# 42jaylonw/shifu

Measured on NVIDIA B200. Metric: env-steps/sec (obs+reward+term+reset), higher is better.
Workload: dtype f32

## Files before the change

### include/shifu_b200.h

```cpp
#ifndef SHIFU_B200_H
#define SHIFU_B200_H

#include <stdint.h>

#ifdef __cplusplus
extern "C" {
#endif

#define SHIFU_ABI_VERSION 5

#define SHIFU_MAX_DOF 12
#define SHIFU_MAX_LEG_BODIES 8
#define SHIFU_MAX_POINTS_X 17
#define SHIFU_MAX_POINTS_Y 11
#define SHIFU_MAX_REWARD_TERMS 8
#define SHIFU_NUM_STATS 16
#define SHIFU_OBS_HEAD 72

#define SHIFU_STREAM_OBS_NOISE 8

enum {
  SHIFU_OK = 0,
  SHIFU_E_NULL = -1,
  SHIFU_E_RANGE = -2,
  SHIFU_E_STATE = -3,
  SHIFU_E_NODEVICE = -4,
  SHIFU_E_ALIGN = -5
};

enum ShifuRewardTerm {
  SHIFU_REW_TRACKING_LIN_VEL = 0,
  SHIFU_REW_TRACKING_ANG_VEL = 1,
  SHIFU_REW_STABILIZING_BASE = 2,
  SHIFU_REW_SMOOTHING_ACTION = 3,
  SHIFU_REW_LEG_COLLISION = 4,
  SHIFU_REW_TORQUES = 5,
  SHIFU_REW_ABB_REACHING = 6,
  SHIFU_REW_ABB_SUCCESS = 7,
  SHIFU_REW_LIN_VEL_Z = 8,
  SHIFU_REW_ANG_VEL_XY = 9,
  SHIFU_REW_ORIENTATION = 10,
  SHIFU_REW_DOF_VEL = 11,
  SHIFU_REW_ACTION_RATE = 12,
  SHIFU_REW_BASE_HEIGHT = 13,
  SHIFU_REW_DOF_POS_LIMITS = 14,
  SHIFU_REW_FEET_AIR_TIME = 15,
  SHIFU_REW_COUNT = 16
};

enum ShifuObsVec {
  SHIFU_OBS_COMMAND = 0,
  SHIFU_OBS_BASE_LIN_VEL = 1,
  SHIFU_OBS_BASE_ANG_VEL = 2,
  SHIFU_OBS_GRAVITY_VEC = 3,
  SHIFU_OBS_PROJECTED_GRAVITY = 4,
  SHIFU_OBS_VEC_COUNT = 5
};

enum {
  SHIFU_STAT_TERM0 = 0,
  SHIFU_STAT_NRESET = 8,
  SHIFU_STAT_LEVEL_SUM = 9,
  SHIFU_STAT_SUCCESS = 10,
  SHIFU_STAT_NENVS = 11
};

typedef struct ShifuCtx ShifuCtx;

typedef struct ShifuA1Desc {
  int32_t abi_version;
  int32_t num_envs;
  int64_t env_offset;
  uint64_t rng_seed;
  int32_t num_dof;
  int32_t num_bodies;
  int32_t num_hist;
  int32_t num_obs;
  int32_t base_body;
  int32_t num_leg_bodies;
  int32_t leg_bodies[SHIFU_MAX_LEG_BODIES];
  int32_t force_body;
  int32_t root_stride;
  int32_t root_offset;
  float q0[SHIFU_MAX_DOF];
  float kp[SHIFU_MAX_DOF];
  float kd[SHIFU_MAX_DOF];
  float torque_limit[SHIFU_MAX_DOF];
  float action_scale;
  float clip_actions;
  float clip_obs;
  int32_t num_points_x;
  int32_t num_points_y;
  float points_x[SHIFU_MAX_POINTS_X];
  float points_y[SHIFU_MAX_POINTS_Y];
  float border_size;
  float horizontal_scale;
  float vertical_scale;
  float height_offset;
  float height_clip;
  int64_t max_episode_length;
  float max_episode_length_s;
  float contact_term_force;
  float default_root[7];
  float reset_xy_range;
  float push_force_max;
  float cmd_low[3];
  float cmd_high[3];
  int32_t curriculum;
  int32_t max_terrain_level;
  int32_t num_terrain_types;
  float level_up_distance;
  float level_down_factor;
  int32_t num_reward_terms;
  int32_t reward_terms[SHIFU_MAX_REWARD_TERMS];
  float reward_params[SHIFU_MAX_REWARD_TERMS][2];
  float dof_pos_limit_low[SHIFU_MAX_DOF];
  float dof_pos_limit_high[SHIFU_MAX_DOF];
  int32_t num_feet;
  int32_t feet_bodies[4];
  float feet_contact_force;
  float air_time_cmd_min;
  float air_time_dt;
  int32_t air_time_reset;
  int32_t obs_layout;
  int32_t obs_vec_src[4];
  float obs_scale[SHIFU_OBS_HEAD];
  float obs_height_scale;
  float obs_noise[SHIFU_OBS_HEAD];
  float obs_height_noise;
} ShifuA1Desc;

typedef struct ShifuA1StepIO {
  float* root_state;
  float* dof_state;
  const float* contact_state;
  const float* actions;
  const float* torques;
  float* history;
  float* command;
  int64_t* ep_len;
  float* ep_sums[SHIFU_MAX_REWARD_TERMS];
  float* base_lin_vel;
  float* base_ang_vel;
  float* projected_gravity;
  float* env_origins;
  int64_t* terrain_levels;
  const int64_t* terrain_types;
  const float* terrain_origins;
  float* dof_targets;
  float* rand_force;
  float* obs_buf;
  float* rew_buf;
  uint8_t* reset_buf;
  uint8_t* time_out_buf;
  uint8_t* contact_term_buf;
  float* measured_heights;
  int64_t step;
  const int64_t* step_dev;
  float* swing_time;
  uint8_t* last_contacts;
  int32_t carry_body_frame;
} ShifuA1StepIO;

typedef struct ShifuAbbDesc {
  int32_t abi_version;
  int32_t num_envs;
  int64_t env_offset;
  uint64_t rng_seed;
  int32_t num_actors;
  int32_t num_bodies;
  int32_t num_dof;
  int32_t ee_body;
  int32_t robot_actor, table_actor, cube_actor, goal_actor;
  float min_ee_pos[3];
  float max_ee_pos[3];
  float q0[SHIFU_MAX_DOF];
  float robot_root[7];
  float table_root[7];
  double box_pos_low[3];
  double box_pos_high[3];
  double goal_z;
  float success_distance;
  int64_t max_episode_length;
  float max_episode_length_s;
  float clip_obs;
  int32_t num_reward_terms;
  int32_t reward_terms[SHIFU_MAX_REWARD_TERMS];
  float reward_params[SHIFU_MAX_REWARD_TERMS][2];
} ShifuAbbDesc;

typedef struct ShifuAbbStepIO {
  float* root_state;
  const float* body_state;
  float* dof_state;
  float* dof_targets;
  int64_t* ep_len;
  float* ep_sums[SHIFU_MAX_REWARD_TERMS];
  float* obs_buf;
  float* rew_buf;
  uint8_t* reset_buf;
  uint8_t* time_out_buf;
  uint8_t* success_buf;
  int64_t step;
  const int64_t* step_dev;
} ShifuAbbStepIO;


int shifu_ctx_create(int device, const ShifuA1Desc* a1, const ShifuAbbDesc* abb, ShifuCtx** out);
int shifu_ctx_create_util(int device, int32_t num_envs, ShifuCtx** out);
int shifu_ctx_destroy(ShifuCtx* ctx);
const char* shifu_last_error(void);
int shifu_abi_version(void);

int shifu_set_height_map(ShifuCtx* ctx, const int16_t* height_samples, int32_t rows, int32_t cols, void* stream);

int shifu_set_level_sum(ShifuCtx* ctx, const int64_t* terrain_levels, void* stream);

int shifu_pd_torque(ShifuCtx* ctx, const float* actions_in, float* actions_out, const float* dof_state,
                    float* torques, int32_t substep, void* stream);

int shifu_body_frame(ShifuCtx* ctx, const float* root_state, int32_t num_envs, int32_t root_stride,
                     int32_t root_offset, float* base_lin_vel, float* base_ang_vel,
                     float* projected_gravity, float* gravity_vec, void* stream);

int shifu_get_heights(ShifuCtx* ctx, const float* root_state, float* measured_heights, int32_t* cell_idx,
                      void* stream);

int shifu_a1_post_physics(ShifuCtx* ctx, const ShifuA1StepIO* io, void* stream);

int shifu_a1_eval_terms(ShifuCtx* ctx, const ShifuA1StepIO* io, float* terms_out, void* stream);

int shifu_a1_reset_idx(ShifuCtx* ctx, const ShifuA1StepIO* io, const int64_t* env_ids, int32_t n_ids,
                       void* stream);

int shifu_abb_reset_idx(ShifuCtx* ctx, const ShifuAbbStepIO* io, const int64_t* env_ids, int32_t n_ids,
                        void* stream);

int shifu_abb_post_physics(ShifuCtx* ctx, const ShifuAbbStepIO* io, void* stream);

typedef struct ShifuArmIkIO {
  const float* body_state;
  const float* jacobian;
  const float* dof_state;
  const float* goal_pose;
  const float* actions;
  float* dof_targets;
  int32_t num_bodies;
  int32_t ee_body;
  int32_t num_links;
  int32_t ee_link;
  int32_t num_dof;
  float ee_velocity;
  float dt;
  float min_ee_pos[3];
  float max_ee_pos[3];
  float tar_quat[4];
  float damping;
} ShifuArmIkIO;
int shifu_arm_ik(ShifuCtx* ctx, const ShifuArmIkIO* io, int32_t num_envs, void* stream);

typedef struct ShifuCameraGatherIO {
  const void* const* color_src;
  const void* const* depth_src;
  const void* const* seg_src;
  const void* const* flow_src;
  void* color_out;
  float* depth_out;
  int32_t* seg_out;
  int16_t* flow_out;
  int32_t height, width;
  int32_t normalize_color;
} ShifuCameraGatherIO;
int shifu_camera_gather(ShifuCtx* ctx, const ShifuCameraGatherIO* io, int32_t num_envs, void* stream);

int shifu_compact_reset_ids(ShifuCtx* ctx, const uint8_t* reset_buf, int32_t n, int64_t* ids_out,
                            int32_t* n_out, void* stream);

int shifu_history_add(ShifuCtx* ctx, float* history, const float* x, int32_t n, int32_t a, int32_t h, void* stream);
int shifu_clip(ShifuCtx* ctx, const float* in, float* out, int64_t count, float c, void* stream);

enum ShifuTerrainKind {
  SHIFU_TERRAIN_PYRAMID = 0,
  SHIFU_TERRAIN_PYRAMID_NOISE = 1,
  SHIFU_TERRAIN_STAIRS = 2,
  SHIFU_TERRAIN_OBSTACLES = 3,
  SHIFU_TERRAIN_STONES = 4,
  SHIFU_TERRAIN_GAP = 5,
  SHIFU_TERRAIN_PIT = 6
};
typedef struct ShifuTerrainTile {
  int32_t kind;
  int32_t i, j;
  int32_t p[4];
  int32_t table_off;
} ShifuTerrainTile;
typedef struct ShifuTerrainDesc {
  int32_t num_rows, num_cols;
  int32_t width_px, length_px;
  int32_t border_px;
  double env_length, env_width;
  double horizontal_scale, vertical_scale;
} ShifuTerrainDesc;
int shifu_terrain_generate(ShifuCtx* ctx, const ShifuTerrainDesc* desc, const ShifuTerrainTile* tiles, int32_t n_tiles,
                           const double* table, int32_t n_table, int16_t* height_map, double* origins, void* stream);

int shifu_collect_stats(ShifuCtx* ctx, double* stats_out, int64_t* step_dev_to_advance, void* stream);
int shifu_collect_stats_ring(ShifuCtx* ctx, double* ring, int32_t slots, int32_t slot, int64_t* step_dev_to_advance,
                             void* stream);

int shifu_publish_extras(ShifuCtx* ctx, const double* stats, float* extras_out, void* stream);
int shifu_publish_extras_ring(ShifuCtx* ctx, const double* stats, float* ring, int32_t slots, int32_t slot,
                              const int64_t* step_dev, void* stream);

int shifu_read_stats_host(ShifuCtx* ctx, double* stats_host, void* stream);

#ifdef __cplusplus
}
#endif
#endif
```

### shifu_b200/_native.py

```python
from __future__ import annotations

import ctypes as C
import os
from typing import Optional

MAX_DOF, MAX_LEG, MAX_PX, MAX_PY, MAX_TERMS, NUM_STATS = 12, 8, 17, 11, 8, 16
ABI_VERSION = 5
OBS_HEAD = 72

REW_TRACKING_LIN_VEL, REW_TRACKING_ANG_VEL, REW_STABILIZING_BASE, REW_SMOOTHING_ACTION = 0, 1, 2, 3
REW_LEG_COLLISION, REW_TORQUES, REW_ABB_REACHING, REW_ABB_SUCCESS = 4, 5, 6, 7
REW_LIN_VEL_Z, REW_ANG_VEL_XY, REW_ORIENTATION, REW_DOF_VEL, REW_ACTION_RATE, REW_BASE_HEIGHT = 8, 9, 10, 11, 12, 13
REW_DOF_POS_LIMITS, REW_FEET_AIR_TIME = 14, 15
OBS_COMMAND, OBS_BASE_LIN_VEL, OBS_BASE_ANG_VEL, OBS_GRAVITY_VEC, OBS_PROJECTED_GRAVITY, OBS_VEC_COUNT = range(6)
STAT_TERM0, STAT_NRESET, STAT_LEVEL_SUM, STAT_SUCCESS, STAT_NENVS = 0, 8, 9, 10, 11

E_NULL, E_RANGE, E_STATE, E_NODEVICE, E_ALIGN = -1, -2, -3, -4, -5


class ShifuNativeError(RuntimeError):
    def __init__(self, code: int, msg: str):
        super().__init__(f"libshifu_b200 error {code}: {msg}")
        self.code = code


class A1Desc(C.Structure):
    _fields_ = [
        ("abi_version", C.c_int32), ("num_envs", C.c_int32), ("env_offset", C.c_int64),
        ("rng_seed", C.c_uint64),
        ("num_dof", C.c_int32), ("num_bodies", C.c_int32), ("num_hist", C.c_int32), ("num_obs", C.c_int32),
        ("base_body", C.c_int32), ("num_leg_bodies", C.c_int32), ("leg_bodies", C.c_int32 * MAX_LEG),
        ("force_body", C.c_int32), ("root_stride", C.c_int32), ("root_offset", C.c_int32),
        ("q0", C.c_float * MAX_DOF), ("kp", C.c_float * MAX_DOF), ("kd", C.c_float * MAX_DOF),
        ("torque_limit", C.c_float * MAX_DOF),
        ("action_scale", C.c_float), ("clip_actions", C.c_float), ("clip_obs", C.c_float),
        ("num_points_x", C.c_int32), ("num_points_y", C.c_int32),
        ("points_x", C.c_float * MAX_PX), ("points_y", C.c_float * MAX_PY),
        ("border_size", C.c_float), ("horizontal_scale", C.c_float), ("vertical_scale", C.c_float),
        ("height_offset", C.c_float), ("height_clip", C.c_float),
        ("max_episode_length", C.c_int64), ("max_episode_length_s", C.c_float),
        ("contact_term_force", C.c_float), ("default_root", C.c_float * 7),
        ("reset_xy_range", C.c_float), ("push_force_max", C.c_float),
        ("cmd_low", C.c_float * 3), ("cmd_high", C.c_float * 3),
        ("curriculum", C.c_int32), ("max_terrain_level", C.c_int32), ("num_terrain_types", C.c_int32),
        ("level_up_distance", C.c_float), ("level_down_factor", C.c_float),
        ("num_reward_terms", C.c_int32), ("reward_terms", C.c_int32 * MAX_TERMS),
        ("reward_params", (C.c_float * 2) * MAX_TERMS),
        ("dof_pos_limit_low", C.c_float * MAX_DOF), ("dof_pos_limit_high", C.c_float * MAX_DOF),
        ("num_feet", C.c_int32), ("feet_bodies", C.c_int32 * 4), ("feet_contact_force", C.c_float),
        ("air_time_cmd_min", C.c_float), ("air_time_dt", C.c_float), ("air_time_reset", C.c_int32),
        ("obs_layout", C.c_int32), ("obs_vec_src", C.c_int32 * 4), ("obs_scale", C.c_float * OBS_HEAD),
        ("obs_height_scale", C.c_float), ("obs_noise", C.c_float * OBS_HEAD), ("obs_height_noise", C.c_float),
    ]


class A1StepIO(C.Structure):
    _fields_ = [
        ("root_state", C.c_void_p), ("dof_state", C.c_void_p), ("contact_state", C.c_void_p),
        ("actions", C.c_void_p), ("torques", C.c_void_p), ("history", C.c_void_p), ("command", C.c_void_p),
        ("ep_len", C.c_void_p), ("ep_sums", C.c_void_p * MAX_TERMS),
        ("base_lin_vel", C.c_void_p), ("base_ang_vel", C.c_void_p), ("projected_gravity", C.c_void_p),
        ("env_origins", C.c_void_p), ("terrain_levels", C.c_void_p), ("terrain_types", C.c_void_p),
        ("terrain_origins", C.c_void_p), ("dof_targets", C.c_void_p), ("rand_force", C.c_void_p),
        ("obs_buf", C.c_void_p), ("rew_buf", C.c_void_p), ("reset_buf", C.c_void_p),
        ("time_out_buf", C.c_void_p), ("contact_term_buf", C.c_void_p), ("measured_heights", C.c_void_p),
        ("step", C.c_int64), ("step_dev", C.c_void_p), ("swing_time", C.c_void_p), ("last_contacts", C.c_void_p),
        ("carry_body_frame", C.c_int32),
    ]


class AbbDesc(C.Structure):
    _fields_ = [
        ("abi_version", C.c_int32), ("num_envs", C.c_int32), ("env_offset", C.c_int64),
        ("rng_seed", C.c_uint64),
        ("num_actors", C.c_int32), ("num_bodies", C.c_int32), ("num_dof", C.c_int32), ("ee_body", C.c_int32),
        ("robot_actor", C.c_int32), ("table_actor", C.c_int32), ("cube_actor", C.c_int32),
        ("goal_actor", C.c_int32),
        ("min_ee_pos", C.c_float * 3), ("max_ee_pos", C.c_float * 3), ("q0", C.c_float * MAX_DOF),
        ("robot_root", C.c_float * 7), ("table_root", C.c_float * 7),
        ("box_pos_low", C.c_double * 3), ("box_pos_high", C.c_double * 3), ("goal_z", C.c_double),
        ("success_distance", C.c_float),
        ("max_episode_length", C.c_int64), ("max_episode_length_s", C.c_float), ("clip_obs", C.c_float),
        ("num_reward_terms", C.c_int32), ("reward_terms", C.c_int32 * MAX_TERMS),
        ("reward_params", (C.c_float * 2) * MAX_TERMS),
    ]


class AbbStepIO(C.Structure):
    _fields_ = [
        ("root_state", C.c_void_p), ("body_state", C.c_void_p), ("dof_state", C.c_void_p),
        ("dof_targets", C.c_void_p), ("ep_len", C.c_void_p), ("ep_sums", C.c_void_p * MAX_TERMS),
        ("obs_buf", C.c_void_p), ("rew_buf", C.c_void_p), ("reset_buf", C.c_void_p),
        ("time_out_buf", C.c_void_p), ("success_buf", C.c_void_p), ("step", C.c_int64),
        ("step_dev", C.c_void_p),
    ]


class ArmIkIO(C.Structure):
    _fields_ = [
        ("body_state", C.c_void_p), ("jacobian", C.c_void_p), ("dof_state", C.c_void_p),
        ("goal_pose", C.c_void_p), ("actions", C.c_void_p), ("dof_targets", C.c_void_p),
        ("num_bodies", C.c_int32), ("ee_body", C.c_int32), ("num_links", C.c_int32), ("ee_link", C.c_int32),
        ("num_dof", C.c_int32), ("ee_velocity", C.c_float), ("dt", C.c_float),
        ("min_ee_pos", C.c_float * 3), ("max_ee_pos", C.c_float * 3), ("tar_quat", C.c_float * 4),
        ("damping", C.c_float),
    ]


class CameraGatherIO(C.Structure):
    _fields_ = [
        ("color_src", C.c_void_p), ("depth_src", C.c_void_p), ("seg_src", C.c_void_p), ("flow_src", C.c_void_p),
        ("color_out", C.c_void_p), ("depth_out", C.c_void_p), ("seg_out", C.c_void_p), ("flow_out", C.c_void_p),
        ("height", C.c_int32), ("width", C.c_int32), ("normalize_color", C.c_int32),
    ]


class TerrainTile(C.Structure):
    _fields_ = [("kind", C.c_int32), ("i", C.c_int32), ("j", C.c_int32), ("p", C.c_int32 * 4), ("table_off", C.c_int32)]


class TerrainDesc(C.Structure):
    _fields_ = [("num_rows", C.c_int32), ("num_cols", C.c_int32), ("width_px", C.c_int32), ("length_px", C.c_int32),
                ("border_px", C.c_int32), ("env_length", C.c_double), ("env_width", C.c_double),
                ("horizontal_scale", C.c_double), ("vertical_scale", C.c_double)]


TERRAIN_PYRAMID, TERRAIN_PYRAMID_NOISE, TERRAIN_STAIRS, TERRAIN_OBSTACLES, TERRAIN_STONES, TERRAIN_GAP, TERRAIN_PIT = range(7)

_VP, _I32, _I64, _F = C.c_void_p, C.c_int32, C.c_int64, C.c_float

SIGNATURES = {
    "shifu_ctx_create": [C.c_int, C.POINTER(A1Desc), C.POINTER(AbbDesc), C.POINTER(_VP)],
    "shifu_ctx_create_util": [C.c_int, _I32, C.POINTER(_VP)],
    "shifu_ctx_destroy": [_VP],
    "shifu_last_error": [],
    "shifu_abi_version": [],
    "shifu_set_height_map": [_VP, _VP, _I32, _I32, _VP],
    "shifu_set_level_sum": [_VP, _VP, _VP],
    "shifu_pd_torque": [_VP, _VP, _VP, _VP, _VP, _I32, _VP],
    "shifu_body_frame": [_VP, _VP, _I32, _I32, _I32, _VP, _VP, _VP, _VP, _VP],
    "shifu_get_heights": [_VP, _VP, _VP, _VP, _VP],
    "shifu_a1_post_physics": [_VP, C.POINTER(A1StepIO), _VP],
    "shifu_a1_eval_terms": [_VP, C.POINTER(A1StepIO), _VP, _VP],
    "shifu_abb_post_physics": [_VP, C.POINTER(AbbStepIO), _VP],
    "shifu_compact_reset_ids": [_VP, _VP, _I32, _VP, _VP, _VP],
    "shifu_history_add": [_VP, _VP, _VP, _I32, _I32, _I32, _VP],
    "shifu_clip": [_VP, _VP, _VP, _I64, _F, _VP],
    "shifu_arm_ik": [_VP, C.POINTER(ArmIkIO), _I32, _VP],
    "shifu_camera_gather": [_VP, C.POINTER(CameraGatherIO), _I32, _VP],
    "shifu_a1_reset_idx": [_VP, C.POINTER(A1StepIO), _VP, _I32, _VP],
    "shifu_abb_reset_idx": [_VP, C.POINTER(AbbStepIO), _VP, _I32, _VP],
    "shifu_collect_stats": [_VP, _VP, _VP, _VP],
    "shifu_collect_stats_ring": [_VP, _VP, _I32, _I32, _VP, _VP],
    "shifu_publish_extras": [_VP, _VP, _VP, _VP],
    "shifu_publish_extras_ring": [_VP, _VP, _VP, _I32, _I32, _VP, _VP],
    "shifu_read_stats_host": [_VP, _VP, _VP],
    "shifu_terrain_generate": [_VP, C.POINTER(TerrainDesc), C.POINTER(TerrainTile), _I32, C.POINTER(C.c_double), _I32,
                               _VP, _VP, _VP],
}
_RESTYPES = {"shifu_last_error": C.c_char_p}

_LIB: Optional[C.CDLL] = None


def lib_path() -> str:
    return os.environ.get("SHIFU_B200_LIB") or os.path.join(os.path.dirname(os.path.abspath(__file__)),
                                                            "libshifu_b200.so")


def load(build_if_missing: bool = True) -> C.CDLL:
    global _LIB
    if _LIB is not None:
        return _LIB
    path = lib_path()
    if build_if_missing and "SHIFU_B200_LIB" not in os.environ:
        from . import build as _build
        try:
            _build.build()
        except Exception as exc:
            if not os.path.exists(path) or _build.needs_build():
                raise ShifuNativeError(E_STATE, f"cannot build {path}: {exc}") from exc
    if not os.path.exists(path):
        raise ShifuNativeError(E_STATE, f"{path} not found; run `python -m shifu_b200.build` "
                                        "(there is no CPU / torch fallback)")
    lib = C.CDLL(path)
    for name, argtypes in SIGNATURES.items():
        fn = getattr(lib, name)
        fn.argtypes = argtypes
        fn.restype = _RESTYPES.get(name, C.c_int)
    if lib.shifu_abi_version() != ABI_VERSION:
        raise ShifuNativeError(E_STATE, f"ABI version mismatch: library {lib.shifu_abi_version()}, "
                                        f"binding {ABI_VERSION}")
    _LIB = lib
    return lib


def check(rc: int) -> None:
    if rc != 0:
        msg = load(False).shifu_last_error()
        raise ShifuNativeError(rc, msg.decode() if msg else "")


def ptr(t) -> Optional[int]:
    if t is None:
        return None
    if not t.is_cuda:
        raise ShifuNativeError(E_NODEVICE, "tensor is not on a CUDA device: the shifu_b200 hot path has "
                                           "no CPU fallback")
    if not t.is_contiguous():
        raise ShifuNativeError(E_ALIGN, "tensor must be contiguous")
    return t.data_ptr()


def current_stream() -> int:
    import torch
    return torch.cuda.current_stream().cuda_stream
```

### shifu_b200/csrc/a1_fused.cuh

```cuda
#pragma once
#include "a1_kernels.cuh"

namespace shifu {

struct A1Smem {
  float root[A1_TILE][13];
  float dof[A1_TILE][A1_DOF * 2];
  float contact[A1_TILE][A1_BODIES * 3];
  float hist[A1_TILE][A1_DOF * A1_HIST];
  float tau[A1_TILE][A1_DOF];
  float act[A1_TILE][A1_DOF];
  float head[A1_TILE][A1_HEAD];
  float rterm[SHIFU_MAX_REWARD_TERMS][A1_TILE];
  float cla[3][A1_TILE][3];
  ScanEnv ev[A1_TILE];
  float zb[A1_TILE];
};

__device__ __forceinline__ void load_span(float* __restrict__ dst, const float* __restrict__ src, int n,
                                          int tid, int nthreads) {
  if ((((uintptr_t)src | (uintptr_t)dst) & 15u) == 0) {
    const int n4 = n >> 2;
    const float4* s4 = reinterpret_cast<const float4*>(src);
    float4* d4 = reinterpret_cast<float4*>(dst);
    for (int i = tid; i < n4; i += nthreads) d4[i] = __ldg(s4 + i);
    for (int i = (n4 << 2) + tid; i < n; i += nthreads) dst[i] = __ldg(src + i);
  } else {
    for (int i = tid; i < n; i += nthreads) dst[i] = __ldg(src + i);
  }
}

__device__ __forceinline__ void store_span(float* __restrict__ dst, const float* __restrict__ src, int n,
                                           int tid, int nthreads) {
  if ((((uintptr_t)src | (uintptr_t)dst) & 15u) == 0) {
    const int n4 = n >> 2;
    const float4* s4 = reinterpret_cast<const float4*>(src);
    float4* d4 = reinterpret_cast<float4*>(dst);
    for (int i = tid; i < n4; i += nthreads) d4[i] = s4[i];
    for (int i = (n4 << 2) + tid; i < n; i += nthreads) dst[i] = src[i];
  } else {
    for (int i = tid; i < n; i += nthreads) dst[i] = src[i];
  }
}

__device__ __forceinline__ void a1_stage_rows(A1Smem& s, const A1K& k, const ShifuA1StepIO& io, int e0, int ne, int t) {
  if (k.root_stride == 1 && k.root_offset == 0) {
    load_span(&s.root[0][0], io.root_state + (long long)e0 * 13, ne * 13, t, A1_THREADS);
  } else {
    for (int i = t; i < ne * 13; i += A1_THREADS) {
      const int e = i / 13, c = i % 13;
      s.root[e][c] = io.root_state[((long long)(e0 + e) * k.root_stride + k.root_offset) * 13 + c];
    }
  }
  load_span(&s.dof[0][0], io.dof_state + (long long)e0 * (A1_DOF * 2), ne * A1_DOF * 2, t, A1_THREADS);
  load_span(&s.contact[0][0], io.contact_state + (long long)e0 * (A1_BODIES * 3), ne * A1_BODIES * 3, t, A1_THREADS);
  load_span(&s.hist[0][0], io.history + (long long)e0 * (A1_DOF * A1_HIST), ne * A1_DOF * A1_HIST, t, A1_THREADS);
  load_span(&s.tau[0][0], io.torques + (long long)e0 * A1_DOF, ne * A1_DOF, t, A1_THREADS);
  load_span(&s.act[0][0], io.actions + (long long)e0 * A1_DOF, ne * A1_DOF, t, A1_THREADS);
}

__device__ __forceinline__ bool force_exceeds(const float* f, float thr_sq) {
  return fma_rn(f[2], f[2], fma_rn(f[1], f[1], mul_rn(f[0], f[0]))) > thr_sq;
}

struct TermCtx {
  const float *cmd, *lin, *ang, *pg;
  const float *dof_row, *hist_row, *act_row, *contact_row;
  float base_z;
  float* swing;
  unsigned char* last;
};

__device__ __noinline__ float a1_extra_term(int code, float p0, float p1, const A1K& k, const TermCtx& c) {
  switch (code) {
    case SHIFU_REW_LIN_VEL_Z:
      return mul_rn(p0, mul_rn(c.lin[2], c.lin[2]));
    case SHIFU_REW_ANG_VEL_XY:
      return mul_rn(p0, add_rn(mul_rn(c.ang[0], c.ang[0]), mul_rn(c.ang[1], c.ang[1])));
    case SHIFU_REW_ORIENTATION:
      return mul_rn(p0, add_rn(mul_rn(c.pg[0], c.pg[0]), mul_rn(c.pg[1], c.pg[1])));
    case SHIFU_REW_DOF_VEL: {
      float acc = 0.0f;
#pragma unroll
      for (int d = 0; d < A1_DOF; ++d) acc = add_rn(acc, mul_rn(c.dof_row[2 * d + 1], c.dof_row[2 * d + 1]));
      return mul_rn(p0, acc);
    }
    case SHIFU_REW_ACTION_RATE: {
      float acc = 0.0f;
#pragma unroll
      for (int d = 0; d < A1_DOF; ++d) {
        const float df = sub_rn(c.hist_row[d * A1_HIST], c.act_row[d]);
        acc = add_rn(acc, mul_rn(df, df));
      }
      return mul_rn(p0, acc);
    }
    case SHIFU_REW_BASE_HEIGHT: {
      const float df = sub_rn(c.base_z, p1);
      return mul_rn(p0, mul_rn(df, df));
    }
    case SHIFU_REW_DOF_POS_LIMITS: {
      float acc = 0.0f;
#pragma unroll
      for (int d = 0; d < A1_DOF; ++d) {
        const float q = c.dof_row[2 * d];
        const float under = -fminf(sub_rn(q, k.dof_lo[d]), 0.0f), over = fmaxf(sub_rn(q, k.dof_hi[d]), 0.0f);
        acc = add_rn(acc, add_rn(under, over));
      }
      return mul_rn(p0, acc);
    }
    case SHIFU_REW_FEET_AIR_TIME: {
      if (c.swing == nullptr) return 0.0f;
      float rew = 0.0f;
      for (int f = 0; f < k.n_feet; ++f) {
        const bool contact = c.contact_row[k.feet[f] * 3 + 2] > k.feet_thr;
        const bool filt = contact | (c.last[f] != 0);
        c.last[f] = contact ? 1 : 0;
        float air = c.swing[f];
        const bool first = (air > 0.0f) & filt;
        air = add_rn(air, k.air_dt);
        rew = add_rn(rew, first ? sub_rn(air, p1) : 0.0f);
        c.swing[f] = filt ? 0.0f : air;
      }
      const bool moving = norm2_fma(c.cmd[0], c.cmd[1]) > k.air_cmd_min;
      return mul_rn(p0, moving ? rew : 0.0f);
    }
    default:
      return 0.0f;
  }
}

template <bool HAS_EXTRA, class Tile>
__device__ __forceinline__ float a1_reward_term(int code, int q, float p0, float p1, const A1K& k, const Tile& in, int e,
                                                const ShifuA1StepIO& io, long long ge) {
  const float* cmd = in.cla[0][e];
  const float* lin = in.cla[1][e];
  const float* ang = in.cla[2][e];
  if (HAS_EXTRA && code >= SHIFU_REW_LIN_VEL_Z) {
    const TermCtx c{cmd, lin, ang, io.projected_gravity + ge * 3, in.dof[e], in.hist[e], in.act[e], in.contact[e],
                    in.root[e][2], io.swing_time ? io.swing_time + ge * k.n_feet : nullptr,
                    io.last_contacts ? io.last_contacts + ge * k.n_feet : nullptr};
    return a1_extra_term(code, p0, p1, k, c);
  }
  switch (code) {
    case SHIFU_REW_TRACKING_LIN_VEL: {
      const float dx = sub_rn(cmd[0], lin[0]), dy = sub_rn(cmd[1], lin[1]);
      const float ne = -add_rn(mul_rn(dx, dx), mul_rn(dy, dy));
      return mul_rn(p0, expf(k.rp_pow2[q] ? mul_rn(ne, k.rp_inv[q]) : div_rn(ne, p1)));
    }
    case SHIFU_REW_TRACKING_ANG_VEL: {
      const float d = sub_rn(cmd[2], ang[2]);
      const float ne = -mul_rn(d, d);
      return mul_rn(p0, expf(k.rp_pow2[q] ? mul_rn(ne, k.rp_inv[q]) : div_rn(ne, p1)));
    }
    case SHIFU_REW_STABILIZING_BASE:
      return add_rn(mul_rn(p0, mul_rn(lin[2], lin[2])),
                    mul_rn(p1, add_rn(mul_rn(ang[0], ang[0]), mul_rn(ang[1], ang[1]))));
    case SHIFU_REW_SMOOTHING_ACTION: {
      float f1 = 0.0f, f2 = 0.0f;
#pragma unroll
      for (int d = 0; d < A1_DOF; ++d) {
        const float a0 = in.hist[e][d * A1_HIST + 0], a1 = in.hist[e][d * A1_HIST + 1],
                    a2 = in.hist[e][d * A1_HIST + 2];
        const float d1 = sub_rn(a1, a0);
        const float d2 = add_rn(sub_rn(a2, mul_rn(2.0f, a1)), a0);
        f1 = add_rn(f1, mul_rn(d1, d1));
        f2 = add_rn(f2, mul_rn(d2, d2));
      }
      return mul_rn(p0, add_rn(f1, f2));
    }
    case SHIFU_REW_LEG_COLLISION: {
      int cnt = 0;
      for (int b = 0; b < k.n_leg; ++b)
        cnt += force_exceeds(&in.contact[e][k.leg[b] * 3], k.rp_thr_sq[q]) ? 1 : 0;
      return mul_rn(p0, (float)cnt);
    }
    case SHIFU_REW_TORQUES: {
      float acc = 0.0f;
#pragma unroll
      for (int d = 0; d < A1_DOF; ++d) acc = add_rn(acc, mul_rn(in.tau[e][d], in.tau[e][d]));
      return mul_rn(p0, acc);
    }
    default:
      return 0.0f;
  }
}

__device__ __noinline__ float a1_eval_term(int q, const A1K& k, const A1Smem& s, int e, const ShifuA1StepIO& io,
                                           long long ge) {
  return a1_reward_term<true>(k.terms[q], q, k.rp[q][0], k.rp[q][1], k, s, e, io, ge);
}

template <bool EXACT_DIV, bool NOISE>
__global__ void __launch_bounds__(A1_THREADS, 5)
a1_post_physics_kernel(const __grid_constant__ A1K k, const __grid_constant__ ShifuA1StepIO io,
                       const __grid_constant__ A1Obs o, int first_tile) {
  __shared__ __align__(16) A1Smem s;
  __shared__ float pg0[A1_TILE][3];
  const int t = threadIdx.x, warp = t >> 5, lane = t & 31;
  const long long step = (io.step_dev != nullptr) ? *io.step_dev : io.step;
  const float bx = k.px[t % A1_NX], by = k.py[(t / A1_NX) % A1_NY];

  for (int e0 = (first_tile + blockIdx.x) * A1_TILE; e0 < k.n; e0 += gridDim.x * A1_TILE) {
    const int ne = min(A1_TILE, k.n - e0);
    const int ge = e0 + lane;
    const bool lane_env = (lane < ne);

    long long len = 0;
    float esum[SHIFU_MAX_REWARD_TERMS];
    float c9[9];
    if (warp == 0 && lane_env) {
      len = io.ep_len[ge];
#pragma unroll
      for (int j = 0; j < 3; ++j) {
        c9[j] = io.command[ge * 3LL + j];
        c9[3 + j] = io.base_lin_vel[ge * 3LL + j];
        c9[6 + j] = io.base_ang_vel[ge * 3LL + j];
      }
#pragma unroll
      for (int j = 0; j < SHIFU_MAX_REWARD_TERMS; ++j) esum[j] = (j < k.n_terms) ? io.ep_sums[j][ge] : 0.0f;
    }
    a1_stage_rows(s, k, io, e0, ne, t);
    if (o.uses_pg)
      for (int i = t; i < ne * 3; i += A1_THREADS) (&pg0[0][0])[i] = io.projected_gravity[e0 * 3LL + i];
    if (warp == 0 && lane_env) {
#pragma unroll
      for (int j = 0; j < 9; ++j) s.cla[j / 3][lane][j % 3] = c9[j];
    }
    __syncthreads();

    bool contact_term = false;
    if (lane_env) {
#pragma unroll 1
      for (int j = warp; j < k.n_terms; j += A1_THREADS / 32) s.rterm[j][lane] = a1_eval_term(j, k, s, lane, io, ge);
      if (warp == 0)
        contact_term = force_exceeds(&s.contact[lane][k.base_body * 3], k.contact_thr_sq);
      if (warp == 5)
        s.ev[lane] = make_scan_env(s.root[lane]);
    }
    __syncthreads();

    if (warp == 0) {
      bool reset = false;
      double st_sum[SHIFU_MAX_REWARD_TERMS];
#pragma unroll
      for (int j = 0; j < SHIFU_MAX_REWARD_TERMS; ++j) st_sum[j] = 0.0;
      long long level_delta = 0;
      if (lane_env) {
        len += 1;
        const bool time_out = len > k.max_len;
        reset = contact_term | time_out;
        float rew = 0.0f;
#pragma unroll
        for (int j = 0; j < SHIFU_MAX_REWARD_TERMS; ++j) {
          if (j < k.n_terms) {
            const float r = s.rterm[j][lane];
            esum[j] = add_rn(esum[j], r);
            rew = add_rn(rew, r);
          }
        }
        io.rew_buf[ge] = rew;
        io.reset_buf[ge] = reset ? 1 : 0;
        io.time_out_buf[ge] = time_out ? 1 : 0;
        io.contact_term_buf[ge] = contact_term ? 1 : 0;
        if (reset) {
          float cmd[3] = {s.cla[0][lane][0], s.cla[0][lane][1], s.cla[0][lane][2]};
          a1_reset_env<true>(k, io, step, ge, s.root[lane], s.dof[lane], s.hist[lane], cmd, esum, len, st_sum,
                             level_delta, io.env_origins[ge * 3LL + 0], io.env_origins[ge * 3LL + 1],
                             io.env_origins[ge * 3LL + 2], k.curriculum ? io.terrain_levels[ge] : 0,
                             k.curriculum ? io.terrain_types[ge] : 0);
          s.cla[0][lane][0] = cmd[0]; s.cla[0][lane][1] = cmd[1]; s.cla[0][lane][2] = cmd[2];
        }
        io.ep_len[ge] = len;
#pragma unroll
        for (int j = 0; j < SHIFU_MAX_REWARD_TERMS; ++j)
          if (j < k.n_terms) io.ep_sums[j][ge] = esum[j];
        s.zb[lane] = sub_rn(s.root[lane][2], k.h_off);
      }
      a1_log_sums(k, reset, st_sum, level_delta, lane);
    }
    __syncthreads();

    {
      const float c = k.clip_obs;
      auto nz = [&](float x, int e, int j) {
        return NOISE ? add_rn(x, obs_noise_at(o, k.seed, k.env_offset + e0 + e, step, j)) : x;
      };
      for (int i = t; i < ne * A1_DOF; i += A1_THREADS) {
        const int e = i / A1_DOF, d = i - e * A1_DOF;
        float* h = s.head[e];
        h[12 + d] = clampf(nz(mul_rn(sub_rn(s.dof[e][2 * d], k.q0[d]), o.scale[12 + d]), e, 12 + d), -c, c);
        h[24 + d] = clampf(nz(mul_rn(s.dof[e][2 * d + 1], o.scale[24 + d]), e, 24 + d), -c, c);
        const float a0 = s.hist[e][d * A1_HIST + 0], a1 = s.hist[e][d * A1_HIST + 1],
                    a2 = s.hist[e][d * A1_HIST + 2];
        h[36 + d] = clampf(nz(mul_rn(a0, o.scale[36 + d]), e, 36 + d), -c, c);
        h[48 + d] = clampf(nz(mul_rn(a1, o.scale[48 + d]), e, 48 + d), -c, c);
        h[60 + d] = clampf(nz(mul_rn(a2, o.scale[60 + d]), e, 60 + d), -c, c);
        s.hist[e][d * A1_HIST + 2] = a1;
        s.hist[e][d * A1_HIST + 1] = a0;
        s.hist[e][d * A1_HIST + 0] = s.act[e][d];
      }
      for (int i = t; i < ne * 12; i += A1_THREADS) {
        const int e = i / 12, j = i - e * 12;
        s.head[e][j] = clampf(nz(mul_rn(a1_obs_vec(o, j, s.cla, e, pg0[e][j % 3]), o.scale[j]), e, j), -c, c);
      }
      if (io.carry_body_frame && warp == 5 && lane_env) {
        const float* r = s.root[lane];
        float o[3];
        rotate_inverse(r + 3, r[7], r[8], r[9], o);
        io.base_lin_vel[ge * 3LL + 0] = o[0]; io.base_lin_vel[ge * 3LL + 1] = o[1];
        io.base_lin_vel[ge * 3LL + 2] = o[2];
        rotate_inverse(r + 3, r[10], r[11], r[12], o);
        io.base_ang_vel[ge * 3LL + 0] = o[0]; io.base_ang_vel[ge * 3LL + 1] = o[1];
        io.base_ang_vel[ge * 3LL + 2] = o[2];
        rotate_inverse(r + 3, 0.0f, 0.0f, -1.0f, o);
        io.projected_gravity[ge * 3LL + 0] = o[0]; io.projected_gravity[ge * 3LL + 1] = o[1];
        io.projected_gravity[ge * 3LL + 2] = o[2];
      }
    }
    __syncthreads();

    {
      float* obase = io.obs_buf + (long long)e0 * A1_OBS;
      const float* hsrc = &s.head[0][0];
      for (int i = t; i < ne * A1_HEAD; i += A1_THREADS) {
        const int e = i / A1_HEAD, j = i - e * A1_HEAD;
        __stcs(obase + (long long)e * A1_OBS + j, hsrc[i]);
      }
      store_span(io.history + (long long)e0 * (A1_DOF * A1_HIST), &s.hist[0][0], ne * A1_DOF * A1_HIST, t,
                 A1_THREADS);
    }

    if (t < A1_POINTS) {
      float* orow = io.obs_buf + (long long)e0 * A1_OBS + A1_HEAD + t;
      float* mrow = (io.measured_heights != nullptr) ? io.measured_heights + (long long)e0 * A1_POINTS + t
                                                     : nullptr;
#pragma unroll (NOISE ? 1 : 4)
      for (int e = 0; e < ne; ++e) {
        unsigned px, py;
        const float hgt = scan_point<EXACT_DIV>(s.ev[e], bx, by, k, &px, &py);
        float v = mul_rn(clampf(sub_rn(s.zb[e], hgt), -k.h_clip, k.h_clip), o.h_scale);
        if (NOISE) v = add_rn(v, obs_noise_at(o, k.seed, k.env_offset + e0 + e, step, A1_HEAD + t));
        v = clampf(v, -k.clip_obs, k.clip_obs);
        __stcs(orow + (long long)e * A1_OBS, v);
        if (mrow != nullptr) __stcs(mrow + (long long)e * A1_POINTS, hgt);
      }
    }
    __syncthreads();
  }
}

__global__ void __launch_bounds__(A1_THREADS)
a1_eval_terms_kernel(const __grid_constant__ A1K k, const __grid_constant__ ShifuA1StepIO io, float* __restrict__ out) {
  __shared__ __align__(16) A1Smem s;
  const int t = threadIdx.x, warp = t >> 5, lane = t & 31;
  for (int e0 = blockIdx.x * A1_TILE; e0 < k.n; e0 += gridDim.x * A1_TILE) {
    const int ne = min(A1_TILE, k.n - e0);
    const int ge = e0 + lane;
    __syncthreads();
    a1_stage_rows(s, k, io, e0, ne, t);
    if (warp == 0 && lane < ne) {
#pragma unroll
      for (int j = 0; j < 3; ++j) {
        s.cla[0][lane][j] = io.command[ge * 3LL + j];
        s.cla[1][lane][j] = io.base_lin_vel[ge * 3LL + j];
        s.cla[2][lane][j] = io.base_ang_vel[ge * 3LL + j];
      }
    }
    __syncthreads();
    if (lane < ne)
#pragma unroll 1
      for (int j = warp; j < k.n_terms; j += A1_THREADS / 32) out[(long long)j * k.n + ge] = a1_eval_term(j, k, s, lane, io, ge);
  }
}

}
```

### shifu_b200/csrc/a1_fused_tma.cuh

```cuda
#pragma once
#include "a1_fused.cuh"
#include "scan_pairs.cuh"
#include "tma_pipe.cuh"

namespace shifu {

constexpr int V3_STAGES = 3;
constexpr int V3_CTAS_PER_SM = 2;
constexpr int V3_BG_WARPS = 3;
constexpr int V3_SCAN_WARPS = 12;
static_assert(V3_BG_WARPS <= A1K_TERM_WARPS, "A1K holds a term list per B warp");
constexpr int V3_B_THREADS = 32 * V3_BG_WARPS, V3_B2_THREADS = 64;
constexpr int V3_C_THREADS = 32 * V3_SCAN_WARPS;
constexpr int V3_DMA_THREADS = 32;
constexpr int V3_THREADS = V3_B_THREADS + V3_C_THREADS + V3_DMA_THREADS;
constexpr int V3_SCAN_BASE = V3_B_THREADS;
constexpr int V3_DMA_BASE = V3_B_THREADS + V3_C_THREADS;
constexpr uint32_t V3_OBS_CHUNK_BYTES = 8 * A1_OBS * 4;

struct alignas(128) V3In {
  float root[A1_TILE][13];
  float dof[A1_TILE][A1_DOF * 2];
  float contact[A1_TILE][A1_BODIES * 3];
  float hist[A1_TILE][A1_DOF * A1_HIST];
  float tau[A1_TILE][A1_DOF];
  float act[A1_TILE][A1_DOF];
  long long ep_len[A1_TILE];
  float cla[3][A1_TILE][3];
  float esum[SHIFU_MAX_REWARD_TERMS][A1_TILE];
  float cout[3][A1_TILE][3];
};
static_assert(sizeof(V3In) == 22528 && offsetof(V3In, ep_len) == 18944 && offsetof(V3In, cout) % 16 == 0, "tile layout");

struct alignas(128) V3Smem {
  V3In in[V3_STAGES];
  float4 sA[4][A1_TILE / 2];
  float4 sB[4][A1_TILE / 2];
  float4 sC[4][A1_TILE / 2];
  float rterm[2][SHIFU_MAX_REWARD_TERMS][A1_TILE];
  uint64_t full_in[V3_STAGES], e_done[V3_STAGES], b_done[V3_STAGES], h_done[V3_STAGES];
};

constexpr uint32_t V3_ROW_BYTES = offsetof(V3In, ep_len);
constexpr uint32_t V3_HIST_BYTES = A1_TILE * A1_DOF * A1_HIST * 4;

__device__ __forceinline__ void v3_issue_hist_load(V3In& in, const ShifuA1StepIO& io, long long e0, uint64_t* bar) {
  pipe::bulk_load(in.hist, io.history + e0 * (A1_DOF * A1_HIST), sizeof(in.hist), bar);
}

__device__ __forceinline__ void v3_issue_loads(V3In& in, const A1K& k, const ShifuA1StepIO& io, long long e0,
                                               uint64_t* bar, bool with_hist) {
  const uint32_t scalars = sizeof(in.ep_len) + sizeof(in.cla) + k.n_terms * sizeof(in.esum[0]);
  pipe::mbar_arrive_expect_tx(bar, V3_ROW_BYTES + scalars);
  pipe::bulk_load(in.root, io.root_state + e0 * 13, sizeof(in.root), bar);
  pipe::bulk_load(in.dof, io.dof_state + e0 * (A1_DOF * 2), sizeof(in.dof), bar);
  pipe::bulk_load(in.contact, io.contact_state + e0 * (A1_BODIES * 3), sizeof(in.contact), bar);
  if (with_hist) v3_issue_hist_load(in, io, e0, bar);
  pipe::bulk_load(in.tau, io.torques + e0 * A1_DOF, sizeof(in.tau), bar);
  pipe::bulk_load(in.act, io.actions + e0 * A1_DOF, sizeof(in.act), bar);
  pipe::bulk_load(in.ep_len, io.ep_len + e0, sizeof(in.ep_len), bar);
  pipe::bulk_load(in.cla[0], io.command + e0 * 3, sizeof(in.cla[0]), bar);
  pipe::bulk_load(in.cla[1], io.base_lin_vel + e0 * 3, sizeof(in.cla[1]), bar);
  pipe::bulk_load(in.cla[2], io.base_ang_vel + e0 * 3, sizeof(in.cla[2]), bar);
  for (int q = 0; q < k.n_terms; ++q) pipe::bulk_load(in.esum[q], io.ep_sums[q] + e0, sizeof(in.esum[q]), bar);
}

template <bool EXACT_DIV, bool HAS_MROW, bool HAS_EXTRA, bool OBS, bool NOISE>
__global__ void __launch_bounds__(V3_THREADS, V3_CTAS_PER_SM)
a1_post_physics_tma_kernel(const __grid_constant__ A1K k, const __grid_constant__ ShifuA1StepIO io, int num_tiles,
                           const __grid_constant__ A1Obs o) {
  extern __shared__ __align__(128) unsigned char smem_raw[];
  V3Smem& s = *reinterpret_cast<V3Smem*>(smem_raw);
  const int t = threadIdx.x;
  const long long step = (io.step_dev != nullptr) ? *io.step_dev : io.step;
  const int first = blockIdx.x, stride = gridDim.x;
  const int my_tiles = (first < num_tiles) ? (num_tiles - first + stride - 1) / stride : 0;

  if (threadIdx.x == 0) {
#pragma unroll
    for (int b = 0; b < V3_STAGES; ++b) {
      pipe::mbar_init(&s.full_in[b], 1);
      pipe::mbar_init(&s.e_done[b], 32);
      pipe::mbar_init(&s.b_done[b], V3_B2_THREADS);
      pipe::mbar_init(&s.h_done[b], V3_C_THREADS);
    }
    pipe::fence_barrier_init();
  }
  __syncthreads();

  if (t >= V3_DMA_BASE && t < V3_DMA_BASE + V3_DMA_THREADS) {
    if (t != V3_DMA_BASE) return;
    for (int j = 0; j < V3_STAGES && j < my_tiles; ++j)
      v3_issue_loads(s.in[j], k, io, (long long)(first + j * stride) * A1_TILE, &s.full_in[j], true);
    for (int j = 0; j < my_tiles; ++j) {
      const int b = j % V3_STAGES;
      const uint32_t par = (j / V3_STAGES) & 1;
      const long long e0 = (long long)(first + j * stride) * A1_TILE;
      pipe::mbar_wait<64>(&s.h_done[b], par);
      pipe::bulk_store(io.history + e0 * (A1_DOF * A1_HIST), s.in[b].hist, V3_HIST_BYTES);
      if (io.carry_body_frame) {
        pipe::bulk_store(io.base_lin_vel + e0 * 3, s.in[b].cout[0], sizeof(s.in[b].cout[0]));
        pipe::bulk_store(io.base_ang_vel + e0 * 3, s.in[b].cout[1], sizeof(s.in[b].cout[1]));
        pipe::bulk_store(io.projected_gravity + e0 * 3, s.in[b].cout[2], sizeof(s.in[b].cout[2]));
      }
      pipe::bulk_commit();
      const long long en = (long long)(first + (j + V3_STAGES) * stride) * A1_TILE;
      if (j + V3_STAGES < my_tiles) v3_issue_loads(s.in[b], k, io, en, &s.full_in[b], false);
      pipe::bulk_wait_read_all();
      if (j + V3_STAGES < my_tiles) v3_issue_hist_load(s.in[b], io, en, &s.full_in[b]);
    }
    pipe::bulk_wait_all();
    return;
  }

  if (t < V3_B_THREADS) {
    const int warp = t >> 5, lane = t & 31;

    for (int j = 0; j < my_tiles; ++j) {
      const int b = j % V3_STAGES;
      const uint32_t par = (j / V3_STAGES) & 1;
      const long long e0 = (long long)(first + j * stride) * A1_TILE;
      const long long ge = e0 + lane;
      V3In& in = s.in[b];
      const int rb = j & 3;
      pipe::mbar_wait<64>(&s.full_in[b], par);

      if (warp == 0) {
        publish_scan_env(make_scan_env(in.root[lane]), lane, s.sA[rb], s.sB[rb], s.sC[rb]);
        pipe::mbar_arrive(&s.e_done[b]);
      }
#pragma unroll 1
      for (int i = 0; i < k.term_count[warp]; ++i) {
        const int q = k.term_list[warp][i];
        s.rterm[j & 1][q][lane] = a1_reward_term<HAS_EXTRA>(k.terms[q], q, k.rp[q][0], k.rp[q][1], k, in, lane, io, ge);
      }
      pipe::named_barrier(1, V3_B_THREADS);
      if (warp >= 2) continue;

      long long len = in.ep_len[lane] + 1;
      const bool contact_term = force_exceeds(&in.contact[lane][k.base_body * 3], k.contact_thr_sq);
      const bool time_out = len > k.max_len;
      const bool reset = contact_term | time_out;
      double st_sum[SHIFU_MAX_REWARD_TERMS];
#pragma unroll
      for (int q = 0; q < SHIFU_MAX_REWARD_TERMS; ++q) st_sum[q] = 0.0;
      long long level_delta = 0;
      float esum[SHIFU_MAX_REWARD_TERMS];
      float cmd[3];
      if (warp == 0) {
#pragma unroll
        for (int q = 0; q < SHIFU_MAX_REWARD_TERMS; ++q) esum[q] = (q < k.n_terms) ? in.esum[q][lane] : 0.0f;
        float rew = 0.0f;
#pragma unroll
        for (int q = 0; q < SHIFU_MAX_REWARD_TERMS; ++q) {
          if (q < k.n_terms) {
            const float r = s.rterm[j & 1][q][lane];
            esum[q] = add_rn(esum[q], r);
            rew = add_rn(rew, r);
          }
        }
        io.rew_buf[ge] = rew;
        io.reset_buf[ge] = reset ? 1 : 0;
        io.time_out_buf[ge] = time_out ? 1 : 0;
        io.contact_term_buf[ge] = contact_term ? 1 : 0;
        if (reset)
          a1_reset_env<true, 2>(k, io, step, (int)ge, nullptr, nullptr, nullptr, cmd, esum, len, st_sum, level_delta,
                                0.0f, 0.0f, 0.0f, 0, 0);
        io.ep_len[ge] = len;
#pragma unroll
        for (int q = 0; q < SHIFU_MAX_REWARD_TERMS; ++q)
          if (q < k.n_terms) io.ep_sums[q][ge] = esum[q];
        a1_log_sums<2>(k, reset, st_sum, level_delta, lane);
      } else {
        if (reset) {
          cmd[0] = in.cla[0][lane][0]; cmd[1] = in.cla[0][lane][1]; cmd[2] = in.cla[0][lane][2];
          a1_reset_env<true, 1, HAS_EXTRA>(k, io, step, (int)ge, in.root[lane], in.dof[lane], in.hist[lane], cmd, esum, len,
                                st_sum, level_delta, io.env_origins[ge * 3 + 0], io.env_origins[ge * 3 + 1],
                                io.env_origins[ge * 3 + 2], k.curriculum ? io.terrain_levels[ge] : 0,
                                k.curriculum ? io.terrain_types[ge] : 0);
          in.cla[0][lane][0] = cmd[0]; in.cla[0][lane][1] = cmd[1]; in.cla[0][lane][2] = cmd[2];
        }
        reinterpret_cast<float*>(&s.sC[rb][lane >> 1])[2 + (lane & 1)] =
            sub_rn(in.root[lane][2], k.h_off);
        if (io.carry_body_frame) {
          const float* r = in.root[lane];
#pragma unroll
          for (int v = 0; v < 3; ++v) {
            float o[3];
            rotate_inverse(r + 3, v == 2 ? 0.0f : r[7 + 3 * v], v == 2 ? 0.0f : r[8 + 3 * v],
                           v == 2 ? -1.0f : r[9 + 3 * v], o);
            in.cout[v][lane][0] = o[0]; in.cout[v][lane][1] = o[1]; in.cout[v][lane][2] = o[2];
          }
          pipe::fence_proxy_async();
        }
        a1_log_sums<1>(k, reset, st_sum, level_delta, lane);
      }
      pipe::mbar_arrive(&s.b_done[b]);
    }
    return;
  }

  {
    const int p = t - V3_SCAN_BASE;
    const int sw = p >> 5, lane = p & 31;
    const float hclip = NOISE ? k.clip_obs : OBS ? o.h_bound : fminf(k.h_clip, k.clip_obs);
    const short* __restrict__ table = k.table;
    const PairScanK sk = pair_scan_k(k);
    const f2_t VS = pk(k.vscale, k.vscale);
    static_assert(V3_SCAN_WARPS % 3 == 0 && 8 % (V3_SCAN_WARPS / 3) == 0, "scan warps: 3 pair groups x rows");
    constexpr int V3_ITEMS = 8 / (V3_SCAN_WARPS / 3);
    float hns[6];
    if (NOISE) {
      const int pd = p % A1_DOF;
#pragma unroll
      for (int m = 0; m < 6; ++m) hns[m] = o.noise[pd + 12 * m];
    }
    for (int j = 0; j < my_tiles; ++j) {
      const int b = j % V3_STAGES;
      const uint32_t par = (j / V3_STAGES) & 1;
      const long long e0 = (long long)(first + j * stride) * A1_TILE;
      const int rb = j & 3;
      pipe::mbar_wait<32>(&s.e_done[b], par);
      {
        struct Item { float bx, by; int q0, pt, it; bool live; };
        auto item = [&](int it) {
          Item r;
          const int raw = 32 * (sw % 3) + lane;
          r.live = raw <= A1_POINTS / 2;
          r.pt = r.live ? raw : A1_POINTS / 2;
          r.q0 = 2 * (V3_ITEMS * (sw / 3) + it);
          r.bx = k.px[r.pt % A1_NX]; r.by = k.py[r.pt / A1_NX];
          r.it = it;
          return r;
        };
        auto index_batch = [&](const Item& w, unsigned (&idx)[8]) {
          const f2_t BX = pk(w.bx, w.bx), BY = pk(w.by, w.by), NBY = pk(-w.by, -w.by);
#pragma unroll
          for (int u = 0; u < 2; ++u)
            point_pair_cells<EXACT_DIV>(sk, BX, BY, NBY, s.sA[rb][w.q0 + u], s.sB[rb][w.q0 + u],
                                        *reinterpret_cast<const float2*>(&s.sC[rb][w.q0 + u]), idx + 4 * u);
        };
        auto load_batch = [&](const unsigned (&idx)[8], int (&h)[8]) {
#pragma unroll
          for (int u = 0; u < 8; ++u) h[u] = __ldg(table + idx[u]);
        };
        auto store_batch = [&](const Item& w, const int (&h)[8]) {
          float* orow = io.obs_buf + (e0 + 2 * w.q0) * A1_OBS + A1_HEAD + w.pt;
          float* mb = HAS_MROW ? io.measured_heights + (e0 + 2 * w.q0) * A1_POINTS + w.pt : nullptr;
          auto emit = [&](float2 zb, int h0, int h1, float* ob, float* m, f2_t noise) {
            const f2_t hg2 = fma2(pk((float)h0, (float)h1), VS, sk.nz);
            float v0, v1;
            f2_t d2 = sub2(pk(zb.x, zb.y), hg2);
            if (NOISE) {
              upk(d2, v0, v1);
              d2 = pk(clampf(v0, -k.h_clip, k.h_clip), clampf(v1, -k.h_clip, k.h_clip));
              d2 = add2(fma2(d2, pk(o.h_scale, o.h_scale), sk.nz), noise);
            } else if (OBS) {
              d2 = mul2(d2, pk(o.h_scale, o.h_scale));
            }
            upk(d2, v0, v1);
            __stcs(ob, clampf(v0, -hclip, hclip));
            __stcs(ob + A1_OBS, clampf(v1, -hclip, hclip));
            if (HAS_MROW) {
              float g0, g1;
              upk(hg2, g0, g1);
              __stcs(m, g0);
              __stcs(m + A1_POINTS, g1);
            }
          };
          if (NOISE || w.live) {
            const int mir = (A1_POINTS - 1) - 2 * w.pt;
#pragma unroll
            for (int u = 0; u < 2; ++u) {
              f2_t npt = 0, nmir = 0;
              if (NOISE) {
                const int c = lane & 1;
                const U4 q = obs_noise_word(k.seed, k.env_offset + e0 + 2 * (w.q0 + u) + c, step, 18 + (w.pt >> 1));
                const uint32_t r0 = __shfl_xor_sync(~0u, c ? q.x : q.z, 1), r1 = __shfl_xor_sync(~0u, c ? q.y : q.w, 1);
                const uint32_t o0 = c ? q.z : q.x, o1 = c ? q.w : q.y;
                const float sh = o.h_noise;
                const float p0 = mul_rn(u_pm1(c ? r0 : o0), sh), p1 = mul_rn(u_pm1(c ? o0 : r0), sh);
                npt = pk(p0, p1);
                nmir = (w.pt == A1_POINTS / 2) ? npt
                                                : pk(mul_rn(u_pm1(c ? r1 : o1), sh), mul_rn(u_pm1(c ? o1 : r1), sh));
              }
              if (!NOISE || w.live) {
                const float2 zb = *reinterpret_cast<const float2*>(&s.sC[rb][w.q0 + u].z);
                emit(zb, h[4 * u], h[4 * u + 1], orow + (2 * u) * A1_OBS, mb + (2 * u) * A1_POINTS, npt);
                emit(zb, h[4 * u + 2], h[4 * u + 3], orow + (2 * u) * A1_OBS + mir, mb + (2 * u) * A1_POINTS + mir, nmir);
              }
            }
          }
        };
        unsigned idx[8];
        int h[8];
        Item cur = item(0);
        index_batch(cur, idx);
        load_batch(idx, h);
        float pgv = 0.0f;
        if (OBS) {
          const int pe = p / A1_DOF, pd = p - pe * A1_DOF;
          if (o.src[pd / 3] == SHIFU_OBS_PROJECTED_GRAVITY) pgv = io.projected_gravity[(e0 + pe) * 3 + pd % 3];
        }
        float hn[6];
        if (NOISE) {
          const int pe = p / A1_DOF, pd = p - pe * A1_DOF, c = pd & 1;
          const long long gid = k.env_offset + e0 + pe;
          const U4 wa = obs_noise_word(k.seed, gid, step, 3 * (pd >> 1) + c);
          const U4 wc = obs_noise_word(k.seed, gid, step, 3 * (pd >> 1) + 2);
          const uint32_t r0 = __shfl_xor_sync(~0u, c ? wa.x : wa.y, 1), r1 = __shfl_xor_sync(~0u, c ? wa.z : wa.w, 1);
          const uint32_t o0 = c ? wa.y : wa.x, o1 = c ? wa.w : wa.z;
          const uint32_t x[6] = {c ? r0 : o0, c ? r1 : o1, c ? o0 : r0, c ? o1 : r1, c ? wc.y : wc.x, c ? wc.w : wc.z};
#pragma unroll
          for (int m = 0; m < 6; ++m) hn[m] = mul_rn(u_pm1(x[m]), hns[m]);
        }
        pipe::mbar_wait<32>(&s.b_done[b], par);
        {
          static_assert(A1_TILE * A1_DOF == V3_C_THREADS && A1_TILE * 12 == V3_C_THREADS, "one item per scan thread");
          V3In& in = s.in[b];
          const float c = k.clip_obs;
          const int e = p / A1_DOF, d = p - e * A1_DOF;
          float* hrow = io.obs_buf + (e0 + e) * A1_OBS;
          const float2 qd = *reinterpret_cast<const float2*>(&in.dof[e][2 * d]);
          const float a0 = in.hist[e][d * A1_HIST + 0], a1 = in.hist[e][d * A1_HIST + 1],
                      a2 = in.hist[e][d * A1_HIST + 2];
          const float v = OBS ? a1_obs_vec(o, d, in.cla, e, pgv)
                              : (d < 9) ? in.cla[d / 3][e][d % 3] : ((d == 11) ? -1.0f : 0.0f);
          in.hist[e][d * A1_HIST + 2] = a1;
          in.hist[e][d * A1_HIST + 1] = a0;
          in.hist[e][d * A1_HIST + 0] = in.act[e][d];
          pipe::fence_proxy_async();
          pipe::mbar_arrive(&s.h_done[b]);
          auto sc = [&](float x, int m) {
            const float y = OBS ? mul_rn(x, o.scale[d + 12 * m]) : x;
            return NOISE ? add_rn(y, hn[m]) : y;
          };
          __stcs(hrow + d, clampf(sc(v, 0), -c, c));
          __stcs(hrow + 12 + d, clampf(sc(sub_rn(qd.x, k.q0[d]), 1), -c, c));
          __stcs(hrow + 24 + d, clampf(sc(qd.y, 2), -c, c));
          __stcs(hrow + 36 + d, clampf(sc(a0, 3), -c, c));
          __stcs(hrow + 48 + d, clampf(sc(a1, 4), -c, c));
          __stcs(hrow + 60 + d, clampf(sc(a2, 5), -c, c));
        }
#pragma unroll 1
        for (int it = 1; it < V3_ITEMS; ++it) {
          const Item nxt = item(it);
          index_batch(nxt, idx);
          store_batch(cur, h);
          load_batch(idx, h);
          cur = nxt;
        }
        store_batch(cur, h);
      }
    }
  }
}

}
```

### shifu_b200/csrc/a1_kernels.cuh

```cuda
#pragma once
#include "exact_math.cuh"
#include "philox.cuh"
#include "../../include/shifu_b200.h"

namespace shifu {

constexpr int A1_DOF = 12, A1_BODIES = 17, A1_HIST = 3, A1_OBS = 259;
constexpr int A1_NX = 17, A1_NY = 11, A1_POINTS = A1_NX * A1_NY;
constexpr int A1_HEAD = A1_OBS - A1_POINTS;
constexpr int A1_TILE = 32;
constexpr int A1_THREADS = 192;
constexpr int TILE_SHIFT = 3;

constexpr int A1K_TERM_WARPS = 4;

struct A1K {
  int n;
  long long env_offset;
  unsigned long long seed;
  int base_body, n_leg, leg[SHIFU_MAX_LEG_BODIES], force_body;
  int root_stride, root_offset;
  float q0[A1_DOF], kp[A1_DOF], kd[A1_DOF], tau_max[A1_DOF];
  float action_scale, clip_actions, clip_obs;
  float px[A1_NX], py[A1_NY];
  float border;
  ConstDiv hdiv;
  int exact_div;
  float vscale, h_off, h_clip;
  long long max_len;
  float max_len_s, contact_thr;
  float root0[7];
  float xy_span, xy_low, force_span, force_low, cmd_span[3], cmd_low[3];
  int curriculum, max_level, n_types;
  float up_dist, down_factor;
  int n_terms, terms[SHIFU_MAX_REWARD_TERMS];
  float rp[SHIFU_MAX_REWARD_TERMS][2];
  float rp_inv[SHIFU_MAX_REWARD_TERMS];
  int rp_pow2[SHIFU_MAX_REWARD_TERMS];
  float rp_thr_sq[SHIFU_MAX_REWARD_TERMS];
  float dof_lo[A1_DOF], dof_hi[A1_DOF];
  int n_feet, feet[4];
  float feet_thr, air_cmd_min, air_dt;
  int air_reset;
  int term_count[A1K_TERM_WARPS], term_list[A1K_TERM_WARPS][SHIFU_MAX_REWARD_TERMS];
  float contact_thr_sq;
  const short* table;
  int trows, tcols;
  int band_w;
  double* stats;
  float neg_zero;
};

static_assert(A1_HEAD == SHIFU_OBS_HEAD, "observation head width");
struct A1Obs {
  int src[4];
  float scale[A1_HEAD];
  float h_scale;
  float h_bound;
  int uses_pg;
  float noise[A1_HEAD];
  float h_noise;
  int noisy;
};
static_assert(STREAM_OBS_NOISE == SHIFU_STREAM_OBS_NOISE, "observation-noise stream");

__device__ __forceinline__ float obs_noise_at(const A1Obs& o, unsigned long long seed, long long gid, long long step,
                                              int j) {
  uint32_t word;
  int lane;
  obs_noise_slot(j, word, lane);
  return mul_rn(u_pm1(u4_lane(obs_noise_word(seed, gid, step, word), lane)), j < A1_HEAD ? o.noise[j] : o.h_noise);
}

template <class Cla>
__device__ __forceinline__ float a1_obs_vec(const A1Obs& o, int j, const Cla& cla, int e, float pg) {
  const int c = j % 3;
  switch (o.src[j / 3]) {
    case SHIFU_OBS_COMMAND: return cla[0][e][c];
    case SHIFU_OBS_BASE_LIN_VEL: return cla[1][e][c];
    case SHIFU_OBS_BASE_ANG_VEL: return cla[2][e][c];
    case SHIFU_OBS_GRAVITY_VEC: return c == 2 ? -1.0f : 0.0f;
    default: return pg;
  }
}

__device__ __forceinline__ int table_index(unsigned px, unsigned py, const A1K& k) {
  return (int)((px & ~7u) * (unsigned)(k.band_w - 1) + px + (py << TILE_SHIFT));
}

__global__ void build_scan_table_kernel(const short* __restrict__ H, int rows, int cols,
                                        short* __restrict__ T, int band_w) {
  const int trows = rows - 1, tcols = cols - 1;
  const long long total = (long long)trows * tcols;
  for (long long i = blockIdx.x * (long long)blockDim.x + threadIdx.x; i < total;
       i += (long long)gridDim.x * blockDim.x) {
    const int px = (int)(i / tcols), py = (int)(i % tcols);
    const short a = H[(long long)px * cols + py];
    const short b = H[(long long)(px + 1) * cols + py];
    const short c = H[(long long)px * cols + py + 1];
    T[(long long)(px >> TILE_SHIFT) * 8 * band_w + (long long)py * 8 + (px & 7)] = min(min(a, b), c);
  }
}

__device__ __forceinline__ float pd_one(float a, float q0, float kp, float kd, float lim, float q, float qd) {
  const float e = sub_rn(add_rn(a, q0), q);
  return clampf(sub_rn(mul_rn(kp, e), mul_rn(kd, qd)), -lim, lim);
}

__device__ __forceinline__ unsigned long long l2_policy_evict_first() {
  unsigned long long p;
  asm("createpolicy.fractional.L2::evict_first.b64 %0, 1.0;" : "=l"(p));
  return p;
}
__device__ __forceinline__ unsigned long long l2_policy_evict_normal() {
  unsigned long long p;
  asm("createpolicy.fractional.L2::evict_normal.b64 %0, 1.0;" : "=l"(p));
  return p;
}
__device__ __forceinline__ float4 ldg_l2(const float4* p, unsigned long long pol) {
  float4 v;
  asm volatile("ld.global.nc.L2::cache_hint.v4.f32 {%0, %1, %2, %3}, [%4], %5;"
               : "=f"(v.x), "=f"(v.y), "=f"(v.z), "=f"(v.w) : "l"(p), "l"(pol));
  return v;
}
__device__ __forceinline__ void stg_l2(float4* p, float4 v, unsigned long long pol) {
  asm volatile("st.global.L2::cache_hint.v4.f32 [%0], {%1, %2, %3, %4}, %5;"
               :: "l"(p), "f"(v.x), "f"(v.y), "f"(v.z), "f"(v.w), "l"(pol) : "memory");
}

__global__ void __launch_bounds__(256)
pd_torque_kernel(const __grid_constant__ A1K k, const float4* __restrict__ a_in, float4* __restrict__ a_out,
                 const float4* __restrict__ dof, float4* __restrict__ tau, int descending) {
  __shared__ __align__(16) float c_q0[A1_DOF], c_kp[A1_DOF], c_kd[A1_DOF], c_lim[A1_DOF];
  if (threadIdx.x < A1_DOF) {
    c_q0[threadIdx.x] = k.q0[threadIdx.x];
    c_kp[threadIdx.x] = k.kp[threadIdx.x];
    c_kd[threadIdx.x] = k.kd[threadIdx.x];
    c_lim[threadIdx.x] = k.tau_max[threadIdx.x];
  }
  __syncthreads();
  const unsigned total = (unsigned)k.n * (A1_DOF / 4);
  const float sc = k.action_scale, ca = k.clip_actions;
  const unsigned long long pol_first = l2_policy_evict_first(), pol_normal = l2_policy_evict_normal();
  for (unsigned i = blockIdx.x * blockDim.x + threadIdx.x; i < total; i += gridDim.x * blockDim.x) {
    const unsigned q = descending ? total - 1u - i : i;
    const unsigned g = q % 3u;
    const unsigned long long pol = i < total / 2u ? pol_first : pol_normal;
    float4 a = ldg_l2(a_in + q, pol);
    if (a_out != nullptr) {
      a.x = clampf(mul_rn(a.x, sc), -ca, ca); a.y = clampf(mul_rn(a.y, sc), -ca, ca);
      a.z = clampf(mul_rn(a.z, sc), -ca, ca); a.w = clampf(mul_rn(a.w, sc), -ca, ca);
      stg_l2(a_out + q, a, pol);
    }
    const float4 s0 = ldg_l2(dof + 2 * (size_t)q, pol), s1 = ldg_l2(dof + 2 * (size_t)q + 1, pol);
    const float4 q0 = reinterpret_cast<const float4*>(c_q0)[g], kp = reinterpret_cast<const float4*>(c_kp)[g];
    const float4 kd = reinterpret_cast<const float4*>(c_kd)[g], lm = reinterpret_cast<const float4*>(c_lim)[g];
    float4 t;
    t.x = pd_one(a.x, q0.x, kp.x, kd.x, lm.x, s0.x, s0.y);
    t.y = pd_one(a.y, q0.y, kp.y, kd.y, lm.y, s0.z, s0.w);
    t.z = pd_one(a.z, q0.z, kp.z, kd.z, lm.z, s1.x, s1.y);
    t.w = pd_one(a.w, q0.w, kp.w, kd.w, lm.w, s1.z, s1.w);
    stg_l2(tau + q, t, pol);
  }
}

__device__ __forceinline__ void rotate_inverse(const float* q, float vx, float vy, float vz, float* out) {
  const float qx = q[0], qy = q[1], qz = q[2], qw = q[3];
  const float s = sub_rn(mul_rn(2.0f, mul_rn(qw, qw)), 1.0f);
  const float cx = fma_rn(qy, vz, -mul_rn(qz, vy));
  const float cy = fma_rn(qz, vx, -mul_rn(qx, vz));
  const float cz = fma_rn(qx, vy, -mul_rn(qy, vx));
  const float dot = add_rn(add_rn(mul_rn(qx, vx), mul_rn(qy, vy)), mul_rn(qz, vz));
  const float v[3] = {vx, vy, vz}, c[3] = {cx, cy, cz}, qq[3] = {qx, qy, qz};
#pragma unroll
  for (int i = 0; i < 3; ++i) {
    const float a = mul_rn(v[i], s);
    const float b = mul_rn(mul_rn(c[i], qw), 2.0f);
    const float cc = mul_rn(mul_rn(qq[i], dot), 2.0f);
    out[i] = add_rn(sub_rn(a, b), cc);
  }
}

__global__ void __launch_bounds__(256)
body_frame_kernel(int n, int root_stride, int root_offset, const float* __restrict__ root, float* __restrict__ lin,
                  float* __restrict__ ang, float* __restrict__ pg, float* __restrict__ gvec) {
  for (int e = blockIdx.x * blockDim.x + threadIdx.x; e < n; e += gridDim.x * blockDim.x) {
    const float* r = root + ((long long)e * root_stride + root_offset) * 13;
    float row[13];
#pragma unroll
    for (int j = 0; j < 13; ++j) row[j] = r[j];
    float o[3];
    rotate_inverse(row + 3, row[7], row[8], row[9], o);
    lin[e * 3 + 0] = o[0]; lin[e * 3 + 1] = o[1]; lin[e * 3 + 2] = o[2];
    rotate_inverse(row + 3, row[10], row[11], row[12], o);
    ang[e * 3 + 0] = o[0]; ang[e * 3 + 1] = o[1]; ang[e * 3 + 2] = o[2];
    rotate_inverse(row + 3, 0.0f, 0.0f, -1.0f, o);
    pg[e * 3 + 0] = o[0]; pg[e * 3 + 1] = o[1]; pg[e * 3 + 2] = o[2];
    if (gvec != nullptr) { gvec[e * 3 + 0] = 0.0f; gvec[e * 3 + 1] = 0.0f; gvec[e * 3 + 2] = -1.0f; }
  }
}

struct ScanEnv {
  float z2, z, w, x, y;
};

__device__ __forceinline__ ScanEnv make_scan_env(const float* root_row) {
  const float qz = root_row[5], qw = root_row[6];
  float nrm = sqrt_rn(add_rn(mul_rn(qz, qz), mul_rn(qw, qw)));
  nrm = fmaxf(nrm, 1e-9f);
  ScanEnv ev;
  ev.z = div_rn(qz, nrm);
  ev.w = div_rn(qw, nrm);
  ev.z2 = mul_rn(ev.z, 2.0f);
  ev.x = root_row[0];
  ev.y = root_row[1];
  return ev;
}

template <bool EXACT_DIV>
__device__ __forceinline__ float scan_point(const ScanEnv& ev, float bx, float by, const A1K& k,
                                            unsigned* opx, unsigned* opy) {
  const float tx = -mul_rn(ev.z2, by);
  const float ty = mul_rn(ev.z2, bx);
  const float rx = add_rn(add_rn(bx, mul_rn(ev.w, tx)), -mul_rn(ev.z, ty));
  const float ry = add_rn(add_rn(by, mul_rn(ev.w, ty)), mul_rn(ev.z, tx));
  const float ax = add_rn(add_rn(rx, ev.x), k.border);
  const float ay = add_rn(add_rn(ry, ev.y), k.border);
  const float fx = EXACT_DIV ? div_rn(ax, k.hdiv.d) : div_const(ax, k.hdiv);
  const float fy = EXACT_DIV ? div_rn(ay, k.hdiv.d) : div_const(ay, k.hdiv);
  const unsigned px = min(__float2uint_rz(fx), (unsigned)(k.trows - 1));
  const unsigned py = min(__float2uint_rz(fy), (unsigned)(k.tcols - 1));
  *opx = px; *opy = py;
  const short h = __ldg(k.table + table_index(px, py, k));
  return mul_rn((float)h, k.vscale);
}

__global__ void __launch_bounds__(A1_THREADS)
get_heights_kernel(const __grid_constant__ A1K k, const float* __restrict__ root, float* __restrict__ mh,
                   int* __restrict__ cell_idx) {
  __shared__ ScanEnv s_ev[A1_TILE];
  const int t = threadIdx.x;
  const float bx = k.px[t % A1_NX], by = k.py[(t / A1_NX) % A1_NY];
  for (int e0 = blockIdx.x * A1_TILE; e0 < k.n; e0 += gridDim.x * A1_TILE) {
    const int ne = min(A1_TILE, k.n - e0);
    __syncthreads();
    if (t < ne) s_ev[t] = make_scan_env(root + ((long long)(e0 + t) * k.root_stride + k.root_offset) * 13);
    __syncthreads();
    if (t < A1_POINTS) {
      for (int e = 0; e < ne; ++e) {
        unsigned px, py;
        const float h = k.exact_div ? scan_point<true>(s_ev[e], bx, by, k, &px, &py)
                                    : scan_point<false>(s_ev[e], bx, by, k, &px, &py);
        const long long o = (long long)(e0 + e) * A1_POINTS + t;
        mh[o] = h;
        if (cell_idx != nullptr) { cell_idx[2 * o] = (int)px; cell_idx[2 * o + 1] = (int)py; }
      }
    }
  }
}

__device__ __forceinline__ double warp_sum(double v) {
#pragma unroll
  for (int o = 16; o > 0; o >>= 1) v += __shfl_xor_sync(0xffffffffu, v, o);
  return v;
}

template <bool MIRROR, int PARTS = 3, bool AIR = true>
__device__ __forceinline__ void a1_reset_env(const A1K& k, const ShifuA1StepIO& io, long long step, int ge,
                                             float* root_row, float* dof_row, float* hist_row,
                                             float (&cmd)[3], float (&esum)[SHIFU_MAX_REWARD_TERMS],
                                             long long& len, double (&st_sum)[SHIFU_MAX_REWARD_TERMS],
                                             long long& level_delta, float ox, float oy, float oz,
                                             long long old_level, long long ty) {
  const long long gid = k.env_offset + ge;
  if (PARTS & 2) {
    len = 0;
#pragma unroll
    for (int j = 0; j < SHIFU_MAX_REWARD_TERMS; ++j) {
      if (j < k.n_terms) { st_sum[j] = (double)esum[j]; esum[j] = 0.0f; }
    }
  }
  if (!(PARTS & 1)) return;
  if (k.curriculum) {
    const float dist = norm2_fma(sub_rn(root_row[0], ox), sub_rn(root_row[1], oy));
    const bool up = dist > k.up_dist;
    const float need = mul_rn(mul_rn(norm2_fma(cmd[0], cmd[1]), k.max_len_s), k.down_factor);
    const bool down = (dist < need) && !up;
    long long level = old_level + (up ? 1 : 0) - (down ? 1 : 0);
    const long long rnd = randint(draw(k.seed, gid, step, STREAM_LEVEL).x, k.max_level);
    level = (level >= k.max_level) ? rnd : (level < 0 ? 0 : level);
    io.terrain_levels[ge] = level;
    level_delta = level - old_level;
    const float* org = io.terrain_origins + (level * k.n_types + ty) * 3;
    ox = org[0]; oy = org[1]; oz = org[2];
    io.env_origins[ge * 3LL + 0] = ox; io.env_origins[ge * 3LL + 1] = oy; io.env_origins[ge * 3LL + 2] = oz;
  }
#pragma unroll
  for (int d = 0; d < A1_DOF; ++d) {
    dof_row[2 * d] = k.q0[d];
    dof_row[2 * d + 1] = 0.0f;
    io.dof_targets[ge * (long long)A1_DOF + d] = k.q0[d];
  }
  if (MIRROR) {
    float4* drow = reinterpret_cast<float4*>(io.dof_state + (long long)ge * (A1_DOF * 2));
    const float4* srow = reinterpret_cast<const float4*>(dof_row);
#pragma unroll
    for (int j = 0; j < A1_DOF * 2 / 4; ++j) drow[j] = srow[j];
  }
  const U4 uxy = draw(k.seed, gid, step, STREAM_XY);
  float rr[13];
  rr[0] = add_rn(add_rn(k.root0[0], ox), add_rn(mul_rn(k.xy_span, u01(uxy.x)), k.xy_low));
  rr[1] = add_rn(add_rn(k.root0[1], oy), add_rn(mul_rn(k.xy_span, u01(uxy.y)), k.xy_low));
  rr[2] = add_rn(k.root0[2], oz);
  rr[3] = k.root0[3]; rr[4] = k.root0[4]; rr[5] = k.root0[5]; rr[6] = k.root0[6];
#pragma unroll
  for (int j = 7; j < 13; ++j) rr[j] = 0.0f;
  float* grow = io.root_state + ((long long)ge * k.root_stride + k.root_offset) * 13;
#pragma unroll
  for (int j = 0; j < 13; ++j) {
    root_row[j] = rr[j];
    if (MIRROR) grow[j] = rr[j];
  }
  const U4 uf = draw(k.seed, gid, step, STREAM_FORCE);
  float* fr = io.rand_force + ((long long)ge * A1_BODIES + k.force_body) * 3;
  fr[0] = add_rn(mul_rn(k.force_span, u01(uf.x)), k.force_low);
  fr[1] = add_rn(mul_rn(k.force_span, u01(uf.y)), k.force_low);
  fr[2] = add_rn(mul_rn(k.force_span, u01(uf.z)), k.force_low);
#pragma unroll
  for (int j = 0; j < A1_DOF * A1_HIST; ++j) hist_row[j] = 0.0f;
  if (AIR && k.air_reset && io.swing_time != nullptr) {
    for (int f = 0; f < k.n_feet; ++f) {
      io.swing_time[(long long)ge * k.n_feet + f] = 0.0f;
      io.last_contacts[(long long)ge * k.n_feet + f] = 0;
    }
  }
  const U4 uc = draw(k.seed, gid, step, STREAM_CMD);
  cmd[0] = add_rn(mul_rn(k.cmd_span[0], u01(uc.x)), k.cmd_low[0]);
  cmd[1] = add_rn(mul_rn(k.cmd_span[1], u01(uc.y)), k.cmd_low[1]);
  cmd[2] = add_rn(mul_rn(k.cmd_span[2], u01(uc.z)), k.cmd_low[2]);
  io.command[ge * 3LL + 0] = cmd[0]; io.command[ge * 3LL + 1] = cmd[1]; io.command[ge * 3LL + 2] = cmd[2];
}

template <int PARTS = 3>
__device__ __forceinline__ void a1_log_sums(const A1K& k, bool reset, const double (&st_sum)[SHIFU_MAX_REWARD_TERMS],
                                            long long level_delta, int lane) {
  const unsigned any = __ballot_sync(0xffffffffu, reset);
  if (!any) return;
  if (PARTS != 3) {
    if (reset) {
      if (PARTS & 2) {
#pragma unroll
        for (int j = 0; j < SHIFU_MAX_REWARD_TERMS; ++j)
// ... 71 lines not shown
```

### shifu_b200/csrc/capi.cu

```cuda
#include <cuda_runtime.h>
#include <cstdio>
#include <cstring>
#include <cstdarg>
#include <cmath>
#include <new>

#include "../../include/shifu_b200.h"
#include "a1_kernels.cuh"
#include "a1_fused.cuh"
#include "a1_fused_tma.cuh"
#include "scan_pairs.cuh"
#include "abb_kernels.cuh"
#include "arm_ik.cuh"
#include "camera_gather.cuh"
#include "common_kernels.cuh"
#include "terrain_gen.cuh"

using namespace shifu;

static thread_local char g_err[512] = "";

static int fail(int code, const char* fmt, ...) {
  va_list ap;
  va_start(ap, fmt);
  vsnprintf(g_err, sizeof(g_err), fmt, ap);
  va_end(ap);
  return code;
}

#define CUDA_TRY(expr)                                                                      \
  do {                                                                                      \
    cudaError_t _e = (expr);                                                                \
    if (_e != cudaSuccess) return fail((int)_e, "%s: %s", #expr, cudaGetErrorString(_e));  \
  } while (0)

#define REQUIRE_PTR(p)                                                      \
  do {                                                                      \
    if ((p) == nullptr) return fail(SHIFU_E_NULL, "%s is NULL", #p);        \
  } while (0)

#define REQUIRE_ALIGNED(p, a)                                                                    \
  do {                                                                                           \
    if ((reinterpret_cast<uintptr_t>(p) & ((a) - 1)) != 0)                                       \
      return fail(SHIFU_E_ALIGN, "%s must be %d-byte aligned", #p, (int)(a));                    \
  } while (0)

struct ShifuCtx {
  int device = 0;
  int sm_count = 0;
  bool is_a1 = false, is_abb = false;
  ShifuA1Desc a1{};
  ShifuAbbDesc abb{};
  A1K a1k{};
  A1Obs a1o{};
  bool obs_custom = false;
  AbbK abbk{};
  short* d_table = nullptr;
  double* d_stats = nullptr;
  unsigned long long* d_chain = nullptr;
  unsigned* d_ticket = nullptr;
  int chain_len = 0;
  unsigned epoch = 0;
  int a1_grid = 0;
  int a1_occ = 0;
  int tma_occ = 0;
  bool use_tma = true;
  bool grid_symmetric = false;
};

static inline cudaStream_t S(void* s) { return reinterpret_cast<cudaStream_t>(s); }

constexpr int A1_TMA_VARIANTS = 24;
template <bool OBS, bool NOISE>
static void a1_tma_fill(const void** t) {
  t[0] = (const void*)a1_post_physics_tma_kernel<false, false, false, OBS, NOISE>;
  t[1] = (const void*)a1_post_physics_tma_kernel<false, false, true, OBS, NOISE>;
  t[2] = (const void*)a1_post_physics_tma_kernel<false, true, false, OBS, NOISE>;
  t[3] = (const void*)a1_post_physics_tma_kernel<false, true, true, OBS, NOISE>;
  t[4] = (const void*)a1_post_physics_tma_kernel<true, false, false, OBS, NOISE>;
  t[5] = (const void*)a1_post_physics_tma_kernel<true, false, true, OBS, NOISE>;
  t[6] = (const void*)a1_post_physics_tma_kernel<true, true, false, OBS, NOISE>;
  t[7] = (const void*)a1_post_physics_tma_kernel<true, true, true, OBS, NOISE>;
}
static const void* const* a1_tma_variants() {
  static const void* table[A1_TMA_VARIANTS];
  static const bool filled = (a1_tma_fill<false, false>(table), a1_tma_fill<true, false>(table + 8),
                              a1_tma_fill<true, true>(table + 16), true);
  (void)filled;
  return table;
}

extern "C" const char* shifu_last_error(void) { return g_err; }
extern "C" int shifu_abi_version(void) { return SHIFU_ABI_VERSION; }

static float sqrt_threshold(float thr) {
  if (!(thr >= 0.0f) || std::isinf(thr)) return thr;
  float s = thr * thr;
  while (s > 0.0f && std::sqrt(s) > thr) s = std::nextafter(s, 0.0f);
  while (std::sqrt(std::nextafter(s, INFINITY)) <= thr) s = std::nextafter(s, INFINITY);
  return s;
}

static int fill_a1obs(const ShifuA1Desc& d, A1Obs& o, bool& custom) {
  if (d.obs_layout != 0 && d.obs_layout != 1) return fail(SHIFU_E_RANGE, "obs_layout=%d must be 0 or 1", d.obs_layout);
  std::memset(&o, 0, sizeof(o));
  for (int i = 0; i < 4; ++i) o.src[i] = i;
  for (int j = 0; j < A1_HEAD; ++j) o.scale[j] = 1.0f;
  o.h_scale = 1.0f;
  o.h_bound = std::fmin(d.height_clip, d.clip_obs);
  custom = false;
  for (int j = 0; j <= A1_HEAD; ++j) {
    const float v = j < A1_HEAD ? d.obs_noise[j] : d.obs_height_noise;
    if (!std::isfinite(v))
      return j < A1_HEAD ? fail(SHIFU_E_RANGE, "obs_noise[%d]=%g is not finite", j, (double)v)
                         : fail(SHIFU_E_RANGE, "obs_height_noise=%g is not finite", (double)v);
    if (v != 0.0f && d.obs_layout == 0)
      return fail(SHIFU_E_RANGE, "observation noise needs obs_layout = 1 (obs_layout = 0 ignores the layout fields)");
  }
  if (d.obs_layout == 0) return SHIFU_OK;
  for (int i = 0; i < 4; ++i) {
    if (d.obs_vec_src[i] < 0 || d.obs_vec_src[i] >= SHIFU_OBS_VEC_COUNT)
      return fail(SHIFU_E_RANGE, "obs_vec_src[%d]=%d is not an enum ShifuObsVec value", i, d.obs_vec_src[i]);
    custom |= d.obs_vec_src[i] != i;
    o.src[i] = d.obs_vec_src[i];
    o.uses_pg |= d.obs_vec_src[i] == SHIFU_OBS_PROJECTED_GRAVITY;
  }
  for (int j = 0; j < A1_HEAD; ++j) {
    if (!std::isfinite(d.obs_scale[j])) return fail(SHIFU_E_RANGE, "obs_scale[%d]=%g is not finite", j, (double)d.obs_scale[j]);
    custom |= d.obs_scale[j] != 1.0f;
    o.scale[j] = d.obs_scale[j];
  }
  if (!std::isfinite(d.obs_height_scale))
    return fail(SHIFU_E_RANGE, "obs_height_scale=%g is not finite", (double)d.obs_height_scale);
  custom |= d.obs_height_scale != 1.0f;
  o.h_scale = d.obs_height_scale;
  o.h_bound = std::fmin(d.height_clip * std::fabs(o.h_scale), d.clip_obs);
  for (int j = 0; j < A1_HEAD; ++j) { o.noise[j] = d.obs_noise[j]; o.noisy |= d.obs_noise[j] != 0.0f; }
  o.h_noise = d.obs_height_noise;
  o.noisy |= d.obs_height_noise != 0.0f;
  custom |= o.noisy != 0;
  return SHIFU_OK;
}

static int fill_a1k(const ShifuA1Desc& d, A1K& k) {
  if (d.abi_version != SHIFU_ABI_VERSION) return fail(SHIFU_E_RANGE, "ShifuA1Desc.abi_version %d != %d", d.abi_version, SHIFU_ABI_VERSION);
  if (d.num_envs <= 0) return fail(SHIFU_E_RANGE, "num_envs must be > 0 (got %d)", d.num_envs);
  if (d.num_dof != A1_DOF || d.num_bodies != A1_BODIES || d.num_hist != A1_HIST || d.num_obs != A1_OBS ||
      d.num_points_x != A1_NX || d.num_points_y != A1_NY)
    return fail(SHIFU_E_RANGE,
                "this build is specialised for dof=%d bodies=%d hist=%d obs=%d grid=%dx%d (got %d %d %d %d %dx%d)",
                A1_DOF, A1_BODIES, A1_HIST, A1_OBS, A1_NX, A1_NY, d.num_dof, d.num_bodies, d.num_hist, d.num_obs,
                d.num_points_x, d.num_points_y);
  if (d.base_body < 0 || d.base_body >= A1_BODIES || d.force_body < 0 || d.force_body >= A1_BODIES)
    return fail(SHIFU_E_RANGE, "base_body/force_body out of range");
  if (d.num_leg_bodies < 0 || d.num_leg_bodies > SHIFU_MAX_LEG_BODIES) return fail(SHIFU_E_RANGE, "num_leg_bodies out of range");
  for (int i = 0; i < d.num_leg_bodies; ++i)
    if (d.leg_bodies[i] < 0 || d.leg_bodies[i] >= A1_BODIES) return fail(SHIFU_E_RANGE, "leg_bodies[%d] out of range", i);
  if (d.num_reward_terms < 0 || d.num_reward_terms > SHIFU_MAX_REWARD_TERMS) return fail(SHIFU_E_RANGE, "num_reward_terms out of range");
  for (int i = 0; i < d.num_reward_terms; ++i)
    if (d.reward_terms[i] < 0 || d.reward_terms[i] >= SHIFU_REW_COUNT ||
        d.reward_terms[i] == SHIFU_REW_ABB_REACHING || d.reward_terms[i] == SHIFU_REW_ABB_SUCCESS)
      return fail(SHIFU_E_RANGE, "reward_terms[%d]=%d is not an A1 term", i, d.reward_terms[i]);
  if (d.root_stride < 1 || d.root_offset < 0 || d.root_offset >= d.root_stride) return fail(SHIFU_E_RANGE, "root_stride/root_offset invalid");
  if (!(d.horizontal_scale > 0.f) || d.max_terrain_level < 1 || d.num_terrain_types < 1) return fail(SHIFU_E_RANGE, "terrain constants invalid");
  std::memset(&k, 0, sizeof(k));
  k.n = d.num_envs;
  k.env_offset = d.env_offset;
  k.seed = d.rng_seed;
  k.base_body = d.base_body;
  k.n_leg = d.num_leg_bodies;
  for (int i = 0; i < d.num_leg_bodies; ++i) k.leg[i] = d.leg_bodies[i];
  k.force_body = d.force_body;
  k.root_stride = d.root_stride;
  k.root_offset = d.root_offset;
  for (int i = 0; i < A1_DOF; ++i) { k.q0[i] = d.q0[i]; k.kp[i] = d.kp[i]; k.kd[i] = d.kd[i]; k.tau_max[i] = d.torque_limit[i]; }
  k.action_scale = d.action_scale; k.clip_actions = d.clip_actions; k.clip_obs = d.clip_obs;
  for (int i = 0; i < A1_NX; ++i) k.px[i] = d.points_x[i];
  for (int i = 0; i < A1_NY; ++i) k.py[i] = d.points_y[i];
  k.border = d.border_size;
  k.hdiv.d = d.horizontal_scale;
  k.hdiv.r = 1.0f / d.horizontal_scale;
  k.exact_div = (d.horizontal_scale == 0.1f) ? 0 : 1;
  k.vscale = d.vertical_scale; k.h_off = d.height_offset; k.h_clip = d.height_clip;
  k.max_len = d.max_episode_length; k.max_len_s = d.max_episode_length_s; k.contact_thr = d.contact_term_force;
  for (int i = 0; i < 7; ++i) k.root0[i] = d.default_root[i];
  k.xy_span = (float)((double)d.reset_xy_range - (double)(-d.reset_xy_range)); k.xy_low = -d.reset_xy_range;
  k.force_span = (float)((double)d.push_force_max - (double)(-d.push_force_max)); k.force_low = -d.push_force_max;
  for (int i = 0; i < 3; ++i) { k.cmd_span[i] = (float)((double)d.cmd_high[i] - (double)d.cmd_low[i]); k.cmd_low[i] = d.cmd_low[i]; }
  k.neg_zero = -0.0f;
  k.curriculum = d.curriculum; k.max_level = d.max_terrain_level; k.n_types = d.num_terrain_types;
  k.up_dist = d.level_up_distance; k.down_factor = d.level_down_factor;
  k.n_terms = d.num_reward_terms;
  for (int i = 0; i < d.num_reward_terms; ++i) {
    k.terms[i] = d.reward_terms[i]; k.rp[i][0] = d.reward_params[i][0]; k.rp[i][1] = d.reward_params[i][1];
    int ex = 0;
    const float p1 = d.reward_params[i][1];
    const bool pow2 = (p1 > 0.0f) && (std::frexp(p1, &ex) == 0.5f) && ex > -100 && ex < 100;
    k.rp_pow2[i] = pow2 ? 1 : 0;
    k.rp_inv[i] = pow2 ? 1.0f / p1 : 0.0f;
    k.rp_thr_sq[i] = sqrt_threshold(p1);
  }
  k.contact_thr_sq = sqrt_threshold(d.contact_term_force);
  for (int i = 0; i < A1_DOF; ++i) { k.dof_lo[i] = d.dof_pos_limit_low[i]; k.dof_hi[i] = d.dof_pos_limit_high[i]; }
  if (d.num_feet < 0 || d.num_feet > 4) return fail(SHIFU_E_RANGE, "num_feet=%d out of range", d.num_feet);
  k.n_feet = d.num_feet;
  for (int i = 0; i < 4; ++i) {
    if (i < d.num_feet && (d.feet_bodies[i] < 0 || d.feet_bodies[i] >= A1_BODIES))
      return fail(SHIFU_E_RANGE, "feet_bodies[%d]=%d out of range", i, d.feet_bodies[i]);
    k.feet[i] = d.feet_bodies[i];
  }
  k.feet_thr = d.feet_contact_force; k.air_cmd_min = d.air_time_cmd_min; k.air_dt = d.air_time_dt; k.air_reset = d.air_time_reset;
  static const int term_cost[SHIFU_REW_COUNT] = {30, 25, 12, 135, 70, 40, 20, 20, 8, 10, 10, 40, 60, 8, 70, 90};
  int load[A1K_TERM_WARPS] = {215, 160, 0, 0}, order[SHIFU_MAX_REWARD_TERMS];
  for (int i = 0; i < k.n_terms; ++i) order[i] = i;
  auto cost_of = [&](int q) { const int c = k.terms[q]; return (c >= 0 && c < SHIFU_REW_COUNT) ? term_cost[c] : 40; };
  for (int i = 0; i < k.n_terms; ++i)
    for (int j = i + 1; j < k.n_terms; ++j)
      if (cost_of(order[j]) > cost_of(order[i])) { const int t = order[i]; order[i] = order[j]; order[j] = t; }
  for (int w = 0; w < A1K_TERM_WARPS; ++w) k.term_count[w] = 0;
  for (int i = 0; i < k.n_terms; ++i) {
    int w = 0;
    for (int v = 1; v < V3_BG_WARPS; ++v) if (load[v] < load[w]) w = v;
    k.term_list[w][k.term_count[w]++] = order[i];
    load[w] += cost_of(order[i]);
  }
  return SHIFU_OK;
}

static int fill_abbk(const ShifuAbbDesc& d, AbbK& k) {
  if (d.abi_version != SHIFU_ABI_VERSION) return fail(SHIFU_E_RANGE, "ShifuAbbDesc.abi_version %d != %d", d.abi_version, SHIFU_ABI_VERSION);
  if (d.num_envs <= 0) return fail(SHIFU_E_RANGE, "num_envs must be > 0 (got %d)", d.num_envs);
  if (d.num_actors < 1 || d.num_bodies < 1 || d.num_dof < 0 || d.num_dof > SHIFU_MAX_DOF) return fail(SHIFU_E_RANGE, "actor/body/dof counts invalid");
  const int acts[4] = {d.robot_actor, d.table_actor, d.cube_actor, d.goal_actor};
  for (int i = 0; i < 4; ++i) if (acts[i] < 0 || acts[i] >= d.num_actors) return fail(SHIFU_E_RANGE, "actor index %d out of range", i);
  if (d.ee_body < 0 || d.ee_body >= d.num_bodies) return fail(SHIFU_E_RANGE, "ee_body out of range");
  if (d.num_reward_terms < 0 || d.num_reward_terms > SHIFU_MAX_REWARD_TERMS) return fail(SHIFU_E_RANGE, "num_reward_terms out of range");
  for (int i = 0; i < d.num_reward_terms; ++i)
    if (d.reward_terms[i] != SHIFU_REW_ABB_REACHING && d.reward_terms[i] != SHIFU_REW_ABB_SUCCESS)
      return fail(SHIFU_E_RANGE, "reward_terms[%d]=%d is not an ABB term", i, d.reward_terms[i]);
  std::memset(&k, 0, sizeof(k));
  k.n = d.num_envs; k.env_offset = d.env_offset; k.seed = d.rng_seed;
  k.n_actors = d.num_actors; k.n_bodies = d.num_bodies; k.n_dof = d.num_dof; k.ee_body = d.ee_body;
  k.robot_actor = d.robot_actor; k.table_actor = d.table_actor; k.cube_actor = d.cube_actor; k.goal_actor = d.goal_actor;
  for (int i = 0; i < 2; ++i) { k.min_xy[i] = d.min_ee_pos[i]; k.max_xy[i] = d.max_ee_pos[i]; }
  for (int i = 0; i < d.num_dof; ++i) k.q0[i] = d.q0[i];
  for (int i = 0; i < 7; ++i) { k.robot_root[i] = d.robot_root[i]; k.table_root[i] = d.table_root[i]; }
  for (int i = 0; i < 3; ++i) { k.pos_low[i] = d.box_pos_low[i]; k.pos_high[i] = d.box_pos_high[i]; }
  k.goal_z = d.goal_z; k.success_dist = d.success_distance;
  k.max_len = d.max_episode_length; k.max_len_s = d.max_episode_length_s; k.clip_obs = d.clip_obs;
  k.n_terms = d.num_reward_terms;
  for (int i = 0; i < d.num_reward_terms; ++i) { k.terms[i] = d.reward_terms[i]; k.rp[i][0] = d.reward_params[i][0]; k.rp[i][1] = d.reward_params[i][1]; }
  return SHIFU_OK;
}

static int ctx_create_impl(int device, const ShifuA1Desc* a1, const ShifuAbbDesc* abb, int util_envs, ShifuCtx** out);

extern "C" int shifu_ctx_create(int device, const ShifuA1Desc* a1, const ShifuAbbDesc* abb, ShifuCtx** out) {
  REQUIRE_PTR(out);
  *out = nullptr;
  if ((a1 == nullptr) == (abb == nullptr)) return fail(SHIFU_E_NULL, "exactly one of a1 / abb must be given");
  return ctx_create_impl(device, a1, abb, 0, out);
}

extern "C" int shifu_ctx_create_util(int device, int32_t num_envs, ShifuCtx** out) {
  REQUIRE_PTR(out);
  *out = nullptr;
  if (num_envs <= 0) return fail(SHIFU_E_RANGE, "num_envs must be > 0 (got %d)", num_envs);
  return ctx_create_impl(device, nullptr, nullptr, num_envs, out);
}

static int ctx_create_impl(int device, const ShifuA1Desc* a1, const ShifuAbbDesc* abb, int util_envs, ShifuCtx** out) {
  A1K a1k; AbbK abbk; A1Obs a1o; bool obs_custom = false;
  if (a1 != nullptr) {
    int rc = fill_a1k(*a1, a1k);
    if (rc == SHIFU_OK) rc = fill_a1obs(*a1, a1o, obs_custom);
    if (rc) return rc;
  }
  else if (abb != nullptr) { int rc = fill_abbk(*abb, abbk); if (rc) return rc; }
  int ndev = 0;
  if (cudaGetDeviceCount(&ndev) != cudaSuccess || ndev <= 0) {
    cudaGetLastError();
    return fail(SHIFU_E_NODEVICE, "no CUDA device: libshifu_b200 has no CPU fallback");
  }
  if (device < 0 || device >= ndev) return fail(SHIFU_E_RANGE, "device %d out of range (%d devices)", device, ndev);
  CUDA_TRY(cudaSetDevice(device));
  cudaDeviceProp prop;
  CUDA_TRY(cudaGetDeviceProperties(&prop, device));
  if (prop.major != 10) return fail(SHIFU_E_NODEVICE, "device %d is sm_%d%d; this library is built for sm_100a only", device, prop.major, prop.minor);
  ShifuCtx* c = new (std::nothrow) ShifuCtx();
  if (c == nullptr) return fail(SHIFU_E_STATE, "out of host memory");
  c->device = device;
  c->sm_count = prop.multiProcessorCount;
  int n = 0;
  if (a1 != nullptr) {
    c->is_a1 = true; c->a1 = *a1; c->a1k = a1k; c->a1o = a1o; c->obs_custom = obs_custom; n = a1->num_envs;
    c->grid_symmetric = true;
    for (int i = 0; i < A1_NX; ++i) c->grid_symmetric &= (a1k.px[i] == -a1k.px[A1_NX - 1 - i]);
    for (int i = 0; i < A1_NY; ++i) c->grid_symmetric &= (a1k.py[i] == -a1k.py[A1_NY - 1 - i]);
  }
  else if (abb != nullptr) { c->is_abb = true; c->abb = *abb; c->abbk = abbk; n = abb->num_envs; }
  else n = util_envs;
  cudaError_t e = cudaMalloc(&c->d_stats, sizeof(double) * (SHIFU_NUM_STATS + 1));
  if (e == cudaSuccess) e = cudaMemset(c->d_stats, 0, sizeof(double) * (SHIFU_NUM_STATS + 1));
  c->chain_len = (n + COMPACT_CHUNK - 1) / COMPACT_CHUNK + 1;
  if (e == cudaSuccess) e = cudaMalloc(&c->d_chain, sizeof(unsigned long long) * c->chain_len);
  if (e == cudaSuccess) e = cudaMemset(c->d_chain, 0, sizeof(unsigned long long) * c->chain_len);
  if (e == cudaSuccess) e = cudaMalloc(&c->d_ticket, sizeof(unsigned) * 2);
  if (e == cudaSuccess) e = cudaMemset(c->d_ticket, 0, sizeof(unsigned) * 2);
  if (e == cudaSuccess && c->is_a1) {
    const void* variants[4] = {
        (const void*)a1_post_physics_kernel<false, false>, (const void*)a1_post_physics_kernel<true, false>,
        (const void*)a1_post_physics_kernel<false, true>, (const void*)a1_post_physics_kernel<true, true>};
    for (int v = 0; v < 4 && e == cudaSuccess; ++v)
      e = cudaFuncSetAttribute(variants[v], cudaFuncAttributePreferredSharedMemoryCarveout, 75);
    int occ = 0;
    if (e == cudaSuccess)
      e = cudaOccupancyMaxActiveBlocksPerMultiprocessor(&occ, a1_post_physics_kernel<false, false>, A1_THREADS, 0);
    const int tiles = (n + A1_TILE - 1) / A1_TILE;
    const int cap = c->sm_count * (occ > 0 ? occ : 1);
    c->a1_grid = tiles < cap ? tiles : cap;
    c->a1_occ = occ;
    const void* const* tma_variants = a1_tma_variants();
    int smem_sm = 0;
    if (e == cudaSuccess) e = cudaDeviceGetAttribute(&smem_sm, cudaDevAttrMaxSharedMemoryPerMultiprocessor, device);
    int carve = 100;
    if (e == cudaSuccess && smem_sm > 0) {
      const long long need = (long long)V3_CTAS_PER_SM * ((long long)sizeof(V3Smem) + 1024);
      carve = (int)((need * 100 + smem_sm - 1) / smem_sm);
      if (carve > 100) carve = 100;
    }
    for (int v = 0; v < A1_TMA_VARIANTS && e == cudaSuccess; ++v) {
      e = cudaFuncSetAttribute(tma_variants[v], cudaFuncAttributeMaxDynamicSharedMemorySize, (int)sizeof(V3Smem));
      if (e == cudaSuccess)
        e = cudaFuncSetAttribute(tma_variants[v], cudaFuncAttributePreferredSharedMemoryCarveout, carve);
    }
    int tocc = 0;
    if (e == cudaSuccess)
      e = cudaOccupancyMaxActiveBlocksPerMultiprocessor(&tocc, a1_post_physics_tma_kernel<false, false, false, false, false>, V3_THREADS,
                                                        sizeof(V3Smem));
    c->tma_occ = tocc;
    const char* kern = getenv("SHIFU_A1_KERNEL");
    c->use_tma = !(kern != nullptr && strcmp(kern, "phased") == 0);
  }
  if (e != cudaSuccess) {
    int rc = fail((int)e, "shifu_ctx_create: %s", cudaGetErrorString(e));
    shifu_ctx_destroy(c);
    return rc;
  }
  c->a1k.stats = c->d_stats;
  c->abbk.stats = c->d_stats;
  CUDA_TRY(cudaDeviceSynchronize());
  *out = c;
  return SHIFU_OK;
}

extern "C" int shifu_ctx_destroy(ShifuCtx* c) {
  if (c == nullptr) return SHIFU_OK;
  cudaFree(c->d_table);
  cudaFree(c->d_stats);
  cudaFree(c->d_chain);
  cudaFree(c->d_ticket);
  delete c;
  return SHIFU_OK;
}

static inline int grid_for(long long work_items, int threads, int sm_count, int per_sm) {
  long long g = (work_items + threads - 1) / threads;
  const long long cap = (long long)sm_count * per_sm;
  if (g > cap) g = cap;
  if (g < 1) g = 1;
  return (int)g;
}

extern "C" int shifu_set_height_map(ShifuCtx* c, const int16_t* hs, int32_t rows, int32_t cols, void* stream) {
  REQUIRE_PTR(c); REQUIRE_PTR(hs);
  if (!c->is_a1) return fail(SHIFU_E_STATE, "height map only applies to an A1 ctx");
  if (rows < 2 || cols < 2 || (long long)rows * cols > (1LL << 30)) return fail(SHIFU_E_RANGE, "map %dx%d out of range", rows, cols);
  const int trows = rows - 1, tcols = cols - 1;
  const int bands = (trows + 7) / 8, band_w = ((tcols + 7) / 8) * 8;
  const size_t elems = (size_t)bands * 8 * band_w;
  CUDA_TRY(cudaStreamSynchronize(S(stream)));
  if (c->d_table != nullptr) { cudaFree(c->d_table); c->d_table = nullptr; }
  CUDA_TRY(cudaMalloc(&c->d_table, elems * sizeof(short)));
  CUDA_TRY(cudaMemsetAsync(c->d_table, 0, elems * sizeof(short), S(stream)));
  build_scan_table_kernel<<<grid_for((long long)trows * tcols, 256, c->sm_count, 8), 256, 0, S(stream)>>>(
      hs, rows, cols, c->d_table, band_w);
  CUDA_TRY(cudaGetLastError());
  CUDA_TRY(cudaStreamSynchronize(S(stream)));
  c->a1k.table = c->d_table;
  c->a1k.trows = trows; c->a1k.tcols = tcols; c->a1k.band_w = band_w;
  return SHIFU_OK;
}

extern "C" int shifu_set_level_sum(ShifuCtx* c, const int64_t* levels, void* stream) {
  REQUIRE_PTR(c); REQUIRE_PTR(levels);
  if (!c->is_a1) return fail(SHIFU_E_STATE, "terrain levels only apply to an A1 ctx");
  CUDA_TRY(cudaMemsetAsync(c->d_stats + SHIFU_NUM_STATS, 0, sizeof(double), S(stream)));
  level_sum_kernel<<<grid_for(c->a1.num_envs, 256, c->sm_count, 2), 256, 0, S(stream)>>>(
      reinterpret_cast<const long long*>(levels), c->a1.num_envs, c->d_stats + SHIFU_NUM_STATS);
  CUDA_TRY(cudaGetLastError());
  return SHIFU_OK;
}

extern "C" int shifu_pd_torque(ShifuCtx* c, const float* a_in, float* a_out, const float* dof, float* tau,
                               int32_t substep, void* stream) {
  REQUIRE_PTR(c); REQUIRE_PTR(a_in); REQUIRE_PTR(dof); REQUIRE_PTR(tau);
  if (!c->is_a1) return fail(SHIFU_E_STATE, "shifu_pd_torque needs an A1 ctx");
  if (substep < 0) return fail(SHIFU_E_RANGE, "shifu_pd_torque: substep must be >= 0 (got %d)", substep);
  REQUIRE_ALIGNED(dof, 16); REQUIRE_ALIGNED(a_in, 16); REQUIRE_ALIGNED(tau, 16);
  if (a_out != nullptr) REQUIRE_ALIGNED(a_out, 16);
  const long long quads = (long long)c->a1.num_envs * (A1_DOF / 4);
  const int descending = substep & 1;
  pd_torque_kernel<<<grid_for(quads, 256, c->sm_count, 8), 256, 0, S(stream)>>>(
      c->a1k, reinterpret_cast<const float4*>(a_in), reinterpret_cast<float4*>(a_out),
      reinterpret_cast<const float4*>(dof), reinterpret_cast<float4*>(tau), descending);
  CUDA_TRY(cudaGetLastError());
  return SHIFU_OK;
}

extern "C" int shifu_body_frame(ShifuCtx* c, const float* root, int32_t n, int32_t root_stride, int32_t root_offset,
                                float* lin, float* ang, float* pg, float* gvec, void* stream) {
  REQUIRE_PTR(c); REQUIRE_PTR(root); REQUIRE_PTR(lin); REQUIRE_PTR(ang); REQUIRE_PTR(pg);
  if (n <= 0 || root_stride < 1 || root_offset < 0 || root_offset >= root_stride)
    return fail(SHIFU_E_RANGE, "shifu_body_frame: n=%d stride=%d offset=%d invalid", n, root_stride, root_offset);
  body_frame_kernel<<<grid_for(n, 256, c->sm_count, 8), 256, 0, S(stream)>>>(n, root_stride, root_offset, root, lin,
                                                                            ang, pg, gvec);
  CUDA_TRY(cudaGetLastError());
  return SHIFU_OK;
}

extern "C" int shifu_get_heights(ShifuCtx* c, const float* root, float* mh, int32_t* cell_idx, void* stream) {
  REQUIRE_PTR(c); REQUIRE_PTR(root); REQUIRE_PTR(mh);
  if (!c->is_a1) return fail(SHIFU_E_STATE, "shifu_get_heights needs an A1 ctx");
  if (c->d_table == nullptr) return fail(SHIFU_E_STATE, "call shifu_set_height_map first");
  const int tiles = (c->a1.num_envs + A1_TILE - 1) / A1_TILE;
  if (cell_idx == nullptr && !c->a1k.exact_div && c->grid_symmetric && c->use_tma) {
    const int cap4 = c->sm_count * 4;
    get_heights_pairs_kernel<<<tiles < cap4 ? tiles : cap4, SP_THREADS, 0, S(stream)>>>(c->a1k, root, mh);
    CUDA_TRY(cudaGetLastError());
    return SHIFU_OK;
  }
  const int cap = c->sm_count * 8;
  get_heights_kernel<<<tiles < cap ? tiles : cap, A1_THREADS, 0, S(stream)>>>(c->a1k, root, mh, cell_idx);
  CUDA_TRY(cudaGetLastError());
  return SHIFU_OK;
}

extern "C" int shifu_a1_eval_terms(ShifuCtx* c, const ShifuA1StepIO* io, float* out, void* stream) {
  REQUIRE_PTR(c); REQUIRE_PTR(io); REQUIRE_PTR(out);
  if (!c->is_a1) return fail(SHIFU_E_STATE, "shifu_a1_eval_terms needs an A1 ctx");
  REQUIRE_PTR(io->root_state); REQUIRE_PTR(io->dof_state); REQUIRE_PTR(io->contact_state); REQUIRE_PTR(io->actions);
  REQUIRE_PTR(io->torques); REQUIRE_PTR(io->history); REQUIRE_PTR(io->command); REQUIRE_PTR(io->base_lin_vel);
  REQUIRE_PTR(io->base_ang_vel); REQUIRE_PTR(io->projected_gravity);
  const int tiles = (c->a1.num_envs + A1_TILE - 1) / A1_TILE;
  const int cap = c->sm_count * 8;
  a1_eval_terms_kernel<<<tiles < cap ? tiles : cap, A1_THREADS, 0, S(stream)>>>(c->a1k, *io, out);
  CUDA_TRY(cudaGetLastError());
  return SHIFU_OK;
}

extern "C" int shifu_a1_post_physics(ShifuCtx* c, const ShifuA1StepIO* io, void* stream) {
  REQUIRE_PTR(c); REQUIRE_PTR(io);
  if (!c->is_a1) return fail(SHIFU_E_STATE, "shifu_a1_post_physics needs an A1 ctx");
  if (c->d_table == nullptr) return fail(SHIFU_E_STATE, "call shifu_set_height_map first");
  REQUIRE_PTR(io->root_state); REQUIRE_PTR(io->dof_state); REQUIRE_PTR(io->contact_state);
  REQUIRE_PTR(io->actions); REQUIRE_PTR(io->torques); REQUIRE_PTR(io->history); REQUIRE_PTR(io->command);
  REQUIRE_PTR(io->ep_len); REQUIRE_PTR(io->base_lin_vel); REQUIRE_PTR(io->base_ang_vel);
  REQUIRE_PTR(io->projected_gravity); REQUIRE_PTR(io->env_origins); REQUIRE_PTR(io->terrain_levels);
  REQUIRE_PTR(io->terrain_types); REQUIRE_PTR(io->terrain_origins); REQUIRE_PTR(io->dof_targets);
  REQUIRE_PTR(io->rand_force); REQUIRE_PTR(io->obs_buf); REQUIRE_PTR(io->rew_buf); REQUIRE_PTR(io->reset_buf);
  REQUIRE_PTR(io->time_out_buf); REQUIRE_PTR(io->contact_term_buf);
  for (int j = 0; j < c->a1.num_reward_terms; ++j)
    if (io->ep_sums[j] == nullptr) return fail(SHIFU_E_NULL, "ep_sums[%d] is NULL", j);
  REQUIRE_ALIGNED(io->dof_state, 16);
  const bool exact = c->a1k.exact_div != 0;
  const int n = c->a1.num_envs;

  auto al16 = [](const void* p) { return (reinterpret_cast<uintptr_t>(p) & 15u) == 0; };
  const bool can_tma = c->use_tma && c->grid_symmetric && c->a1k.root_stride == 1 && c->a1k.root_offset == 0 && al16(io->root_state) &&
                       al16(io->dof_state) && al16(io->contact_state) && al16(io->history) && al16(io->torques) &&
                       al16(io->actions) && al16(io->obs_buf) && al16(io->ep_len) && al16(io->command) &&
                       al16(io->base_lin_vel) && al16(io->base_ang_vel) && al16(io->projected_gravity) &&
                       [&] { for (int q = 0; q < c->a1k.n_terms; ++q) if (!al16(io->ep_sums[q])) return false; return true; }();
  const int full_tiles = can_tma ? n / A1_TILE : 0;
  if (full_tiles > 0) {
    const int cap = c->sm_count * (c->tma_occ > 0 ? c->tma_occ : 1);
    const dim3 grid(full_tiles < cap ? full_tiles : cap), block(V3_THREADS);
    const size_t smem = sizeof(V3Smem);
    const bool mrow = io->measured_heights != nullptr;
    bool extra = false;
    for (int q = 0; q < c->a1k.n_terms; ++q) extra |= c->a1k.terms[q] >= SHIFU_REW_LIN_VEL_Z;
    int tiles_arg = full_tiles;
    void* args[4] = {(void*)&c->a1k, const_cast<ShifuA1StepIO*>(io), (void*)&tiles_arg, (void*)&c->a1o};
    const int variant = (c->obs_custom ? 8 : 0) + (c->a1o.noisy ? 8 : 0) + (exact ? 4 : 0) + (mrow ? 2 : 0) + (extra ? 1 : 0);
    CUDA_TRY(cudaLaunchKernel(a1_tma_variants()[variant], grid, block, args, smem, S(stream)));
  }
  const int tiles = (n + A1_TILE - 1) / A1_TILE - full_tiles;
  if (tiles > 0) {
    const int cap = c->sm_count * (c->a1_occ > 0 ? c->a1_occ : 1);
    const dim3 grid(tiles < cap ? tiles : cap), block(A1_THREADS);
    const A1K& k = c->a1k;
    const A1Obs& o = c->a1o;
    if (o.noisy) {
      if (exact) a1_post_physics_kernel<true, true><<<grid, block, 0, S(stream)>>>(k, *io, o, full_tiles);
      else a1_post_physics_kernel<false, true><<<grid, block, 0, S(stream)>>>(k, *io, o, full_tiles);
    } else {
      if (exact) a1_post_physics_kernel<true, false><<<grid, block, 0, S(stream)>>>(k, *io, o, full_tiles);
      else a1_post_physics_kernel<false, false><<<grid, block, 0, S(stream)>>>(k, *io, o, full_tiles);
    }
    CUDA_TRY(cudaGetLastError());
  }
  return SHIFU_OK;
}

extern "C" int shifu_abb_post_physics(ShifuCtx* c, const ShifuAbbStepIO* io, void* stream) {
  REQUIRE_PTR(c); REQUIRE_PTR(io);
  if (!c->is_abb) return fail(SHIFU_E_STATE, "shifu_abb_post_physics needs an ABB ctx");
  REQUIRE_PTR(io->root_state); REQUIRE_PTR(io->body_state); REQUIRE_PTR(io->dof_state); REQUIRE_PTR(io->dof_targets);
  REQUIRE_PTR(io->ep_len); REQUIRE_PTR(io->obs_buf); REQUIRE_PTR(io->rew_buf); REQUIRE_PTR(io->reset_buf);
  REQUIRE_PTR(io->time_out_buf); REQUIRE_PTR(io->success_buf);
  for (int j = 0; j < c->abb.num_reward_terms; ++j)
    if (io->ep_sums[j] == nullptr) return fail(SHIFU_E_NULL, "ep_sums[%d] is NULL", j);
  abb_post_physics_kernel<<<grid_for(c->abb.num_envs, 128, c->sm_count, 16), 128, 0, S(stream)>>>(c->abbk, *io);
  CUDA_TRY(cudaGetLastError());
  return SHIFU_OK;
}

extern "C" int shifu_abb_reset_idx(ShifuCtx* c, const ShifuAbbStepIO* io, const int64_t* ids, int32_t n_ids, void* stream) {
  REQUIRE_PTR(c); REQUIRE_PTR(io);
  if (c->is_a1) return fail(SHIFU_E_STATE, "shifu_abb_reset_idx needs an ABB ctx");
  if (n_ids < 0 || n_ids > c->abb.num_envs) return fail(SHIFU_E_RANGE, "n_ids=%d out of range", n_ids);
  if (n_ids == 0) return SHIFU_OK;
  REQUIRE_PTR(io->root_state); REQUIRE_PTR(io->dof_state); REQUIRE_PTR(io->dof_targets); REQUIRE_PTR(io->ep_len);
  REQUIRE_PTR(io->reset_buf); REQUIRE_PTR(io->success_buf);
  for (int j = 0; j < c->abb.num_reward_terms; ++j)
    if (io->ep_sums[j] == nullptr) return fail(SHIFU_E_NULL, "ep_sums[%d] is NULL", j);
  abb_reset_idx_kernel<<<grid_for(n_ids, 128, c->sm_count, 16), 128, 0, S(stream)>>>(
      c->abbk, *io, reinterpret_cast<const long long*>(ids), n_ids);
  CUDA_TRY(cudaGetLastError());
  return SHIFU_OK;
}

extern "C" int shifu_compact_reset_ids(ShifuCtx* c, const uint8_t* flags, int32_t n, int64_t* ids, int32_t* n_out, void* stream) {
  REQUIRE_PTR(c); REQUIRE_PTR(flags); REQUIRE_PTR(ids); REQUIRE_PTR(n_out);
  if (n <= 0) return fail(SHIFU_E_RANGE, "n must be > 0 (got %d)", n);
  const int chunks = (n + COMPACT_CHUNK - 1) / COMPACT_CHUNK;
  if (chunks > c->chain_len) return fail(SHIFU_E_RANGE, "n=%d exceeds the ctx's num_envs", n);
  c->epoch += 1;
  compact_ids_kernel<<<chunks, COMPACT_THREADS, 0, S(stream)>>>(flags, n, reinterpret_cast<long long*>(ids), n_out,
                                                               c->d_chain, c->d_ticket, c->epoch);
  CUDA_TRY(cudaGetLastError());
  return SHIFU_OK;
}

extern "C" int shifu_history_add(ShifuCtx* c, float* hist, const float* x, int32_t n, int32_t a, int32_t h, void* stream) {
  REQUIRE_PTR(c); REQUIRE_PTR(hist); REQUIRE_PTR(x);
  if (n <= 0 || a <= 0 || h <= 0) return fail(SHIFU_E_RANGE, "history shape (%d,%d,%d) invalid", n, a, h);
  const long long rows = (long long)n * a;
  history_add_kernel<<<grid_for(rows, 256, c->sm_count, 8), 256, 0, S(stream)>>>(hist, x, rows, h);
  CUDA_TRY(cudaGetLastError());
  return SHIFU_OK;
}

extern "C" int shifu_arm_ik(ShifuCtx* c, const ShifuArmIkIO* io, int32_t n, void* stream) {
  REQUIRE_PTR(c); REQUIRE_PTR(io); REQUIRE_PTR(io->body_state); REQUIRE_PTR(io->jacobian); REQUIRE_PTR(io->dof_state);
  REQUIRE_PTR(io->dof_targets);
  if ((io->goal_pose == nullptr) == (io->actions == nullptr))
    return fail(SHIFU_E_RANGE, "shifu_arm_ik: exactly one of goal_pose / actions must be given");
  if (n <= 0) return fail(SHIFU_E_RANGE, "num_envs must be > 0");
  if (io->num_dof < 1 || io->num_dof > SHIFU_MAX_DOF) return fail(SHIFU_E_RANGE, "num_dof=%d out of range", io->num_dof);
  if (io->ee_body < 0 || io->ee_body >= io->num_bodies || io->ee_link < 0 || io->ee_link >= io->num_links)
    return fail(SHIFU_E_RANGE, "end-effector body/link index out of range");
  arm_ik_kernel<<<grid_for(n, 128, c->sm_count, 16), 128, 0, S(stream)>>>(*io, n);
  CUDA_TRY(cudaGetLastError());
  return SHIFU_OK;
}

extern "C" int shifu_camera_gather(ShifuCtx* c, const ShifuCameraGatherIO* io, int32_t n, void* stream) {
  REQUIRE_PTR(c); REQUIRE_PTR(io);
  if (n <= 0 || io->height <= 0 || io->width <= 0) return fail(SHIFU_E_RANGE, "num_envs, height and width must be > 0");
  if ((io->color_src && !io->color_out) || (io->depth_src && !io->depth_out) || (io->seg_src && !io->seg_out) ||
      (io->flow_src && !io->flow_out))
    return fail(SHIFU_E_NULL, "shifu_camera_gather: an image type has a source table but no output buffer");
  if (!io->color_src && !io->depth_src && !io->seg_src && !io->flow_src) return SHIFU_OK;
  const long long px = (long long)io->height * io->width;
  if (px % 8 != 0) return fail(SHIFU_E_RANGE, "height*width=%lld must be a multiple of 8", px);
  int bx = (int)((px / 4 + 255) / 256);
  if (bx > 8) bx = 8;
  const dim3 grid(bx, n < 65535 ? n : 65535);
  camera_gather_kernel<<<grid, 256, 0, S(stream)>>>(*io, n);
  CUDA_TRY(cudaGetLastError());
  return SHIFU_OK;
}

extern "C" int shifu_clip(ShifuCtx* c, const float* in, float* out, int64_t count, float lim, void* stream) {
  REQUIRE_PTR(c); REQUIRE_PTR(in); REQUIRE_PTR(out);
  if (count <= 0) return fail(SHIFU_E_RANGE, "count must be > 0");
  clip_kernel<<<grid_for((count + 3) / 4, 256, c->sm_count, 8), 256, 0, S(stream)>>>(in, out, count, lim);
  CUDA_TRY(cudaGetLastError());
  return SHIFU_OK;
}

extern "C" int shifu_a1_reset_idx(ShifuCtx* c, const ShifuA1StepIO* io, const int64_t* ids, int32_t n_ids, void* stream) {
  REQUIRE_PTR(c); REQUIRE_PTR(io);
  if (!c->is_a1) return fail(SHIFU_E_STATE, "shifu_a1_reset_idx needs an A1 ctx");
  if (n_ids < 0 || n_ids > c->a1.num_envs) return fail(SHIFU_E_RANGE, "n_ids=%d out of range", n_ids);
  if (n_ids == 0) return SHIFU_OK;
  REQUIRE_PTR(io->root_state); REQUIRE_PTR(io->dof_state); REQUIRE_PTR(io->history); REQUIRE_PTR(io->command);
  REQUIRE_PTR(io->ep_len); REQUIRE_PTR(io->env_origins); REQUIRE_PTR(io->terrain_levels);
  REQUIRE_PTR(io->terrain_types); REQUIRE_PTR(io->terrain_origins); REQUIRE_PTR(io->dof_targets);
  REQUIRE_PTR(io->rand_force); REQUIRE_PTR(io->reset_buf);
  for (int j = 0; j < c->a1.num_reward_terms; ++j)
    if (io->ep_sums[j] == nullptr) return fail(SHIFU_E_NULL, "ep_sums[%d] is NULL", j);
  a1_reset_idx_kernel<<<grid_for(n_ids, 128, c->sm_count, 16), 128, 0, S(stream)>>>(
      c->a1k, *io, reinterpret_cast<const long long*>(ids), n_ids);
  CUDA_TRY(cudaGetLastError());
  return SHIFU_OK;
}

extern "C" int shifu_collect_stats(ShifuCtx* c, double* out, int64_t* step_dev, void* stream) {
  REQUIRE_PTR(c); REQUIRE_PTR(out);
  const double n = c->is_a1 ? c->a1.num_envs : c->abb.num_envs;
  collect_stats_kernel<<<1, 32, 0, S(stream)>>>(c->d_stats, c->d_stats + SHIFU_NUM_STATS, out, 1, 0, n,
                                                reinterpret_cast<long long*>(step_dev));
  CUDA_TRY(cudaGetLastError());
  return SHIFU_OK;
}

extern "C" int shifu_collect_stats_ring(ShifuCtx* c, double* ring, int32_t slots, int32_t slot, int64_t* step_dev, void* stream) {
  REQUIRE_PTR(c); REQUIRE_PTR(ring);
  if (slots < 1 || slot >= slots) return fail(SHIFU_E_RANGE, "slot %d outside the ring of %d", slot, slots);
  if (slot < 0 && step_dev == nullptr) return fail(SHIFU_E_NULL, "slot < 0 needs the device step counter");
  const double n = c->is_a1 ? c->a1.num_envs : c->abb.num_envs;
  collect_stats_kernel<<<1, 32, 0, S(stream)>>>(c->d_stats, c->d_stats + SHIFU_NUM_STATS, ring, slots, slot, n,
                                                reinterpret_cast<long long*>(step_dev));
  CUDA_TRY(cudaGetLastError());
  return SHIFU_OK;
}

extern "C" int shifu_publish_extras(ShifuCtx* c, const double* stats, float* extras, void* stream) {
  REQUIRE_PTR(c); REQUIRE_PTR(stats); REQUIRE_PTR(extras);
  const float ls = c->is_a1 ? c->a1.max_episode_length_s : c->abb.max_episode_length_s;
  const int nt = c->is_a1 ? c->a1.num_reward_terms : c->abb.num_reward_terms;
  publish_extras_kernel<<<1, 32, 0, S(stream)>>>(stats, extras, 1, 0, nullptr, ls, nt);
  CUDA_TRY(cudaGetLastError());
  return SHIFU_OK;
}

extern "C" int shifu_publish_extras_ring(ShifuCtx* c, const double* stats, float* ring, int32_t slots, int32_t slot,
                                         const int64_t* step_dev, void* stream) {
  REQUIRE_PTR(c); REQUIRE_PTR(stats); REQUIRE_PTR(ring);
  if (slots < 1) return fail(SHIFU_E_RANGE, "slots must be >= 1 (got %d)", slots);
  if (slot >= slots) return fail(SHIFU_E_RANGE, "slot %d outside the ring of %d", slot, slots);
  if (slot < 0 && step_dev == nullptr) return fail(SHIFU_E_NULL, "slot < 0 needs the device step counter");
  const float ls = c->is_a1 ? c->a1.max_episode_length_s : c->abb.max_episode_length_s;
  const int nt = c->is_a1 ? c->a1.num_reward_terms : c->abb.num_reward_terms;
  publish_extras_kernel<<<1, 32, 0, S(stream)>>>(stats, ring, slots, slot, reinterpret_cast<const long long*>(step_dev),
                                                 ls, nt);
  CUDA_TRY(cudaGetLastError());
  return SHIFU_OK;
}

extern "C" int shifu_terrain_generate(ShifuCtx* c, const ShifuTerrainDesc* d, const ShifuTerrainTile* tiles, int32_t n_tiles,
                                      const double* table, int32_t n_table, int16_t* map, double* origins, void* stream) {
  REQUIRE_PTR(c); REQUIRE_PTR(d); REQUIRE_PTR(tiles); REQUIRE_PTR(map); REQUIRE_PTR(origins);
  if (n_tiles <= 0 || n_tiles > d->num_rows * d->num_cols) return fail(SHIFU_E_RANGE, "n_tiles=%d out of range", n_tiles);
  if (n_table < 0 || (n_table > 0 && table == nullptr)) return fail(SHIFU_E_NULL, "table is NULL");
  if (d->width_px <= 1 || d->length_px <= 1 || d->width_px != d->length_px)
    return fail(SHIFU_E_RANGE, "tiles must be square (terrain.py:100-104 builds SubTerrain(width, width))");
  const int tot_rows = d->num_rows * d->length_px + 2 * d->border_px, tot_cols = d->num_cols * d->width_px + 2 * d->border_px;
  ShifuTerrainTile* d_tiles = nullptr; double* d_table = nullptr;
  CUDA_TRY(cudaMalloc(&d_tiles, sizeof(ShifuTerrainTile) * n_tiles));
  cudaError_t e = cudaMalloc(&d_table, sizeof(double) * (n_table > 0 ? n_table : 1));
  if (e != cudaSuccess) { cudaFree(d_tiles); return fail((int)e, "cudaMalloc: %s", cudaGetErrorString(e)); }
  cudaMemcpyAsync(d_tiles, tiles, sizeof(ShifuTerrainTile) * n_tiles, cudaMemcpyHostToDevice, S(stream));
  if (n_table > 0) cudaMemcpyAsync(d_table, table, sizeof(double) * n_table, cudaMemcpyHostToDevice, S(stream));
  cudaMemsetAsync(map, 0, sizeof(int16_t) * (size_t)tot_rows * tot_cols, S(stream));
  const int px = d->width_px * d->length_px;
  terrain_raster_kernel<<<dim3(n_tiles, (px + 255) / 256 > 8 ? 8 : (px + 255) / 256), 256, 0, S(stream)>>>(
      d_tiles, d_table, d->width_px, d->length_px, d->border_px, tot_cols, map);
  const double hs = d->horizontal_scale;
  const int wx1 = (int)((d->env_length / 2. - 1) / hs), wx2 = (int)((d->env_length / 2. + 1) / hs);
  const int wy1 = (int)((d->env_width / 2. - 1) / hs), wy2 = (int)((d->env_width / 2. + 1) / hs);
  terrain_origins_kernel<<<n_tiles, 32, 0, S(stream)>>>(d_tiles, map, d->width_px, d->length_px, d->border_px, tot_cols,
                                                        d->num_cols, d->env_length, d->env_width, wx1, wx2, wy1, wy2,
                                                        d->vertical_scale, origins);
  e = cudaGetLastError();
  cudaStreamSynchronize(S(stream));
  cudaFree(d_tiles); cudaFree(d_table);
  if (e != cudaSuccess) return fail((int)e, "terrain kernels: %s", cudaGetErrorString(e));
  return SHIFU_OK;
}

extern "C" int shifu_read_stats_host(ShifuCtx* c, double* host, void* stream) {
  REQUIRE_PTR(c); REQUIRE_PTR(host);
  CUDA_TRY(cudaMemcpyAsync(host, c->d_stats, sizeof(double) * SHIFU_NUM_STATS, cudaMemcpyDeviceToHost, S(stream)));
  CUDA_TRY(cudaStreamSynchronize(S(stream)));
  return SHIFU_OK;
}
```

### shifu_b200/csrc/common_kernels.cuh

```cuda
#pragma once
#include "exact_math.cuh"
#include "../../include/shifu_b200.h"

namespace shifu {

constexpr int COMPACT_THREADS = 256;
constexpr int COMPACT_PER_THREAD = 16;
constexpr int COMPACT_CHUNK = COMPACT_THREADS * COMPACT_PER_THREAD;

__global__ void __launch_bounds__(COMPACT_THREADS)
compact_ids_kernel(const unsigned char* __restrict__ flags, int n, long long* __restrict__ ids,
                   int* __restrict__ n_out, unsigned long long* __restrict__ chain,
                   unsigned* __restrict__ ticket, unsigned epoch) {
  __shared__ int s_warp[COMPACT_THREADS / 32];
  __shared__ int s_base, s_b;
  const int t = threadIdx.x, lane = t & 31, warp = t >> 5;
  if (t == 0) s_b = (int)atomicAdd(ticket, 1u);
  __syncthreads();
  const int b = s_b;
  const long long first = (long long)b * COMPACT_CHUNK + (long long)t * COMPACT_PER_THREAD;

  unsigned mask = 0;
  if (first + COMPACT_PER_THREAD <= n && ((reinterpret_cast<uintptr_t>(flags) & 15u) == 0)) {
    const uint4 v = __ldg(reinterpret_cast<const uint4*>(flags + first));
    const unsigned w[4] = {v.x, v.y, v.z, v.w};
#pragma unroll
    for (int i = 0; i < 4; ++i)
#pragma unroll
      for (int j = 0; j < 4; ++j)
        if ((w[i] >> (8 * j)) & 0xffu) mask |= 1u << (4 * i + j);
  } else {
#pragma unroll
    for (int i = 0; i < COMPACT_PER_THREAD; ++i)
      if (first + i < n && flags[first + i]) mask |= 1u << i;
  }
  const int cnt = __popc(mask);

  int incl = cnt;
#pragma unroll
  for (int o = 1; o < 32; o <<= 1) {
    const int v = __shfl_up_sync(0xffffffffu, incl, o);
    if (lane >= o) incl += v;
  }
  if (lane == 31) s_warp[warp] = incl;
  __syncthreads();
  int warp_base = 0, total = 0;
#pragma unroll
  for (int w = 0; w < COMPACT_THREADS / 32; ++w) {
    if (w < warp) warp_base += s_warp[w];
    total += s_warp[w];
  }
  if (t == 0) {
    __threadfence();
    atomicExch(chain + b, ((unsigned long long)epoch << 32) | (unsigned)total);
  }
  if (warp == 0) {
    int base = 0;
    for (int p0 = 0; p0 < b; p0 += 32) {
      const int p = p0 + lane;
      int c = 0;
      if (p < b) {
        unsigned long long v;
        do {
          v = *reinterpret_cast<volatile unsigned long long*>(chain + p);
        } while ((unsigned)(v >> 32) != epoch);
        c = (int)(unsigned)v;
      }
#pragma unroll
      for (int o = 16; o > 0; o >>= 1) c += __shfl_xor_sync(0xffffffffu, c, o);
      base += c;
    }
    if (lane == 0) {
      s_base = base;
      if (b == gridDim.x - 1) *n_out = base + total;
    }
  }
  __syncthreads();
  long long* out = ids + s_base + warp_base + (incl - cnt);
  unsigned m = mask;
  while (m) {
    const int i = __ffs(m) - 1;
    m &= m - 1;
    *out++ = first + i;
  }
  if (t == 0) {
    __threadfence();
    if (atomicAdd(ticket + 1, 1u) == gridDim.x - 1) { ticket[0] = 0u; ticket[1] = 0u; }
  }
}

__global__ void history_add_kernel(float* __restrict__ hist, const float* __restrict__ x, long long rows, int h) {
  for (long long i = blockIdx.x * (long long)blockDim.x + threadIdx.x; i < rows;
       i += (long long)gridDim.x * blockDim.x) {
    float* r = hist + i * h;
    for (int j = h - 1; j > 0; --j) r[j] = r[j - 1];
    r[0] = x[i];
  }
}

__global__ void clip_kernel(const float* __restrict__ in, float* __restrict__ out, long long n, float c) {
  const long long n4 = n >> 2;
  const bool vec = (((reinterpret_cast<uintptr_t>(in) | reinterpret_cast<uintptr_t>(out)) & 15u) == 0);
  const long long stride = (long long)gridDim.x * blockDim.x;
  const long long tid = blockIdx.x * (long long)blockDim.x + threadIdx.x;
  if (vec) {
    for (long long i = tid; i < n4; i += stride) {
      float4 v = reinterpret_cast<const float4*>(in)[i];
      v.x = clampf(v.x, -c, c); v.y = clampf(v.y, -c, c); v.z = clampf(v.z, -c, c); v.w = clampf(v.w, -c, c);
      reinterpret_cast<float4*>(out)[i] = v;
    }
    for (long long i = (n4 << 2) + tid; i < n; i += stride) out[i] = clampf(in[i], -c, c);
  } else {
    for (long long i = tid; i < n; i += stride) out[i] = clampf(in[i], -c, c);
  }
}

__global__ void collect_stats_kernel(double* __restrict__ acc, double* __restrict__ level_sum,
                                     double* __restrict__ out, int slots, int slot, double n_envs, long long* step_dev) {
  const int i = threadIdx.x;
  if (slot < 0) slot = (int)(*step_dev % slots);
  __syncwarp();
  if (i == 31 && step_dev != nullptr) *step_dev += 1;
  out += (size_t)slot * SHIFU_NUM_STATS;
  if (i >= SHIFU_NUM_STATS) return;
  double v = acc[i];
  acc[i] = 0.0;
  if (i == SHIFU_STAT_LEVEL_SUM) {
    v += *level_sum;
    *level_sum = v;
  }
  if (i == SHIFU_STAT_NENVS) v = n_envs;
  out[i] = v;
}

__global__ void publish_extras_kernel(const double* __restrict__ stats, float* __restrict__ ring, int slots, int slot,
                                      const long long* __restrict__ step_dev, float max_len_s, int n_terms) {
  const int i = threadIdx.x;
  if (i >= SHIFU_NUM_STATS) return;
  if (slot < 0) {
    slot = (int)((*step_dev - 1) % slots);
    stats += (size_t)slot * SHIFU_NUM_STATS;
  }
  const int prev = (slot + slots - 1) % slots;
  float* extras = ring + (size_t)slot * SHIFU_NUM_STATS;
  const float* old = ring + (size_t)prev * SHIFU_NUM_STATS;
  const double nreset = stats[SHIFU_STAT_NRESET];
  if (i == SHIFU_STAT_NRESET) { extras[i] = (float)nreset; return; }
  float v = old[i];
  if (nreset > 0.0) {
    if (i < SHIFU_MAX_REWARD_TERMS) {
      if (i < n_terms) v = div_rn((float)(stats[i] / nreset), max_len_s);
    } else if (i == SHIFU_STAT_LEVEL_SUM) {
      v = (float)(stats[i] / stats[SHIFU_STAT_NENVS]);
    } else if (i == SHIFU_STAT_SUCCESS) {
      v = (float)(stats[i] / nreset);
    }
  }
  extras[i] = v;
}

__global__ void __launch_bounds__(256) level_sum_kernel(const long long* __restrict__ levels, int n, double* __restrict__ out) {
  __shared__ double s[256];
  double a = 0.0;
  for (int i = blockIdx.x * blockDim.x + threadIdx.x; i < n; i += gridDim.x * blockDim.x) a += (double)levels[i];
  s[threadIdx.x] = a;
  __syncthreads();
  for (int o = blockDim.x / 2; o > 0; o >>= 1) {
    if ((int)threadIdx.x < o) s[threadIdx.x] += s[threadIdx.x + o];
    __syncthreads();
  }
  if (threadIdx.x == 0) atomicAdd(out, s[0]);
}

}
```

### shifu_b200/gym/autofuse.py

```python
from __future__ import annotations

from typing import Callable, Dict, Iterable, Optional

import torch

from shifu_b200 import hotpath, terms
from shifu_b200 import _native as nv


NotFusable = terms.NotFusable


def _code(fn):
    fn = getattr(fn, "__func__", fn)
    code = getattr(fn, "__code__", None)
    if code is None:
        raise NotFusable(f"{fn!r} is not a Python function")
    return code


def _names(fn) -> set:
    code = _code(fn)
    out = set(code.co_names)
    for c in code.co_consts:
        if hasattr(c, "co_names"):
            out |= set(c.co_names)
    return out


def _numbers(fn) -> set:
    return {float(c) for c in _code(fn).co_consts if isinstance(c, (int, float)) and not isinstance(c, bool)}


def _require(fn, what: str, names: Iterable[str] = (), numbers: Iterable[float] = ()):
    missing = set(names) - _names(fn)
    if missing:
        raise NotFusable(f"{what}: does not reference {sorted(missing)} — not the hook the fused kernel replaces")
    nums = _numbers(fn)
    for v in numbers:
        if not any(abs(v - c) <= 1e-12 * max(1.0, abs(v)) for c in nums):
            raise NotFusable(f"{what}: literal {v} not found (found {sorted(nums)})")


_AIR_STATE = {"swing_time", "feet_air_time", "last_contacts"}


def _require_reset_idx(cls) -> bool:
    clears = False
    for klass in cls.__mro__:
        fn = klass.__dict__.get("reset_idx")
        if fn is None:
            continue
        names = _names(fn)
        if {"update_terrain_curriculum", "sample_command"} <= names:
            return clears or bool(names & _AIR_STATE)
        other = names - _AIR_STATE - {"super", "reset_idx"}
        if other or not (names & _AIR_STATE):
            raise NotFusable(f"reset_idx: {klass.__name__}.reset_idx also touches {sorted(other)} — not a hook the "
                             "fused kernel replaces")
        clears = True
    raise NotFusable("reset_idx: does not reference ['sample_command', 'update_terrain_curriculum'] — not the hook "
                     "the fused kernel replaces")


def _overridden(obj, name: str, base) -> bool:
    return getattr(type(obj), name, None) is not getattr(base, name, None)


_close = terms.check_close



def fuse_a1(env, carry_body_frame: bool = True, rng_seed: int = 0x5EED):
    from shifu_b200.gym.sim_facade import TerrainGymEnv
    from shifu_b200.gym.vec_env import ShifuVecEnv
    from shifu_b200.units import LeggedRobot
    isg, cfg = env.isg_env, env.cfg
    rb = getattr(env, "robot", None)
    if not isinstance(isg, TerrainGymEnv) or not isinstance(rb, LeggedRobot):
        raise NotFusable("needs a TerrainGymEnv with a LeggedRobot")
    tc = cfg.terrain
    if (len(tc.measured_points_x), len(tc.measured_points_y)) != (nv.MAX_PX, nv.MAX_PY) or not tc.measure_heights:
        raise NotFusable("the fused kernel is compiled for the 17x11 measured-point grid")
    if (rb.num_dof, rb.num_bodies, cfg.num_actions, cfg.num_actions_history) != (12, 17, 12, 3):
        raise NotFusable("the fused kernel is compiled for 12 dofs / 17 bodies / 3 past actions")
    if cfg.num_obs != 72 + nv.MAX_PX * nv.MAX_PY or cfg.num_privileged_obs is not None:
        raise NotFusable("observation width is not 72 + 187")
    layout = rb.affine_root_layout()
    if layout is None:
        raise NotFusable("non-affine root_indices")
    for attr in ("command_buf", "terrain_levels", "contact_terminate_indices", "cmd_lin_vel_x", "cmd_lin_vel_y",
                 "cmd_ang_vel_yaw"):
        if not hasattr(env, attr):
            raise NotFusable(f"env.{attr} is missing")
    for attr in ("torques", "rand_force_buf", "leg_indices", "p_gains", "d_gains"):
        if not hasattr(rb, attr):
            raise NotFusable(f"robot.{attr} is missing")
    air_time_reset = _require_reset_idx(type(env))
    _require(type(env).sample_command, "sample_command",
             ("torch_rand_float", "cmd_lin_vel_x", "cmd_lin_vel_y", "cmd_ang_vel_yaw", "command_buf"))
    _require(type(env).update_terrain_curriculum, "update_terrain_curriculum",
             ("init_done", "norm", "base_pose", "env_origins", "env_length", "command_buf", "max_episode_length_s",
              "terrain_levels", "randint_like", "max_terrain_level", "where", "clip", "update_terrain_level"),
             (2, 0.5, 1, 0))
    if _overridden(env, "step", ShifuVecEnv):
        _require(type(env).step, "step", ("step",))
        scales = [c for c in _numbers(type(env).step) if c not in (0.0,)]
        if len(scales) != 1:
            raise NotFusable(f"step: expected exactly one action-scale literal, found {scales}")
    if _overridden(env, "episode_log", ShifuVecEnv):
        _require(type(env).episode_log, "episode_log", ("terrain_levels", "mean"))
    _require(type(rb).step, "robot.step",
             ("decimation", "p_gains", "default_dof_pos", "dof_pos", "d_gains", "dof_vel", "clip", "torque_limits",
              "_internal_motor_step", "simulate", "refresh_dof_state_tensor", "post_step", "apply_force_on_base",
              "rand_force_buf"))
    _require(type(rb)._reset_root_state, "robot._reset_root_state",
             ("root_indices", "root_state", "default_base_pose", "env_origins", "torch_rand_float"), (-1, 1, 2, 3, 7))
    force_fn = getattr(type(rb), "update_rand_force_buf", None) or type(rb).reset_idx
    _require(force_fn, "robot.update_rand_force_buf", ("rigid_body_dict", "rand_force_buf", "torch_rand_float"))
    forces = [c for c in _numbers(force_fn) if c > 0 and c != 3.0]
    if len(forces) != 1:
        raise NotFusable(f"robot.update_rand_force_buf: expected one force literal, found {forces}")
    base_name = [c for c in _code(force_fn).co_consts if isinstance(c, str)]
    force_body = rb.rigid_body_dict[base_name[0]] if base_name and base_name[0] in rb.rigid_body_dict else 0
    compiled = terms.compile_a1_terms(env, env.reward_functions)
    names = [t.name for t in compiled]
    obs = terms.compile_a1_obs(env)
    desc = a1_env_desc(env, [(t.name, t.code, t.p0, t.p1) for t in compiled], rng_seed=rng_seed, obs=obs,
                       action_scale=1.0,
                       force_body=force_body, push_force_max=float(forces[0]), air_time_reset=air_time_reset,
                       **terms.desc_extras(compiled))
    hp = a1_hot_path(env, desc, names, carry_body_frame, bool(getattr(cfg, "store_measured_heights", False)))
    hp.adopt(actions=env.actions, history=env.actions_recorder.history_buf, command=env.command_buf,
             torques=rb.torques, base_lin_vel=rb.base_lin_vel, base_ang_vel=rb.base_ang_vel,
             projected_gravity=rb.projected_gravity, ep_len=env.episode_length_buf, rand_force=rb.rand_force_buf,
             dof_targets=rb.dof_targets, terrain_levels=env.terrain_levels)
    air = terms.air_time_state(env)
    if air is not None and any(t.code == nv.REW_FEET_AIR_TIME for t in compiled):
        hp.adopt(swing_time=air[0], last_contacts=air[1])
    terms.verify_a1_terms(env, hp, env.reward_functions, compiled)
    terms.verify_a1_obs(env, obs)
    _check_a1_termination(env)
    return hp


def _check_a1_termination(env):
    rb, isg = env.robot, env.isg_env
    with terms.A1Probe(env) as pr:
        pr.randomize(4321)
        had = isg.__dict__.get("_measured_heights")
        isg.measured_heights = torch.randn(env.num_envs, isg.num_height_points, device=env.device)
        try:
            env.compute_termination()
            force = rb.contact_forces[:, int(env.contact_terminate_indices), :]
            contact = torch.norm(force, dim=-1) > 1.
            time_out = env.episode_length_buf > env.max_episode_length
            _close(env.time_out_buf, time_out, "compute_termination (time_out_buf)")
            _close(env.reset_buf, time_out | contact, "compute_termination (reset_buf)")
        finally:
            if had is None:
                del isg.measured_heights
            else:
                isg.measured_heights = had


def a1_env_desc(env, terms, *, rng_seed: int, force_body: int, push_force_max: float, **kw) -> nv.A1Desc:
    rb, isg, tc = env.robot, env.isg_env, env.cfg.terrain
    stride, offset = rb.affine_root_layout()
    desc = hotpath.a1_desc(
        env.num_envs, env_offset=env.env_offset, rng_seed=rng_seed, terms=terms,
        q0=tuple(rb.cfg.default_dof_pos), kp=tuple(float(v) for v in rb.p_gains.tolist()),
        kd=tuple(float(v) for v in rb.d_gains.tolist()), torque_limit=tuple(rb.torque_limits.tolist()),
        points_x=tuple(tc.measured_points_x), points_y=tuple(tc.measured_points_y),
        border_size=float(tc.border_size), horizontal_scale=tc.horizontal_scale, vertical_scale=tc.vertical_scale,
        max_episode_length=int(env.max_episode_length), max_episode_length_s=float(env.max_episode_length_s),
        default_root=tuple(rb.cfg.default_pos) + tuple(rb.cfg.default_quat), curriculum=tc.curriculum,
        max_terrain_level=isg.max_terrain_level, num_terrain_types=tc.num_cols, env_length=isg.terrain.env_length,
        base_body=int(env.contact_terminate_indices), leg_bodies=tuple(rb.leg_indices.tolist()),
        force_body=force_body, root_stride=stride, root_offset=offset,
        clip_actions=float(env.clip_actions), clip_obs=float(env.clip_obs), **kw)
    desc.push_force_max = push_force_max
    desc.cmd_low[0], desc.cmd_high[0] = env.cmd_lin_vel_x
    desc.cmd_low[1], desc.cmd_high[1] = env.cmd_lin_vel_y
    desc.cmd_low[2], desc.cmd_high[2] = env.cmd_ang_vel_yaw
    return desc


def a1_hot_path(env, desc: nv.A1Desc, names, carry_body_frame: bool, want_measured_heights: bool) -> hotpath.A1HotPath:
    isg = env.isg_env
    return hotpath.A1HotPath(desc, root_state=isg.root_state, dof_state=isg.dof_state, contact_state=isg.contact_state,
                             height_samples=isg.height_samples, terrain_origins=isg.terrain_origins,
                             terrain_types=isg.terrain_types, env_origins=isg.env_origins, terms=names,
                             carry_body_frame=carry_body_frame, want_measured_heights=want_measured_heights)


def bind_a1(env, hp):
    rb, isg = env.robot, env.isg_env
    env.actions, env.obs_buf, env.rew_buf, env.reset_buf = hp.actions, hp.obs_buf, hp.rew_buf, hp.reset_buf
    env._episode_length_buf = hp.ep_len
    env.time_out_buf, env.contact_terminate_buf = hp.time_out_buf, hp.contact_terminate_buf
    env.episode_rewards = hp.ep_sums
    env.command_buf, env.terrain_levels = hp.command, hp.terrain_levels
    env.actions_recorder.history_buf = hp.history
    rb.torques, rb.dof_targets, rb.rand_force_buf = hp.torques, hp.dof_targets, hp.rand_force
    rb.base_lin_vel, rb.base_ang_vel = hp.base_lin_vel, hp.base_ang_vel
    rb.projected_gravity, rb.gravity_vec = hp.projected_gravity, hp.gravity_vec
    isg.measured_heights = hp.measured_heights
    isg.__dict__["_heights_on_demand"] = hp.measured_heights is None
    env.extras.update(hp.extras())
    hp.body_frame()


def _resident_state(env) -> bool:
    sim = env.isg_env.sim
    return (getattr(sim, "provider", 0) is None and not getattr(env.isg_env.gym, "needs_indexed_resets", True)
            and getattr(env, "use_cuda_graph", True))


def a1_fused_step(env, hp, actions: torch.Tensor):
    gym, sim, rb, isg = env.isg_env.gym, env.isg_env.sim, env.robot, env.isg_env
    actions = actions.contiguous()
    env.common_step_counter += 1
    hp.step_counter = env.common_step_counter - 1
    if _resident_state(env):
        hp.graph_step(actions, isg.decimation, allreduce=env.stats_allreduce)
        env.extras.update(hp.extras())
        return env.obs_buf, env.privileged_obs_buf, env.rew_buf, env.reset_buf, env.extras
    for i in range(isg.decimation):
        hp.pd_torque(actions if i == 0 else None)
        rb._internal_motor_step(rb.torques)
        gym.simulate(sim)
        gym.refresh_dof_state_tensor(sim)
    if not hp.carry_body_frame:
        hp.body_frame()
    rb.apply_force_on_base(rb.rand_force_buf.view(-1, 3))
    isg.refresh_state()
    hp.post_physics()
    hp.finalize(env.stats_allreduce)
    push_resets(env, hp)
    env.extras.update(hp.extras())
    return env.obs_buf, env.privileged_obs_buf, env.rew_buf, env.reset_buf, env.extras



def fuse_abb(env, rng_seed: int = 0x5EED):
    from shifu_b200.units import ArmRobot, Box
    cfg = env.cfg
    rb = getattr(env, "robot", None)
    if not isinstance(rb, ArmRobot) or not all(isinstance(getattr(env, a, None), Box) for a in ("table", "cube", "goal")):
        raise NotFusable("needs an ArmRobot with table / cube / goal boxes")
    if cfg.num_obs != 6 or cfg.num_actions_history or cfg.num_privileged_obs is not None:
        raise NotFusable("observation is not the 6-column push-box observation")
    actors = [rb, env.table, env.cube, env.goal]
    layouts = [a.affine_root_layout() for a in actors]
    if any(l is None or l[0] != len(actors) for l in layouts):
        raise NotFusable("needs the 4-actor interleaved root layout")
    for box in (env.cube, env.goal):
        _require(type(box)._reset_root_state, f"{type(box).__name__}._reset_root_state",
                 ("root_indices", "uniform", "pos_range", "euler_range", "quat_from_euler_xyz", "root_state"), (3, 7, 13))
        if not (hasattr(box, "pos_range") and hasattr(box, "euler_range")):
            raise NotFusable("boxes without pos_range / euler_range")
    names = [fn.__name__ for fn in env.reward_functions]
    if names != ["reward_reaching", "reward_success"]:
        raise NotFusable(f"reward list {names} is not [reward_reaching, reward_success]")
    return abb_hot_path(env, rng_seed, _fit_abb_terms(env))


def abb_hot_path(env, rng_seed: int, term_params: Dict[str, tuple]) -> hotpath.AbbHotPath:
    isg, rb = env.isg_env, env.robot
    actors = [rb, env.table, env.cube, env.goal]
    names = [fn.__name__ for fn in env.reward_functions]
    desc = hotpath.abb_desc(env.num_envs, env_offset=env.env_offset, rng_seed=rng_seed, terms=names,
                            term_params=term_params)
    desc.num_actors = len(actors)
    desc.robot_actor, desc.table_actor, desc.cube_actor, desc.goal_actor = (a.affine_root_layout()[1] for a in actors)
    desc.num_bodies = sum(a.num_bodies for a in actors)
    desc.num_dof, desc.ee_body = rb.num_dof, int(rb.ee_indices[0])
    for i in range(3):
        desc.min_ee_pos[i], desc.max_ee_pos[i] = float(rb.cfg.min_ee_pos[i]), float(rb.cfg.max_ee_pos[i])
        desc.box_pos_low[i], desc.box_pos_high[i] = env.cube.pos_range["low"][i], env.cube.pos_range["high"][i]
    for i, v in enumerate(rb.cfg.default_dof_pos):
        desc.q0[i] = v
    for i, v in enumerate([*rb.cfg.default_pos, *rb.cfg.default_quat]):
        desc.robot_root[i] = v
    for i, v in enumerate([*env.table.cfg.default_pos, *env.table.cfg.default_quat]):
        desc.table_root[i] = v
    desc.goal_z = env.goal.pos_range["low"][2]
    desc.success_distance = term_params["reward_success"][1]
    desc.max_episode_length, desc.max_episode_length_s = int(env.max_episode_length), float(env.max_episode_length_s)
    desc.clip_obs = float(env.clip_obs)
    return hotpath.AbbHotPath(desc, root_state=isg.root_state, body_state=isg.body_state, dof_state=isg.dof_state,
                              terms=names)


def _fit_abb_terms(env) -> Dict[str, tuple]:
    import math
    isg, rb = env.isg_env, env.robot
    n = env.num_envs
    root = isg.root_state.view(n, -1, 13)
    body = isg.body_state.view(n, -1, 13)
    ee = int(rb.ee_indices[0])
    saved = (isg.root_state.clone(), isg.body_state.clone(), env.episode_length_buf.clone())
    attrs = {a: getattr(env, a, None) for a in ("obs_buf", "reset_buf", "time_out_buf", "success_buf")}

    def scene(cube_xy, goal_xy, ee_xy):
        root.zero_(); body.zero_()
        root[0, 2, :2] = torch.tensor(cube_xy, device=env.device)
        root[0, 3, :2] = torch.tensor(goal_xy, device=env.device)
        body[0, ee, :2] = torch.tensor(ee_xy, device=env.device)

    def bisect(f, lo, hi):
        for _ in range(50):
            mid = 0.5 * (lo + hi)
            lo, hi = (mid, hi) if f(mid) else (lo, mid)
        return 0.5 * (lo + hi)

    try:
        scene((0, 0), (0, 0), (0, 0))
        success_rew = float(env.reward_success()[0])
        thr = bisect(lambda d: (scene((0, 0), (d, 0), (0, 0)), float(env.reward_success()[0]) != 0.0)[1], 0.0, 1.0)
        thr = terms._snap(thr, type(env).is_success if hasattr(type(env), "is_success") else env.reward_success)
        ws = bisect(lambda d: (scene((0, 0), (0, 0), (d, 0)), float(env.reward_reaching()[0]) != 0.0)[1], 0.0, 1.0)
        ws = terms._snap(ws, env.reward_reaching)
        scene((0, 0), (0.1, 0), (0, 0))
        r = float(env.reward_reaching()[0])
        if not 0.0 < r < 1.0:
            raise NotFusable("reward_reaching is not [ee near cube] * exp(-d^2 / c)")
        width = terms._snap(-0.01 / math.log(r), env.reward_reaching)
        params = {"reward_reaching": (ws, width), "reward_success": (success_rew, thr)}
        g = torch.Generator(device=env.device).manual_seed(7)
        root.copy_(torch.randn(root.shape, generator=g, device=env.device) * 0.08)
        body.copy_(torch.randn(body.shape, generator=g, device=env.device) * 0.08)
        env.episode_length_buf.copy_(torch.randint(0, int(env.max_episode_length) + 20, (n,), generator=g,
                                                   device=env.device))
        cube, goal, eep = root[:, 2, :2], root[:, 3, :2], body[:, ee, :2]
        dist = torch.linalg.norm(goal - cube, dim=1)
        ee_dist = torch.linalg.norm(eep - cube, dim=1)
        _close(env.reward_reaching(), (ee_dist < ws).float() * torch.exp(-torch.square(dist) / width), "reward_reaching")
        _close(env.reward_success(), (dist < thr).float() * success_rew, "reward_success")
        env.compute_observations()
        _close(env.obs_buf, torch.cat([cube, goal, eep], dim=1), "compute_observations")
        env.compute_termination()
        lo = torch.tensor(rb.cfg.min_ee_pos[:2], device=env.device)
        hi = torch.tensor(rb.cfg.max_ee_pos[:2], device=env.device)
        out = ((cube < lo).any(1) | (cube > hi).any(1) | (eep < lo).any(1) | (eep > hi).any(1))
        time_out = env.episode_length_buf > env.max_episode_length
        _close(env.reset_buf, time_out | out | (dist < thr), "compute_termination")
        return params
    finally:
        isg.root_state.copy_(saved[0]); isg.body_state.copy_(saved[1]); env.episode_length_buf.copy_(saved[2])
        for a, v in attrs.items():
            if v is not None:
                setattr(env, a, v)


def bind_abb(env, hp):
    env.obs_buf, env.rew_buf, env.reset_buf = hp.obs_buf, hp.rew_buf, hp.reset_buf
    env._episode_length_buf, env.time_out_buf, env.success_buf = hp.ep_len, hp.time_out_buf, hp.success_buf
    env.episode_rewards = hp.ep_sums
    hp.dof_targets = env.robot.dof_targets
    hp._io = None
    env.extras.update(hp.extras())


def abb_fused_step(env, hp, actions: torch.Tensor):
    k = env.isg_env.kernels()
    k.clip(actions, env.clip_actions, out=env.actions)
    env.isg_env.step(env.actions)
    env.common_step_counter += 1
    hp.step_counter = env.common_step_counter - 1
    hp.post_physics()
    hp.finalize(env.stats_allreduce)
    push_resets(env, hp)
    env.extras.update(hp.extras())
    return env.obs_buf, env.privileged_obs_buf, env.rew_buf, env.reset_buf, env.extras



def push_resets(env, hp, env_ids: Optional[torch.Tensor] = None):
    if not getattr(env.isg_env.gym, "needs_indexed_resets", True):
        return
    ids = hp.reset_id_list() if env_ids is None else env_ids
    if len(ids):
        env.robot.push_dof_reset(ids)
        env.isg_env.push_root_reset(ids)


def fused_reset_idx(env, hp, env_ids: Optional[torch.Tensor]):
    hp.step_counter = env.common_step_counter
    hp.reset_idx(env_ids, env.stats_allreduce)
    push_resets(env, hp, torch.arange(env.num_envs, device=env.device) if env_ids is None else env_ids)
    env.extras.update(hp.extras())


RECIPES = {"a1": (fuse_a1, bind_a1, a1_fused_step), "abb": (fuse_abb, bind_abb, abb_fused_step)}


def install(env, recipe: str, hp):
    _, bind, step = RECIPES[recipe]
    bind(env, hp)
    env.hot, env._fusion, env._fusion_tried = hp, (recipe, hp, step), True
    env.reset_idx = lambda env_ids: fused_reset_idx(env, hp, env_ids)


def try_fuse(env, **kw):
    report = []
    for name, (fuse, _, _) in RECIPES.items():
        try:
            hp = fuse(env, **{k: v for k, v in kw.items() if k in fuse.__code__.co_varnames})
        except (NotFusable, terms.TermMismatch, KeyError, AttributeError) as exc:
            report.append(f"{name}: {exc}")
            continue
        install(env, name, hp)
        env.fusion_report = f"fused: {name}"
        return
    env.fusion_report = "user-hook mode — " + "; ".join(report)
```

### shifu_b200/hotpath.py

```python
from __future__ import annotations

import ctypes as C
import math
from dataclasses import dataclass
from typing import Dict, List, Optional, Sequence, Tuple

import numpy as np
import torch

from . import _native as nv

A1_TERM_CODES = {
    "tracking_lin_vel": nv.REW_TRACKING_LIN_VEL, "tracking_ang_vel": nv.REW_TRACKING_ANG_VEL,
    "stabilizing_base": nv.REW_STABILIZING_BASE, "smoothing_action": nv.REW_SMOOTHING_ACTION,
    "leg_collision": nv.REW_LEG_COLLISION, "torques_penalize": nv.REW_TORQUES,
    "lin_vel_z": nv.REW_LIN_VEL_Z, "ang_vel_xy": nv.REW_ANG_VEL_XY, "orientation": nv.REW_ORIENTATION,
    "dof_vel": nv.REW_DOF_VEL, "action_rate": nv.REW_ACTION_RATE, "base_height": nv.REW_BASE_HEIGHT,
    "dof_pos_limits": nv.REW_DOF_POS_LIMITS, "feet_air_time": nv.REW_FEET_AIR_TIME,
}
A1_DEFAULT_TERMS = ("tracking_lin_vel", "tracking_ang_vel", "stabilizing_base", "smoothing_action", "leg_collision",
                    "torques_penalize")
A1_TERM_PARAMS = {
    "tracking_lin_vel": (1.0, 0.25), "tracking_ang_vel": (0.5, 0.25), "stabilizing_base": (-2.0, -0.005),
    "smoothing_action": (-0.005, 0.0), "leg_collision": (-1.0, 0.1), "torques_penalize": (-2e-5, 0.0),
# ... 76 lines not shown
            leg_bodies=(2, 3, 6, 7, 10, 11, 14, 15), force_body=0, root_stride=1, root_offset=0,
            action_scale=0.5, clip_actions=1., clip_obs=100.,
            dof_pos_limits=None, feet_bodies=(4, 8, 12, 16), feet_contact_force=1.0, air_time_cmd_min=0.1,
            air_time_dt=0.02, air_time_reset=True, obs: Optional[ObsLayout] = None) -> nv.A1Desc:
    d = nv.A1Desc()
    d.abi_version = nv.ABI_VERSION
    d.num_envs, d.env_offset, d.rng_seed = num_envs, env_offset, rng_seed
    d.num_dof, d.num_bodies, d.num_hist, d.num_obs = 12, 17, 3, 259
    d.base_body, d.force_body = base_body, force_body
    d.num_leg_bodies = len(leg_bodies)
    for i, b in enumerate(leg_bodies):
        d.leg_bodies[i] = b
    d.root_stride, d.root_offset = root_stride, root_offset
    for i in range(12):
        d.q0[i], d.kp[i], d.kd[i], d.torque_limit[i] = q0[i], kp[i], kd[i], torque_limit[i]
    d.action_scale, d.clip_actions, d.clip_obs = action_scale, clip_actions, clip_obs
    d.num_points_x, d.num_points_y = len(points_x), len(points_y)
    if len(points_x) > nv.MAX_PX or len(points_y) > nv.MAX_PY:
        raise ValueError("measured-point grid larger than the compiled 17x11")
    for i, v in enumerate(points_x):
        d.points_x[i] = v
    for i, v in enumerate(points_y):
        d.points_y[i] = v
    d.border_size, d.horizontal_scale, d.vertical_scale = border_size, horizontal_scale, vertical_scale
    d.height_offset, d.height_clip = 0.5, 1.0
    d.max_episode_length, d.max_episode_length_s = int(max_episode_length), max_episode_length_s
    d.contact_term_force = 1.0
    for i in range(7):
        d.default_root[i] = default_root[i]
    d.reset_xy_range, d.push_force_max = 1.0, 5.0
    for i in range(3):
        d.cmd_low[i], d.cmd_high[i] = -1.0, 1.0
    d.curriculum = int(bool(curriculum))
    d.max_terrain_level, d.num_terrain_types = max_terrain_level, num_terrain_types
    d.level_up_distance, d.level_down_factor = env_length / 2, 0.5
    for i in range(12):
        lo, hi = dof_pos_limits[i] if dof_pos_limits is not None else (-3.0e38, 3.0e38)
        d.dof_pos_limit_low[i], d.dof_pos_limit_high[i] = lo, hi
    if len(feet_bodies) > 4:
        raise ValueError("at most 4 feet")
    d.num_feet = len(feet_bodies)
    for i, b in enumerate(feet_bodies):
        d.feet_bodies[i] = int(b)
    d.feet_contact_force, d.air_time_cmd_min, d.air_time_dt = feet_contact_force, air_time_cmd_min, air_time_dt
    d.air_time_reset = int(bool(air_time_reset))
    comp = compile_reward_terms(list(terms), A1_TERM_CODES, {**A1_TERM_PARAMS, **(term_params or {})})
    d.num_reward_terms = len(comp)
    for i, (code, p0, p1) in enumerate(comp):
        d.reward_terms[i] = code
        d.reward_params[i][0], d.reward_params[i][1] = p0, p1
    if obs is not None and not obs.is_reference():
        d.obs_layout = 1
        for i, name in enumerate(obs.slots):
            d.obs_vec_src[i] = OBS_SOURCES[name]
        for j, v in enumerate(obs.scales):
            d.obs_scale[j] = v
        d.obs_height_scale = obs.height_scale
        for j, v in enumerate(obs.noise):
            d.obs_noise[j] = v
        d.obs_height_noise = obs.height_noise
    return d


class _Ctx:

    def __init__(self, device: torch.device, a1: Optional[nv.A1Desc] = None, abb: Optional[nv.AbbDesc] = None):
        self.lib = nv.load()
        if device.type != "cuda":
            raise nv.ShifuNativeError(nv.E_NODEVICE, f"device {device} is not CUDA: the shifu_b200 hot "
                                                     "path has no CPU fallback")
        self.handle = C.c_void_p()
        idx = device.index if device.index is not None else torch.cuda.current_device()
        nv.check(self.lib.shifu_ctx_create(idx, C.byref(a1) if a1 is not None else None,
                                           C.byref(abb) if abb is not None else None, C.byref(self.handle)))

    def close(self):
        if getattr(self, "handle", None) is not None and self.handle.value:
            self.lib.shifu_ctx_destroy(self.handle)
            self.handle = C.c_void_p()

    def __del__(self):
        try:
            self.close()
        except Exception:
            pass


class EnvKernels:

    def __init__(self, device, num_envs: int):
        self.lib = nv.load()
        self.device = torch.device(device)
        if self.device.type != "cuda":
            raise nv.ShifuNativeError(nv.E_NODEVICE, f"device {device} is not CUDA: the shifu_b200 kernels "
                                                     "have no CPU fallback")
        self.n = num_envs
        self.handle = C.c_void_p()
        idx = self.device.index if self.device.index is not None else torch.cuda.current_device()
        nv.check(self.lib.shifu_ctx_create_util(idx, num_envs, C.byref(self.handle)))
        self._ids = torch.zeros(num_envs, device=self.device, dtype=torch.long)
        self._cnt = torch.zeros(1, device=self.device, dtype=torch.int32)

    def __del__(self):
        try:
            if self.handle.value:
                self.lib.shifu_ctx_destroy(self.handle)
        except Exception:
            pass

    def nonzero(self, flags: torch.Tensor) -> torch.Tensor:
        f = flags if flags.dtype in (torch.bool, torch.uint8) else (flags != 0)
        f = f.contiguous()
        nv.check(self.lib.shifu_compact_reset_ids(self.handle, nv.ptr(f), f.numel(), nv.ptr(self._ids),
                                                  nv.ptr(self._cnt), nv.current_stream()))
        return self._ids[: int(self._cnt.item())].clone()

    def history_add(self, history_buf: torch.Tensor, x: torch.Tensor):
        n, a, h = history_buf.shape
        nv.check(self.lib.shifu_history_add(self.handle, nv.ptr(history_buf), nv.ptr(x.contiguous()), n, a, h,
                                            nv.current_stream()))

    def clip(self, x: torch.Tensor, c: float, out: Optional[torch.Tensor] = None) -> torch.Tensor:
        x = x.contiguous()
        out = torch.empty_like(x) if out is None else out
        nv.check(self.lib.shifu_clip(self.handle, nv.ptr(x), nv.ptr(out), x.numel(), float(c), nv.current_stream()))
        return out

    def arm_ik(self, *, body_state, num_bodies: int, ee_body: int, jacobian, ee_link: int, dof_state, num_dof: int,
               dof_targets, goal_pose=None, actions=None, ee_velocity: float = 0.0, dt: float = 0.0,
               min_ee_pos=(0., 0., 0.), max_ee_pos=(0., 0., 0.), tar_quat=(0., 0., 0., 1.), damping: float = 0.05):
        io = nv.ArmIkIO()
        if not (jacobian.is_contiguous() and jacobian.dim() == 4 and jacobian.shape[2] == 6):
            raise ValueError("jacobian must be the contiguous (N, links, 6, dofs) gym tensor")
        io.body_state, io.jacobian, io.dof_state = nv.ptr(body_state), nv.ptr(jacobian), nv.ptr(dof_state)
        io.goal_pose = nv.ptr(goal_pose.contiguous()) if goal_pose is not None else None
        io.actions = nv.ptr(actions.contiguous()) if actions is not None else None
        io.dof_targets = nv.ptr(dof_targets)
        io.num_bodies, io.ee_body, io.num_links, io.ee_link = num_bodies, ee_body, jacobian.shape[1], ee_link
        io.num_dof, io.ee_velocity, io.dt, io.damping = num_dof, ee_velocity, dt, damping
        for i in range(3):
            io.min_ee_pos[i], io.max_ee_pos[i] = float(min_ee_pos[i]), float(max_ee_pos[i])
        for i in range(4):
            io.tar_quat[i] = float(tar_quat[i])
        nv.check(self.lib.shifu_arm_ik(self.handle, C.byref(io), jacobian.shape[0], nv.current_stream()))
        return dof_targets

    def camera_gather(self, *, height: int, width: int, normalize_color: bool, color=None, depth=None, seg=None,
                      flow=None):
        io = nv.CameraGatherIO()
        io.height, io.width, io.normalize_color = height, width, int(bool(normalize_color))
        n = None
        for name, pair in (("color", color), ("depth", depth), ("seg", seg), ("flow", flow)):
            if pair is None:
                continue
            table, out = pair
            if table.dtype != torch.int64 or not table.is_contiguous():
                raise ValueError(f"{name}: the pointer table must be a contiguous int64 tensor")
            n = table.numel() if n is None else n
            if table.numel() != n or out.shape[0] != n or not out.is_contiguous():
                raise ValueError(f"{name}: table / output size mismatch")
            setattr(io, name + "_src", nv.ptr(table))
            setattr(io, name + "_out", nv.ptr(out))
        if n is not None:
            nv.check(self.lib.shifu_camera_gather(self.handle, C.byref(io), n, nv.current_stream()))

    def body_frame(self, root_state, n, stride, offset, lin, ang, pg, gvec=None):
        nv.check(self.lib.shifu_body_frame(self.handle, nv.ptr(root_state), n, stride, offset, nv.ptr(lin),
                                           nv.ptr(ang), nv.ptr(pg), nv.ptr(gvec), nv.current_stream()))


EXTRAS_SLOTS = 64


class _StepStats:

    def _init_stats(self, dev):
        self.stats_ring = torch.zeros(EXTRAS_SLOTS, nv.NUM_STATS, device=dev, dtype=torch.double)
        self.extras_ring = torch.zeros(EXTRAS_SLOTS, nv.NUM_STATS, device=dev, dtype=torch.float)
        self._stats_slot = 0
        self._side = None
        self._pending = None
        self._slot_events = {}

    @property
    def slot(self) -> int:
        return self.step_counter % EXTRAS_SLOTS

    @property
    def stats(self) -> torch.Tensor:
        return self.stats_ring[self._stats_slot]

    @property
    def extras_arr(self) -> torch.Tensor:
        return self.extras_ring[self.slot]

    def wait_stats(self):
        if self._pending is not None:
            torch.cuda.current_stream().wait_event(self._pending)
            self._pending = None

    def _slot_guard(self):
        done = self._slot_events.pop(self.slot, None)
        if done is not None:
            torch.cuda.current_stream().wait_event(done)

    def _collect(self, advance_step_dev: bool):
        self._stats_slot = self.slot
        if not torch.cuda.is_current_stream_capturing():
            self._slot_guard()
        nv.check(self.lib.shifu_collect_stats_ring(self.ctx.handle, nv.ptr(self.stats_ring), EXTRAS_SLOTS,
                                                   -1 if advance_step_dev else self.slot,
                                                   nv.ptr(self.step_dev) if advance_step_dev else None,
                                                   nv.current_stream()))

    def _publish(self, allreduce, from_step_dev: bool = False):
        lib, h, slot = self.lib, self.ctx.handle, self.slot
        st = self.stats_ring[slot]
        if allreduce is None:
            nv.check(lib.shifu_publish_extras_ring(h, nv.ptr(self.stats_ring) if from_step_dev else nv.ptr(st),
                                                   nv.ptr(self.extras_ring), EXTRAS_SLOTS, -1 if from_step_dev else slot,
                                                   nv.ptr(self.step_dev), nv.current_stream()))
            return
        if self._side is None:
            self._side = torch.cuda.Stream(device=self.device)
        self._side.wait_stream(torch.cuda.current_stream())
        with torch.cuda.stream(self._side):
            allreduce(st)
            nv.check(lib.shifu_publish_extras_ring(h, nv.ptr(st), nv.ptr(self.extras_ring), EXTRAS_SLOTS, slot, None,
                                                   nv.current_stream()))
            self._pending = torch.cuda.Event()
            self._pending.record(self._side)
            self._slot_events[slot] = self._pending

    def _finalize_stats(self, allreduce, advance_step_dev: bool):
        self._collect(advance_step_dev)
        self._publish(allreduce, from_step_dev=advance_step_dev)


class HeightScan:

    def __init__(self, desc: nv.A1Desc, height_samples: torch.Tensor, root_state: torch.Tensor):
        self.ctx = _Ctx(root_state.device, a1=desc)
        self.lib = self.ctx.lib
        self.root_state = root_state
        self.height_samples = height_samples.contiguous()
        self.out = torch.zeros(desc.num_envs, desc.num_points_x * desc.num_points_y, device=root_state.device)
        nv.check(self.lib.shifu_set_height_map(self.ctx.handle, nv.ptr(self.height_samples),
                                               self.height_samples.shape[0], self.height_samples.shape[1],
                                               nv.current_stream()))

    def run(self, cell_idx: Optional[torch.Tensor] = None) -> torch.Tensor:
        nv.check(self.lib.shifu_get_heights(self.ctx.handle, nv.ptr(self.root_state), nv.ptr(self.out),
                                            nv.ptr(cell_idx), nv.current_stream()))
        return self.out


class A1HotPath(_StepStats):

    def __init__(self, desc: nv.A1Desc, *, root_state, dof_state, contact_state, height_samples,
                 terrain_origins, terrain_types, env_origins, terms: Sequence[str] = A1_DEFAULT_TERMS,
                 carry_body_frame: bool = False, want_measured_heights: bool = True):
        dev = root_state.device
        self.device = dev
        self.desc = desc
        self.n = n = desc.num_envs
        self.terms = list(terms)
        self.ctx = _Ctx(dev, a1=desc)
        self.lib = self.ctx.lib
        f = dict(device=dev, dtype=torch.float)
        self.root_state, self.dof_state, self.contact_state = root_state, dof_state, contact_state
        self.height_samples = height_samples.to(dev).contiguous()
        assert self.height_samples.dtype == torch.int16
        self.terrain_origins = terrain_origins.to(**f).contiguous()
        self.terrain_types = terrain_types.to(dev, torch.long).contiguous()
        self.env_origins = env_origins
        self.actions = torch.zeros(n, 12, **f)
        self.torques = torch.zeros(n, 12, **f)
        self.history = torch.zeros(n, 12, 3, **f)
        self.command = torch.zeros(n, 3, **f)
        self.ep_len = torch.zeros(n, device=dev, dtype=torch.long)
        self.ep_sums = {k: torch.zeros(n, **f) for k in self.terms}
        self.base_lin_vel = torch.zeros(n, 3, **f)
        self.base_ang_vel = torch.zeros(n, 3, **f)
        self.projected_gravity = torch.zeros(n, 3, **f)
        self.gravity_vec = torch.tensor([0., 0., -1.], **f).repeat(n, 1)
        self.terrain_levels = torch.zeros(n, device=dev, dtype=torch.long)
        self.dof_targets = torch.zeros(n, 12, **f)
        self.rand_force = torch.zeros(n, 17, 3, **f)
        self.obs_buf = torch.zeros(n, 259, **f)
        self.rew_buf = torch.zeros(n, **f)
        self.reset_buf = torch.ones(n, device=dev, dtype=torch.bool)
        self.time_out_buf = torch.zeros(n, device=dev, dtype=torch.bool)
        self.contact_terminate_buf = torch.zeros(n, device=dev, dtype=torch.bool)
        self.measured_heights = torch.zeros(n, 187, **f) if want_measured_heights else None
        self.reset_ids = torch.zeros(n, device=dev, dtype=torch.long)
        self.n_reset = torch.zeros(1, device=dev, dtype=torch.int32)
        self.step_dev = torch.zeros(1, device=dev, dtype=torch.long)
        self.swing_time = torch.zeros(n, max(desc.num_feet, 1), **f)
        self.last_contacts = torch.zeros(n, max(desc.num_feet, 1), device=dev, dtype=torch.bool)
        self.step_counter = 0
        self._pd_substep = -1
        self._init_stats(dev)
        self._graph, self._graph_warm, self._dev_step, self._graph_actions = None, 0, -1, None
        self._fork = None
        self.carry_body_frame = carry_body_frame
        self._io = None
        nv.check(self.lib.shifu_set_height_map(self.ctx.handle, nv.ptr(self.height_samples),
                                               self.height_samples.shape[0], self.height_samples.shape[1],
                                               nv.current_stream()))
        self.sync_level_sum()

    def _build_io(self, use_step_dev: bool) -> nv.A1StepIO:
        io = nv.A1StepIO()
        p = nv.ptr
        io.root_state, io.dof_state, io.contact_state = p(self.root_state), p(self.dof_state), p(self.contact_state)
        io.actions, io.torques, io.history, io.command = p(self.actions), p(self.torques), p(self.history), p(self.command)
        io.ep_len = p(self.ep_len)
        for i, k in enumerate(self.terms):
            io.ep_sums[i] = p(self.ep_sums[k])
        io.base_lin_vel, io.base_ang_vel = p(self.base_lin_vel), p(self.base_ang_vel)
        io.projected_gravity = p(self.projected_gravity)
        io.env_origins, io.terrain_levels = p(self.env_origins), p(self.terrain_levels)
        io.terrain_types, io.terrain_origins = p(self.terrain_types), p(self.terrain_origins)
        io.dof_targets, io.rand_force = p(self.dof_targets), p(self.rand_force)
        io.obs_buf, io.rew_buf, io.reset_buf = p(self.obs_buf), p(self.rew_buf), p(self.reset_buf)
        io.time_out_buf, io.contact_term_buf = p(self.time_out_buf), p(self.contact_terminate_buf)
        io.measured_heights = p(self.measured_heights)
        io.step = self.step_counter
        io.step_dev = p(self.step_dev) if use_step_dev else None
        io.swing_time, io.last_contacts = p(self.swing_time), p(self.last_contacts)
        io.carry_body_frame = int(self.carry_body_frame)
        return io

    def io(self, use_step_dev: bool = False) -> nv.A1StepIO:
        if self._io is None or bool(self._io.step_dev) != use_step_dev:
            self._io = self._build_io(use_step_dev)
        self._io.step = self.step_counter
        self._io.carry_body_frame = int(self.carry_body_frame)
        return self._io

    def invalidate_io(self):
        self._io = None

    _ADOPTABLE = ("actions", "torques", "history", "command", "ep_len", "base_lin_vel", "base_ang_vel",
                  "projected_gravity", "terrain_levels", "dof_targets", "rand_force", "swing_time", "last_contacts")

    def adopt(self, **tensors):
        for name, t in tensors.items():
            if name not in self._ADOPTABLE:
                raise KeyError(f"{name} cannot be adopted")
            mine = getattr(self, name)
            if t.shape != mine.shape or t.dtype != mine.dtype or t.device != mine.device or not t.is_contiguous():
                raise ValueError(f"{name}: expected contiguous {tuple(mine.shape)} {mine.dtype} on {mine.device}, got "
                                 f"{tuple(t.shape)} {t.dtype} on {t.device}")
            setattr(self, name, t)
        self.invalidate_io()
        if "terrain_levels" in tensors:
            self.sync_level_sum()

    def eval_terms(self) -> torch.Tensor:
        out = torch.empty(len(self.terms), self.n, device=self.device, dtype=torch.float)
        nv.check(self.lib.shifu_a1_eval_terms(self.ctx.handle, C.byref(self.io(False)), nv.ptr(out), nv.current_stream()))
        return out

    def sync_level_sum(self):
        nv.check(self.lib.shifu_set_level_sum(self.ctx.handle, nv.ptr(self.terrain_levels), nv.current_stream()))

    def pd_torque(self, raw_actions: Optional[torch.Tensor] = None):
        s = nv.current_stream()
        self._pd_substep = 0 if raw_actions is not None else self._pd_substep + 1
        if raw_actions is not None:
            nv.check(self.lib.shifu_pd_torque(self.ctx.handle, nv.ptr(raw_actions), nv.ptr(self.actions),
                                              nv.ptr(self.dof_state), nv.ptr(self.torques), self._pd_substep, s))
        else:
            nv.check(self.lib.shifu_pd_torque(self.ctx.handle, nv.ptr(self.actions), None,
                                              nv.ptr(self.dof_state), nv.ptr(self.torques), self._pd_substep, s))

    def body_frame(self):
        nv.check(self.lib.shifu_body_frame(self.ctx.handle, nv.ptr(self.root_state), self.n,
                                           self.desc.root_stride, self.desc.root_offset,
                                           nv.ptr(self.base_lin_vel), nv.ptr(self.base_ang_vel),
                                           nv.ptr(self.projected_gravity), nv.ptr(self.gravity_vec),
                                           nv.current_stream()))

    def get_heights(self, out: Optional[torch.Tensor] = None, cell_idx: Optional[torch.Tensor] = None):
        out = self.measured_heights if out is None else out
        nv.check(self.lib.shifu_get_heights(self.ctx.handle, nv.ptr(self.root_state), nv.ptr(out),
                                            nv.ptr(cell_idx), nv.current_stream()))
        return out

    def post_physics(self, use_step_dev: bool = False):
        self.step_counter += 1
        nv.check(self.lib.shifu_a1_post_physics(self.ctx.handle, C.byref(self.io(use_step_dev)), nv.current_stream()))

    def compact(self):
        nv.check(self.lib.shifu_compact_reset_ids(self.ctx.handle, nv.ptr(self.reset_buf), self.n,
                                                  nv.ptr(self.reset_ids), nv.ptr(self.n_reset), nv.current_stream()))

    def reset_idx(self, env_ids: Optional[torch.Tensor], allreduce=None):
        n_ids = self.n if env_ids is None else int(env_ids.numel())
        if env_ids is not None:
            env_ids = env_ids.to(self.device, torch.long).contiguous()
        self.wait_stats()
        nv.check(self.lib.shifu_a1_reset_idx(self.ctx.handle, C.byref(self.io(False)), nv.ptr(env_ids), n_ids,
                                             nv.current_stream()))
        if n_ids > 0 and self.carry_body_frame:
            self.body_frame()
        if n_ids > 0 or allreduce is not None:
            self._finalize_stats(allreduce, False)

    def finalize(self, allreduce=None, advance_step_dev: bool = False):
        self.compact()
        self._finalize_stats(allreduce, advance_step_dev)

    def step_resident(self, raw_actions: torch.Tensor, decimation: int = 4, use_step_dev: bool = False,
                      allreduce=None, publish: bool = True):
        self.pd_torque(raw_actions)
        for _ in range(decimation - 1):
            self.pd_torque()
        if not self.carry_body_frame:
            self.body_frame()
        self.post_physics(use_step_dev)
        main = torch.cuda.current_stream()
        if torch.cuda.is_current_stream_capturing():
            if self._fork is None:
                self._fork = torch.cuda.Stream(device=self.device)
            self._fork.wait_stream(main)
            with torch.cuda.stream(self._fork):
                self.compact()
        else:
            self.compact()
        self._collect(use_step_dev)
        if publish:
            self._publish(allreduce, from_step_dev=use_step_dev)
        if torch.cuda.is_current_stream_capturing():
            main.wait_stream(self._fork)

    def graph_step(self, raw_actions: torch.Tensor, decimation: int = 4, allreduce=None):
        if self._graph is None:
            if self._graph_warm < 2:
                self._graph_warm += 1
                return self.step_resident(raw_actions, decimation, allreduce=allreduce)
            if self._graph_actions is None:
                self._graph_actions = torch.empty_like(raw_actions)
            if raw_actions.data_ptr() != self._graph_actions.data_ptr():
                self._graph_actions.copy_(raw_actions)
            self.step_dev.fill_(self.step_counter + 1)
            torch.cuda.synchronize(self.device)
            graph = torch.cuda.CUDAGraph()
            before = self.step_counter
            with torch.cuda.graph(graph):
                self.step_resident(self._graph_actions, decimation, use_step_dev=True, publish=allreduce is None)
            self.step_counter = before
            self._graph, self._graph_decimation, self._dev_step = graph, decimation, before + 1
            self._graph_publishes = allreduce is None
        if decimation != self._graph_decimation or raw_actions.shape != self._graph_actions.shape or \
                self._graph_publishes != (allreduce is None):
            raise ValueError("graph_step was captured for another decimation / action shape / collective mode")
        if self._dev_step != self.step_counter + 1:
            self.step_dev.fill_(self.step_counter + 1)
        if raw_actions.data_ptr() != self._graph_actions.data_ptr():
            self._graph_actions.copy_(raw_actions)
        self.step_counter += 1
        self._stats_slot = self.slot
        self._slot_guard()
        self._graph.replay()
        self._dev_step = self.step_counter + 1
        if allreduce is not None:
            self._publish(allreduce)

    def action_input(self) -> torch.Tensor:
        if self._graph_actions is None:
            self._graph_actions = torch.zeros(self.n, 12, device=self.device)
        return self._graph_actions

    def extras(self) -> Dict:
        arr = self.extras_arr
        ep = {k: arr[i] for i, k in enumerate(self.terms)}
        ep["terrain_levels"] = arr[nv.STAT_LEVEL_SUM]
        return {"episode": ep, "time_outs": self.time_out_buf}

    def reset_id_list(self) -> torch.Tensor:
        return self.reset_ids[: int(self.n_reset.item())]


def abb_desc(num_envs: int, *, env_offset: int = 0, rng_seed: int = 0x5EED,
             terms: Sequence[str] = tuple(ABB_TERM_CODES), term_params: Optional[Dict[str, tuple]] = None) -> nv.AbbDesc:
    d = nv.AbbDesc()
    d.abi_version = nv.ABI_VERSION
    d.num_envs, d.env_offset, d.rng_seed = num_envs, env_offset, rng_seed
    d.num_actors, d.num_bodies, d.num_dof, d.ee_body = 4, 10, 6, 6
    d.robot_actor, d.table_actor, d.cube_actor, d.goal_actor = 0, 1, 2, 3
    for i, v in enumerate((-0.2, -0.2, 0.11)):
        d.min_ee_pos[i] = v
    for i, v in enumerate((0.2, 0.2, 0.14)):
        d.max_ee_pos[i] = v
    for i, v in enumerate((0., 0.6437, 0.1748, 0., 0.7541, 0.)):
        d.q0[i] = v
    for i, v in enumerate((-0.48, 0, 0, 0, 0, 0, 1)):
        d.robot_root[i] = v
    for i, v in enumerate((0, 0, 0.05, 0, 0, 0, 1)):
        d.table_root[i] = v
    for i, (lo, hi) in enumerate(((-0.1, 0.1), (-0.1, 0.1), (0.125, 0.125))):
        d.box_pos_low[i], d.box_pos_high[i] = lo, hi
    d.goal_z = 0.1
    d.success_distance = 0.02
    d.max_episode_length, d.max_episode_length_s, d.clip_obs = 200, 20., 10.
    comp = compile_reward_terms(list(terms), ABB_TERM_CODES, {**ABB_TERM_PARAMS, **(term_params or {})})
    d.num_reward_terms = len(comp)
    for i, (code, p0, p1) in enumerate(comp):
        d.reward_terms[i] = code
        d.reward_params[i][0], d.reward_params[i][1] = p0, p1
    return d


class AbbHotPath(_StepStats):
    def __init__(self, desc: nv.AbbDesc, *, root_state, body_state, dof_state,
                 terms: Sequence[str] = tuple(ABB_TERM_CODES)):
        dev = root_state.device
        self.device, self.desc, self.n = dev, desc, desc.num_envs
        n = self.n
        self.terms = list(terms)
        self.ctx = _Ctx(dev, abb=desc)
        self.lib = self.ctx.lib
        f = dict(device=dev, dtype=torch.float)
        self.root_state, self.body_state, self.dof_state = root_state, body_state, dof_state
        self.dof_targets = torch.zeros(n, 6, **f)
        self.ep_len = torch.zeros(n, device=dev, dtype=torch.long)
        self.ep_sums = {k: torch.zeros(n, **f) for k in self.terms}
        self.obs_buf = torch.zeros(n, 6, **f)
        self.rew_buf = torch.zeros(n, **f)
        self.reset_buf = torch.ones(n, device=dev, dtype=torch.bool)
        self.time_out_buf = torch.zeros(n, device=dev, dtype=torch.bool)
        self.success_buf = torch.zeros(n, device=dev, dtype=torch.bool)
        self.reset_ids = torch.zeros(n, device=dev, dtype=torch.long)
        self.n_reset = torch.zeros(1, device=dev, dtype=torch.int32)
        self.step_dev = torch.zeros(1, device=dev, dtype=torch.long)
        self.step_counter = 0
        self._init_stats(dev)
        self._io = None

    def io(self, use_step_dev: bool = False) -> nv.AbbStepIO:
        if self._io is None or bool(self._io.step_dev) != use_step_dev:
            io = nv.AbbStepIO()
            p = nv.ptr
            io.root_state, io.body_state, io.dof_state = p(self.root_state), p(self.body_state), p(self.dof_state)
            io.dof_targets, io.ep_len = p(self.dof_targets), p(self.ep_len)
            for i, k in enumerate(self.terms):
                io.ep_sums[i] = p(self.ep_sums[k])
            io.obs_buf, io.rew_buf, io.reset_buf = p(self.obs_buf), p(self.rew_buf), p(self.reset_buf)
            io.time_out_buf, io.success_buf = p(self.time_out_buf), p(self.success_buf)
            io.step_dev = p(self.step_dev) if use_step_dev else None
            self._io = io
        self._io.step = self.step_counter
        return self._io

    def post_physics(self, use_step_dev: bool = False):
        self.step_counter += 1
        nv.check(self.lib.shifu_abb_post_physics(self.ctx.handle, C.byref(self.io(use_step_dev)), nv.current_stream()))

    def finalize(self, allreduce=None, advance_step_dev: bool = False):
        nv.check(self.lib.shifu_compact_reset_ids(self.ctx.handle, nv.ptr(self.reset_buf), self.n,
                                                  nv.ptr(self.reset_ids), nv.ptr(self.n_reset), nv.current_stream()))
        self._finalize_stats(allreduce, advance_step_dev)

    def reset_idx(self, env_ids: Optional[torch.Tensor], allreduce=None):
        n_ids = self.n if env_ids is None else int(env_ids.numel())
        if env_ids is not None:
            env_ids = env_ids.to(self.device, torch.long).contiguous()
        self.wait_stats()
        nv.check(self.lib.shifu_abb_reset_idx(self.ctx.handle, C.byref(self.io(False)), nv.ptr(env_ids), n_ids,
                                              nv.current_stream()))
        if n_ids > 0 or allreduce is not None:
            self._finalize_stats(allreduce, False)

    def step_resident(self, use_step_dev: bool = False, allreduce=None):
        self.post_physics(use_step_dev)
        self.finalize(allreduce, advance_step_dev=use_step_dev)

    def extras(self) -> Dict:
        arr = self.extras_arr
        ep = {k: arr[i] for i, k in enumerate(self.terms)}
        ep["success_rate"] = arr[nv.STAT_SUCCESS]
        return {"episode": ep, "time_outs": self.time_out_buf}

    def reset_id_list(self) -> torch.Tensor:
        return self.reset_ids[: int(self.n_reset.item())]
```

Before: 1.957 billion.

## Fuse reset-id compaction and stats finalization into the post-physics kernel

Reset-id stream compaction now happens inside the post-physics kernels. Each tile publishes its reset count with a tag, and later tiles compute a decoupled look-back prefix, so the separate compact kernel and its forked stream go away. The last CTA to retire (tracked by a ticket) collects the stats, publishes the extras ring and advances step_dev, replacing the separate collect and publish kernels. This removes several small launches per step. In exchange, launches become cooperative and blocks spin-wait on earlier tiles' status, which adds tag and epoch management and a risk of stalls.

```diff
diff --git a/include/shifu_b200.h b/include/shifu_b200.h
--- a/include/shifu_b200.h
+++ b/include/shifu_b200.h
@@ -7,7 +7,7 @@
 extern "C" {
 #endif
 
-#define SHIFU_ABI_VERSION 5
+#define SHIFU_ABI_VERSION 6
 
 #define SHIFU_MAX_DOF 12
 #define SHIFU_MAX_LEG_BODIES 8
@@ -156,10 +156,16 @@
   uint8_t* contact_term_buf;
   float* measured_heights;
   int64_t step;
-  const int64_t* step_dev;
+  int64_t* step_dev;
   float* swing_time;
   uint8_t* last_contacts;
   int32_t carry_body_frame;
+  int64_t* reset_ids;
+  int32_t* n_reset;
+  double* stats_ring;
+  float* extras_ring;
+  int32_t stats_slots;
+  int32_t stats_slot;
 } ShifuA1StepIO;
 
 typedef struct ShifuAbbDesc {
diff --git a/shifu_b200/_native.py b/shifu_b200/_native.py
--- a/shifu_b200/_native.py
+++ b/shifu_b200/_native.py
@@ -5,7 +5,7 @@
 from typing import Optional
 
 MAX_DOF, MAX_LEG, MAX_PX, MAX_PY, MAX_TERMS, NUM_STATS = 12, 8, 17, 11, 8, 16
-ABI_VERSION = 5
+ABI_VERSION = 6
 OBS_HEAD = 72
 
 REW_TRACKING_LIN_VEL, REW_TRACKING_ANG_VEL, REW_STABILIZING_BASE, REW_SMOOTHING_ACTION = 0, 1, 2, 3
@@ -66,6 +66,8 @@
         ("time_out_buf", C.c_void_p), ("contact_term_buf", C.c_void_p), ("measured_heights", C.c_void_p),
         ("step", C.c_int64), ("step_dev", C.c_void_p), ("swing_time", C.c_void_p), ("last_contacts", C.c_void_p),
         ("carry_body_frame", C.c_int32),
+        ("reset_ids", C.c_void_p), ("n_reset", C.c_void_p), ("stats_ring", C.c_void_p), ("extras_ring", C.c_void_p),
+        ("stats_slots", C.c_int32), ("stats_slot", C.c_int32),
     ]
 
 
diff --git a/shifu_b200/csrc/a1_fused.cuh b/shifu_b200/csrc/a1_fused.cuh
--- a/shifu_b200/csrc/a1_fused.cuh
+++ b/shifu_b200/csrc/a1_fused.cuh
@@ -1,5 +1,6 @@
 #pragma once
 #include "a1_kernels.cuh"
+#include "common_kernels.cuh"
 
 namespace shifu {
 
@@ -199,6 +200,9 @@
   const int t = threadIdx.x, warp = t >> 5, lane = t & 31;
   const long long step = (io.step_dev != nullptr) ? *io.step_dev : io.step;
   const float bx = k.px[t % A1_NX], by = k.py[(t / A1_NX) % A1_NY];
+  const unsigned tag = (io.reset_ids != nullptr) ? launch_tag(k.ticket) : 0u;
+  int incl = (io.reset_ids != nullptr && first_tile > 0) ? *io.n_reset : 0;
+  const int last_tile = (k.n + A1_TILE - 1) / A1_TILE - 1;
 
   for (int e0 = (first_tile + blockIdx.x) * A1_TILE; e0 < k.n; e0 += gridDim.x * A1_TILE) {
     const int ne = min(A1_TILE, k.n - e0);
@@ -276,6 +280,15 @@
           if (j < k.n_terms) io.ep_sums[j][ge] = esum[j];
         s.zb[lane] = sub_rn(s.root[lane][2], k.h_off);
       }
+      if (io.reset_ids != nullptr) {
+        const unsigned m = __ballot_sync(0xffffffffu, reset);
+        const int tile = e0 / A1_TILE;
+        if (lane == 0) tile_publish(k.tile_status, tile, tag, __popc(m));
+        const int pre = tile_prefix(k.tile_status, tag, tile, first_tile, gridDim.x, incl, lane);
+        tile_write_ids(reinterpret_cast<long long*>(io.reset_ids), pre, m, e0, lane);
+        incl = pre + __popc(m);
+        if (lane == 0 && tile == last_tile) *io.n_reset = incl;
+      }
       a1_log_sums(k, reset, st_sum, level_delta, lane);
     }
     __syncthreads();
@@ -347,6 +360,12 @@
     }
     __syncthreads();
   }
+  if ((io.reset_ids != nullptr || io.stats_ring != nullptr) && warp == 0) {
+    const bool last = __shfl_sync(0xffffffffu, lane == 0 ? retire_cta(k.ticket) : false, 0);
+    if (last && io.stats_ring != nullptr)
+      finish_step_warp(k.stats, k.stats + SHIFU_NUM_STATS, (double)k.n, io.stats_ring, io.extras_ring, io.stats_slots,
+                       io.stats_slot, reinterpret_cast<long long*>(io.step_dev), k.max_len_s, k.n_terms, lane);
+  }
 }
 
 __global__ void __launch_bounds__(A1_THREADS)
diff --git a/shifu_b200/csrc/a1_fused_tma.cuh b/shifu_b200/csrc/a1_fused_tma.cuh
--- a/shifu_b200/csrc/a1_fused_tma.cuh
+++ b/shifu_b200/csrc/a1_fused_tma.cuh
@@ -2,6 +2,7 @@
 #include "a1_fused.cuh"
 #include "scan_pairs.cuh"
 #include "tma_pipe.cuh"
+#include "common_kernels.cuh"
 
 namespace shifu {
 
@@ -16,6 +17,8 @@
 constexpr int V3_THREADS = V3_B_THREADS + V3_C_THREADS + V3_DMA_THREADS;
 constexpr int V3_SCAN_BASE = V3_B_THREADS;
 constexpr int V3_DMA_BASE = V3_B_THREADS + V3_C_THREADS;
+constexpr int V3_ID_DEFER = 2;
+static_assert(V3_ID_DEFER + 1 <= 4, "reset-mask ring");
 constexpr uint32_t V3_OBS_CHUNK_BYTES = 8 * A1_OBS * 4;
 
 struct alignas(128) V3In {
@@ -38,6 +41,9 @@
   float4 sB[4][A1_TILE / 2];
   float4 sC[4][A1_TILE / 2];
   float rterm[2][SHIFU_MAX_REWARD_TERMS][A1_TILE];
+  unsigned rmask[4];
+  unsigned tag;
+  int incl;
   uint64_t full_in[V3_STAGES], e_done[V3_STAGES], b_done[V3_STAGES], h_done[V3_STAGES];
 };
 
@@ -85,6 +91,8 @@
       pipe::mbar_init(&s.h_done[b], V3_C_THREADS);
     }
     pipe::fence_barrier_init();
+    s.tag = launch_tag(k.ticket);
+    s.incl = 0;
   }
   __syncthreads();
 
@@ -115,6 +123,18 @@
 
   if (t < V3_B_THREADS) {
     const int warp = t >> 5, lane = t & 31;
+    auto compact_tile = [&](int jd) {
+      const int tile = first + jd * stride;
+      const unsigned m = s.rmask[jd & 3];
+      const int pre = tile_prefix(k.tile_status, s.tag, tile, 0, stride, s.incl, lane);
+      tile_write_ids(reinterpret_cast<long long*>(io.reset_ids), pre, m, (long long)tile * A1_TILE, lane);
+      __syncwarp();
+      if (lane == 0) {
+        s.incl = pre + __popc(m);
+        if (tile == num_tiles - 1) *io.n_reset = pre + __popc(m);
+      }
+      __syncwarp();
+    };
 
     for (int j = 0; j < my_tiles; ++j) {
       const int b = j % V3_STAGES;
@@ -135,7 +155,10 @@
         s.rterm[j & 1][q][lane] = a1_reward_term<HAS_EXTRA>(k.terms[q], q, k.rp[q][0], k.rp[q][1], k, in, lane, io, ge);
       }
       pipe::named_barrier(1, V3_B_THREADS);
-      if (warp >= 2) continue;
+      if (warp >= 2) {
+        if (io.reset_ids != nullptr && j >= V3_ID_DEFER) compact_tile(j - V3_ID_DEFER);
+        continue;
+      }
 
       long long len = in.ep_len[lane] + 1;
       const bool contact_term = force_exceeds(&in.contact[lane][k.base_body * 3], k.contact_thr_sq);
@@ -163,6 +186,13 @@
         io.reset_buf[ge] = reset ? 1 : 0;
         io.time_out_buf[ge] = time_out ? 1 : 0;
         io.contact_term_buf[ge] = contact_term ? 1 : 0;
+        if (io.reset_ids != nullptr) {
+          const unsigned m = __ballot_sync(0xffffffffu, reset);
+          if (lane == 0) {
+            s.rmask[j & 3] = m;
+            tile_publish(k.tile_status, first + j * stride, s.tag, __popc(m));
+          }
+        }
         if (reset)
           a1_reset_env<true, 2>(k, io, step, (int)ge, nullptr, nullptr, nullptr, cmd, esum, len, st_sum, level_delta,
                                 0.0f, 0.0f, 0.0f, 0, 0);
@@ -197,6 +227,15 @@
       }
       pipe::mbar_arrive(&s.b_done[b]);
     }
+    if (io.reset_ids == nullptr && io.stats_ring == nullptr) return;
+    pipe::named_barrier(1, V3_B_THREADS);
+    if (warp != 2) return;
+    if (io.reset_ids != nullptr)
+      for (int jd = my_tiles - V3_ID_DEFER > 0 ? my_tiles - V3_ID_DEFER : 0; jd < my_tiles; ++jd) compact_tile(jd);
+    const bool last = __shfl_sync(0xffffffffu, lane == 0 ? retire_cta(k.ticket) : false, 0);
+    if (last && io.stats_ring != nullptr && (long long)num_tiles * A1_TILE == k.n)
+      finish_step_warp(k.stats, k.stats + SHIFU_NUM_STATS, (double)k.n, io.stats_ring, io.extras_ring, io.stats_slots,
+                       io.stats_slot, reinterpret_cast<long long*>(io.step_dev), k.max_len_s, k.n_terms, lane);
     return;
   }
 
diff --git a/shifu_b200/csrc/a1_kernels.cuh b/shifu_b200/csrc/a1_kernels.cuh
--- a/shifu_b200/csrc/a1_kernels.cuh
+++ b/shifu_b200/csrc/a1_kernels.cuh
@@ -48,6 +48,8 @@
   int trows, tcols;
   int band_w;
   double* stats;
+  unsigned* tile_status;
+  unsigned* ticket;
   float neg_zero;
 };
 
diff --git a/shifu_b200/csrc/capi.cu b/shifu_b200/csrc/capi.cu
--- a/shifu_b200/csrc/capi.cu
+++ b/shifu_b200/csrc/capi.cu
@@ -58,9 +58,9 @@
   short* d_table = nullptr;
   double* d_stats = nullptr;
   unsigned long long* d_chain = nullptr;
+  unsigned* d_tile_status = nullptr;
   unsigned* d_ticket = nullptr;
   int chain_len = 0;
-  unsigned epoch = 0;
   int a1_grid = 0;
   int a1_occ = 0;
   int tma_occ = 0;
@@ -305,8 +305,11 @@
   c->chain_len = (n + COMPACT_CHUNK - 1) / COMPACT_CHUNK + 1;
   if (e == cudaSuccess) e = cudaMalloc(&c->d_chain, sizeof(unsigned long long) * c->chain_len);
   if (e == cudaSuccess) e = cudaMemset(c->d_chain, 0, sizeof(unsigned long long) * c->chain_len);
-  if (e == cudaSuccess) e = cudaMalloc(&c->d_ticket, sizeof(unsigned) * 2);
-  if (e == cudaSuccess) e = cudaMemset(c->d_ticket, 0, sizeof(unsigned) * 2);
+  if (e == cudaSuccess) e = cudaMalloc(&c->d_ticket, sizeof(unsigned) * TICKET_WORDS);
+  if (e == cudaSuccess) e = cudaMemset(c->d_ticket, 0, sizeof(unsigned) * TICKET_WORDS);
+  const size_t tiles_n = (size_t)(n + A1_TILE - 1) / A1_TILE;
+  if (e == cudaSuccess && c->is_a1) e = cudaMalloc(&c->d_tile_status, sizeof(unsigned) * tiles_n);
+  if (e == cudaSuccess && c->is_a1) e = cudaMemset(c->d_tile_status, 0, sizeof(unsigned) * tiles_n);
   if (e == cudaSuccess && c->is_a1) {
     const void* variants[4] = {
         (const void*)a1_post_physics_kernel<false, false>, (const void*)a1_post_physics_kernel<true, false>,
@@ -348,6 +351,8 @@
     return rc;
   }
   c->a1k.stats = c->d_stats;
+  c->a1k.tile_status = c->d_tile_status;
+  c->a1k.ticket = c->d_ticket;
   c->abbk.stats = c->d_stats;
   CUDA_TRY(cudaDeviceSynchronize());
   *out = c;
@@ -359,6 +364,7 @@
   cudaFree(c->d_table);
   cudaFree(c->d_stats);
   cudaFree(c->d_chain);
+  cudaFree(c->d_tile_status);
   cudaFree(c->d_ticket);
   delete c;
   return SHIFU_OK;
@@ -473,8 +479,24 @@
   for (int j = 0; j < c->a1.num_reward_terms; ++j)
     if (io->ep_sums[j] == nullptr) return fail(SHIFU_E_NULL, "ep_sums[%d] is NULL", j);
   REQUIRE_ALIGNED(io->dof_state, 16);
+  if (io->reset_ids != nullptr) REQUIRE_PTR(io->n_reset);
+  if (io->extras_ring != nullptr && io->stats_ring == nullptr) return fail(SHIFU_E_NULL, "extras_ring needs stats_ring");
+  if (io->stats_ring != nullptr) {
+    if (io->stats_slots < 1 || io->stats_slot >= io->stats_slots)
+      return fail(SHIFU_E_RANGE, "stats_slot %d outside the ring of %d", io->stats_slot, io->stats_slots);
+    if (io->stats_slot < 0 && io->step_dev == nullptr) return fail(SHIFU_E_NULL, "stats_slot < 0 needs step_dev");
+  }
   const bool exact = c->a1k.exact_div != 0;
   const int n = c->a1.num_envs;
+  cudaLaunchAttribute coop{};
+  coop.id = cudaLaunchAttributeCooperative;
+  coop.val.cooperative = 1;
+  auto launch = [&](const void* fn, dim3 grid, dim3 block, void** args, size_t smem) {
+    cudaLaunchConfig_t cfg{};
+    cfg.gridDim = grid; cfg.blockDim = block; cfg.dynamicSmemBytes = smem; cfg.stream = S(stream);
+    cfg.attrs = &coop; cfg.numAttrs = 1;
+    return cudaLaunchKernelExC(&cfg, fn, args);
+  };
 
   auto al16 = [](const void* p) { return (reinterpret_cast<uintptr_t>(p) & 15u) == 0; };
   const bool can_tma = c->use_tma && c->grid_symmetric && c->a1k.root_stride == 1 && c->a1k.root_offset == 0 && al16(io->root_state) &&
@@ -493,22 +515,17 @@
     int tiles_arg = full_tiles;
     void* args[4] = {(void*)&c->a1k, const_cast<ShifuA1StepIO*>(io), (void*)&tiles_arg, (void*)&c->a1o};
     const int variant = (c->obs_custom ? 8 : 0) + (c->a1o.noisy ? 8 : 0) + (exact ? 4 : 0) + (mrow ? 2 : 0) + (extra ? 1 : 0);
-    CUDA_TRY(cudaLaunchKernel(a1_tma_variants()[variant], grid, block, args, smem, S(stream)));
+    CUDA_TRY(launch(a1_tma_variants()[variant], grid, block, args, smem));
   }
   const int tiles = (n + A1_TILE - 1) / A1_TILE - full_tiles;
   if (tiles > 0) {
     const int cap = c->sm_count * (c->a1_occ > 0 ? c->a1_occ : 1);
     const dim3 grid(tiles < cap ? tiles : cap), block(A1_THREADS);
-    const A1K& k = c->a1k;
-    const A1Obs& o = c->a1o;
-    if (o.noisy) {
-      if (exact) a1_post_physics_kernel<true, true><<<grid, block, 0, S(stream)>>>(k, *io, o, full_tiles);
-      else a1_post_physics_kernel<false, true><<<grid, block, 0, S(stream)>>>(k, *io, o, full_tiles);
-    } else {
-      if (exact) a1_post_physics_kernel<true, false><<<grid, block, 0, S(stream)>>>(k, *io, o, full_tiles);
-      else a1_post_physics_kernel<false, false><<<grid, block, 0, S(stream)>>>(k, *io, o, full_tiles);
-    }
-    CUDA_TRY(cudaGetLastError());
+    int first_tile = full_tiles;
+    void* args[4] = {(void*)&c->a1k, const_cast<ShifuA1StepIO*>(io), (void*)&c->a1o, (void*)&first_tile};
+    const void* fn = c->a1o.noisy ? (exact ? (const void*)a1_post_physics_kernel<true, true> : (const void*)a1_post_physics_kernel<false, true>)
+                                  : (exact ? (const void*)a1_post_physics_kernel<true, false> : (const void*)a1_post_physics_kernel<false, false>);
+    CUDA_TRY(launch(fn, grid, block, args, 0));
   }
   return SHIFU_OK;
 }
@@ -546,9 +563,8 @@
   if (n <= 0) return fail(SHIFU_E_RANGE, "n must be > 0 (got %d)", n);
   const int chunks = (n + COMPACT_CHUNK - 1) / COMPACT_CHUNK;
   if (chunks > c->chain_len) return fail(SHIFU_E_RANGE, "n=%d exceeds the ctx's num_envs", n);
-  c->epoch += 1;
   compact_ids_kernel<<<chunks, COMPACT_THREADS, 0, S(stream)>>>(flags, n, reinterpret_cast<long long*>(ids), n_out,
-                                                               c->d_chain, c->d_ticket, c->epoch);
+                                                               c->d_chain, c->d_ticket);
   CUDA_TRY(cudaGetLastError());
   return SHIFU_OK;
 }
diff --git a/shifu_b200/csrc/common_kernels.cuh b/shifu_b200/csrc/common_kernels.cuh
--- a/shifu_b200/csrc/common_kernels.cuh
+++ b/shifu_b200/csrc/common_kernels.cuh
@@ -8,16 +8,37 @@
 constexpr int COMPACT_PER_THREAD = 16;
 constexpr int COMPACT_CHUNK = COMPACT_THREADS * COMPACT_PER_THREAD;
 
+constexpr int TICKET_NEXT = 0, TICKET_RETIRED = 1, TICKET_EPOCH = 2, TICKET_WORDS = 3;
+
+__device__ __forceinline__ unsigned launch_tag(const unsigned* ticket) {
+  return *reinterpret_cast<const volatile unsigned*>(ticket + TICKET_EPOCH) + 1u;
+}
+
+__device__ __forceinline__ bool retire_cta(unsigned* ticket) {
+  __threadfence();
+  if (atomicAdd(ticket + TICKET_RETIRED, 1u) != gridDim.x - 1) return false;
+  __threadfence();
+  ticket[TICKET_NEXT] = 0u;
+  ticket[TICKET_RETIRED] = 0u;
+  ticket[TICKET_EPOCH] += 1u;
+  return true;
+}
+
 __global__ void __launch_bounds__(COMPACT_THREADS)
 compact_ids_kernel(const unsigned char* __restrict__ flags, int n, long long* __restrict__ ids,
                    int* __restrict__ n_out, unsigned long long* __restrict__ chain,
-                   unsigned* __restrict__ ticket, unsigned epoch) {
+                   unsigned* __restrict__ ticket) {
   __shared__ int s_warp[COMPACT_THREADS / 32];
   __shared__ int s_base, s_b;
+  __shared__ unsigned s_epoch;
   const int t = threadIdx.x, lane = t & 31, warp = t >> 5;
-  if (t == 0) s_b = (int)atomicAdd(ticket, 1u);
+  if (t == 0) {
+    s_b = (int)atomicAdd(ticket + TICKET_NEXT, 1u);
+    s_epoch = launch_tag(ticket);
+  }
   __syncthreads();
   const int b = s_b;
+  const unsigned epoch = s_epoch;
   const long long first = (long long)b * COMPACT_CHUNK + (long long)t * COMPACT_PER_THREAD;
 
   unsigned mask = 0;
@@ -83,10 +104,7 @@
     m &= m - 1;
     *out++ = first + i;
   }
-  if (t == 0) {
-    __threadfence();
-    if (atomicAdd(ticket + 1, 1u) == gridDim.x - 1) { ticket[0] = 0u; ticket[1] = 0u; }
-  }
+  if (t == 0) retire_cta(ticket);
 }
 
 __global__ void history_add_kernel(float* __restrict__ hist, const float* __restrict__ x, long long rows, int h) {
@@ -115,6 +133,33 @@
   }
 }
 
+__device__ __forceinline__ double collect_stat(int i, double* acc, double* level_sum, double n_envs) {
+  double v = __ldcg(acc + i);
+  acc[i] = 0.0;
+  if (i == SHIFU_STAT_LEVEL_SUM) {
+    v += *level_sum;
+    *level_sum = v;
+  }
+  if (i == SHIFU_STAT_NENVS) v = n_envs;
+  return v;
+}
+
+__device__ __forceinline__ float extras_value(int i, double st_i, double nreset, double nenvs, float old, float max_len_s,
+                                              int n_terms) {
+  if (i == SHIFU_STAT_NRESET) return (float)nreset;
+  float v = old;
+  if (nreset > 0.0) {
+    if (i < SHIFU_MAX_REWARD_TERMS) {
+      if (i < n_terms) v = div_rn((float)(st_i / nreset), max_len_s);
+    } else if (i == SHIFU_STAT_LEVEL_SUM) {
+      v = (float)(st_i / nenvs);
+    } else if (i == SHIFU_STAT_SUCCESS) {
+      v = (float)(st_i / nreset);
+    }
+  }
+  return v;
+}
+
 __global__ void collect_stats_kernel(double* __restrict__ acc, double* __restrict__ level_sum,
                                      double* __restrict__ out, int slots, int slot, double n_envs, long long* step_dev) {
   const int i = threadIdx.x;
@@ -123,14 +168,7 @@
   if (i == 31 && step_dev != nullptr) *step_dev += 1;
   out += (size_t)slot * SHIFU_NUM_STATS;
   if (i >= SHIFU_NUM_STATS) return;
-  double v = acc[i];
-  acc[i] = 0.0;
-  if (i == SHIFU_STAT_LEVEL_SUM) {
-    v += *level_sum;
-    *level_sum = v;
-  }
-  if (i == SHIFU_STAT_NENVS) v = n_envs;
-  out[i] = v;
+  out[i] = collect_stat(i, acc, level_sum, n_envs);
 }
 
 __global__ void publish_extras_kernel(const double* __restrict__ stats, float* __restrict__ ring, int slots, int slot,
@@ -142,21 +180,63 @@
     stats += (size_t)slot * SHIFU_NUM_STATS;
   }
   const int prev = (slot + slots - 1) % slots;
-  float* extras = ring + (size_t)slot * SHIFU_NUM_STATS;
-  const float* old = ring + (size_t)prev * SHIFU_NUM_STATS;
-  const double nreset = stats[SHIFU_STAT_NRESET];
-  if (i == SHIFU_STAT_NRESET) { extras[i] = (float)nreset; return; }
-  float v = old[i];
-  if (nreset > 0.0) {
-    if (i < SHIFU_MAX_REWARD_TERMS) {
-      if (i < n_terms) v = div_rn((float)(stats[i] / nreset), max_len_s);
-    } else if (i == SHIFU_STAT_LEVEL_SUM) {
-      v = (float)(stats[i] / stats[SHIFU_STAT_NENVS]);
-    } else if (i == SHIFU_STAT_SUCCESS) {
-      v = (float)(stats[i] / nreset);
-    }
-  }
-  extras[i] = v;
+  ring[(size_t)slot * SHIFU_NUM_STATS + i] =
+      extras_value(i, stats[i], stats[SHIFU_STAT_NRESET], stats[SHIFU_STAT_NENVS],
+                   ring[(size_t)prev * SHIFU_NUM_STATS + i], max_len_s, n_terms);
+}
+
+__device__ __forceinline__ void finish_step_warp(double* acc, double* level_sum, double n_envs, double* stats, float* extras,
+                                                 int slots, int slot, long long* step_dev, float max_len_s, int n_terms,
+                                                 int lane) {
+  if (slot < 0) slot = (int)(*step_dev % slots);
+  const int i = lane < SHIFU_NUM_STATS ? lane : 0;
+  const double v = (lane < SHIFU_NUM_STATS) ? collect_stat(i, acc, level_sum, n_envs) : 0.0;
+  if (lane < SHIFU_NUM_STATS) stats[(size_t)slot * SHIFU_NUM_STATS + i] = v;
+  const double nreset = __shfl_sync(0xffffffffu, v, SHIFU_STAT_NRESET);
+  const double nenvs = __shfl_sync(0xffffffffu, v, SHIFU_STAT_NENVS);
+  if (extras != nullptr && lane < SHIFU_NUM_STATS) {
+    const int prev = (slot + slots - 1) % slots;
+    extras[(size_t)slot * SHIFU_NUM_STATS + i] =
+        extras_value(i, v, nreset, nenvs, extras[(size_t)prev * SHIFU_NUM_STATS + i], max_len_s, n_terms);
+  }
+  if (lane == 0 && step_dev != nullptr) *step_dev += 1;
+}
+
+constexpr unsigned TILE_TAG_MASK = (1u << 26) - 1u;
+
+__device__ __forceinline__ void tile_publish(unsigned* status, int tile, unsigned tag, unsigned count) {
+  asm volatile("st.relaxed.gpu.global.u32 [%0], %1;" ::"l"(status + tile), "r"(((tag & TILE_TAG_MASK) << 6) | count)
+               : "memory");
+}
+
+__device__ __forceinline__ unsigned tile_status_load(const unsigned* status, int tile) {
+  unsigned v;
+  asm volatile("ld.relaxed.gpu.global.u32 %0, [%1];" : "=r"(v) : "l"(status + tile) : "memory");
+  return v;
+}
+
+__device__ __noinline__ int tile_prefix(const unsigned* status, unsigned tag, int tile, int lo, int stride, int below,
+                                           int lane) {
+  const unsigned want = tag & TILE_TAG_MASK;
+  const int from = max(lo, tile - stride + 1);
+  int sum = 0;
+  for (int t0 = tile - 1 - lane; t0 >= from; t0 -= 4 * 32) {
+    unsigned v[4];
+#pragma unroll
+    for (int u = 0; u < 4; ++u) v[u] = (t0 - 32 * u >= from) ? tile_status_load(status, t0 - 32 * u) : (want << 6);
+#pragma unroll
+    for (int u = 0; u < 4; ++u) {
+      while ((v[u] >> 6) != want) v[u] = tile_status_load(status, t0 - 32 * u);
+      sum += (int)(v[u] & 63u);
+    }
+  }
+#pragma unroll
+  for (int o = 16; o > 0; o >>= 1) sum += __shfl_xor_sync(0xffffffffu, sum, o);
+  return below + sum;
+}
+
+__device__ __forceinline__ void tile_write_ids(long long* ids, int prefix, unsigned mask, long long e0, int lane) {
+  if ((mask >> lane) & 1u) ids[prefix + __popc(mask & ((1u << lane) - 1u))] = e0 + lane;
 }
 
 __global__ void __launch_bounds__(256) level_sum_kernel(const long long* __restrict__ levels, int n, double* __restrict__ out) {
diff --git a/shifu_b200/gym/autofuse.py b/shifu_b200/gym/autofuse.py
--- a/shifu_b200/gym/autofuse.py
+++ b/shifu_b200/gym/autofuse.py
@@ -235,7 +235,7 @@
         hp.body_frame()
     rb.apply_force_on_base(rb.rand_force_buf.view(-1, 3))
     isg.refresh_state()
-    hp.post_physics()
+    hp.post_physics(publish=env.stats_allreduce is None)
     hp.finalize(env.stats_allreduce)
     push_resets(env, hp)
     env.extras.update(hp.extras())
diff --git a/shifu_b200/hotpath.py b/shifu_b200/hotpath.py
--- a/shifu_b200/hotpath.py
+++ b/shifu_b200/hotpath.py
@@ -402,7 +402,6 @@
         self._pd_substep = -1
         self._init_stats(dev)
         self._graph, self._graph_warm, self._dev_step, self._graph_actions = None, 0, -1, None
-        self._fork = None
         self.carry_body_frame = carry_body_frame
         self._io = None
         nv.check(self.lib.shifu_set_height_map(self.ctx.handle, nv.ptr(self.height_samples),
@@ -430,6 +429,8 @@
         io.step_dev = p(self.step_dev) if use_step_dev else None
         io.swing_time, io.last_contacts = p(self.swing_time), p(self.last_contacts)
         io.carry_body_frame = int(self.carry_body_frame)
+        io.reset_ids, io.n_reset = p(self.reset_ids), p(self.n_reset)
+        io.stats_ring, io.stats_slots = p(self.stats_ring), EXTRAS_SLOTS
         return io
 
     def io(self, use_step_dev: bool = False) -> nv.A1StepIO:
@@ -489,13 +490,15 @@
                                             nv.ptr(cell_idx), nv.current_stream()))
         return out
 
-    def post_physics(self, use_step_dev: bool = False):
+    def post_physics(self, use_step_dev: bool = False, publish: bool = True):
         self.step_counter += 1
-        nv.check(self.lib.shifu_a1_post_physics(self.ctx.handle, C.byref(self.io(use_step_dev)), nv.current_stream()))
-
-    def compact(self):
-        nv.check(self.lib.shifu_compact_reset_ids(self.ctx.handle, nv.ptr(self.reset_buf), self.n,
-                                                  nv.ptr(self.reset_ids), nv.ptr(self.n_reset), nv.current_stream()))
+        self._stats_slot = self.slot
+        if not torch.cuda.is_current_stream_capturing():
+            self._slot_guard()
+        io = self.io(use_step_dev)
+        io.stats_slot = -1 if use_step_dev else self.slot
+        io.extras_ring = nv.ptr(self.extras_ring) if publish else None
+        nv.check(self.lib.shifu_a1_post_physics(self.ctx.handle, C.byref(io), nv.current_stream()))
 
     def reset_idx(self, env_ids: Optional[torch.Tensor], allreduce=None):
         n_ids = self.n if env_ids is None else int(env_ids.numel())
@@ -509,9 +512,9 @@
         if n_ids > 0 or allreduce is not None:
             self._finalize_stats(allreduce, False)
 
-    def finalize(self, allreduce=None, advance_step_dev: bool = False):
-        self.compact()
-        self._finalize_stats(allreduce, advance_step_dev)
+    def finalize(self, allreduce=None):
+        if allreduce is not None:
+            self._publish(allreduce)
 
     def step_resident(self, raw_actions: torch.Tensor, decimation: int = 4, use_step_dev: bool = False,
                       allreduce=None, publish: bool = True):
@@ -520,21 +523,9 @@
             self.pd_torque()
         if not self.carry_body_frame:
             self.body_frame()
-        self.post_physics(use_step_dev)
-        main = torch.cuda.current_stream()
-        if torch.cuda.is_current_stream_capturing():
-            if self._fork is None:
-                self._fork = torch.cuda.Stream(device=self.device)
-            self._fork.wait_stream(main)
-            with torch.cuda.stream(self._fork):
-                self.compact()
-        else:
-            self.compact()
-        self._collect(use_step_dev)
-        if publish:
-            self._publish(allreduce, from_step_dev=use_step_dev)
-        if torch.cuda.is_current_stream_capturing():
-            main.wait_stream(self._fork)
+        self.post_physics(use_step_dev, publish=publish and allreduce is None)
+        if publish and allreduce is not None:
+            self._publish(allreduce)
 
     def graph_step(self, raw_actions: torch.Tensor, decimation: int = 4, allreduce=None):
         if self._graph is None:
```

Result: slower. 1.716 billion, median of 6 (-12.3%).
